# numericalEFT/MCIntegration.jl

Hardware: AMD Instinct MI355X
Metric: Msamples/sec (whole node), 16-D Gaussian :vegas (higher is better)
Workload: dtype f64

## Files before the change

mcintegration.jl_amd/_lib.py:

```python
import ctypes as C
import os

_PKG = os.path.dirname(os.path.abspath(__file__))
_SO = os.path.join(_PKG, "lib", "libmci_hip.so")

MCI_OK = 0
ERR_NAMES = {1: "INVALID", 2: "HIP", 3: "COMPILE", 4: "NORMALIZATION", 5: "HISTOGRAM", 6: "COMM", 7: "NO_DEVICE"}
CONTINUOUS, DISCRETE, FERMIK = 0, 1, 2
VEGAS, VEGASMC, MCMC = 0, 1, 2
ABI_VERSION = 5
SOLVERS = {"vegas": VEGAS, "vegasmc": VEGASMC, "mcmc": MCMC, VEGAS: VEGAS, VEGASMC: VEGASMC, MCMC: MCMC}

c_double_p = C.POINTER(C.c_double)
c_int32_p = C.POINTER(C.c_int32)


class MCIError(RuntimeError):
    def __init__(self, code, msg):
        super().__init__("[MCI_ERR_%s] %s" % (ERR_NAMES.get(code, code), msg))
        self.code = code


class LeafDesc(C.Structure):
    _fields_ = [("kind", C.c_int32), ("pool", C.c_int32), ("lower", C.c_double), ("upper", C.c_double),
# ... 54 lines not shown
    ("mci_get_histogram_copies", C.c_int, [_VP, c_int32_p]),
    ("mci_set_kernel_timing", C.c_int, [_VP, C.c_int32]),
    ("mci_iteration_run", C.c_int, [_VP, C.c_int32, C.c_int64, C.c_int64, C.c_int64, C.c_int32, C.c_uint64, C.c_int64, C.c_int64, C.c_double]),
    ("mci_iteration_reduce", C.c_int, [_VP]),
    ("mci_iteration_finish", C.c_int, [_VP, C.c_int32, C.c_int64, C.c_int32, C.c_double, c_double_p, c_double_p]),
    ("mci_integrate", C.c_int, [_VP, C.POINTER(IntegrateArgs), C.POINTER(ResultC)]),
    ("mci_integrate_sweep", C.c_int, [_VP, C.POINTER(IntegrateArgs), C.c_int32, c_double_p, C.POINTER(C.c_uint64), c_double_p, c_double_p,
                                      C.POINTER(ResultC), c_double_p, c_double_p, c_int32_p]),
    ("mci_sweep_supported", C.c_int, [_VP, C.POINTER(IntegrateArgs), C.c_char_p, C.c_int32]),
    ("mci_set_sweep_leaves", C.c_int, [_VP, C.c_int32]),
    ("mci_sweep_map_doubles", C.c_int, [_VP, c_int32_p]),
    ("mci_get_iteration_log", C.c_int, [_VP, C.c_int32, c_double_p]),
    ("mci_reserve_iteration_log", C.c_int, [_VP, C.c_int32]),
    ("mci_get_packed", C.c_int, [_VP, c_double_p, C.c_int64]),
    ("mci_set_packed", C.c_int, [_VP, c_double_p, C.c_int64]),
    ("mci_packed_device_ptr", _VP, [_VP]),
    ("mci_get_grid", C.c_int, [_VP, C.c_int32, c_double_p, C.c_int32]),
    ("mci_set_grid", C.c_int, [_VP, C.c_int32, c_double_p, C.c_int32]),
    ("mci_get_distribution", C.c_int, [_VP, C.c_int32, c_double_p, c_double_p, C.c_int32]),
    ("mci_set_distribution", C.c_int, [_VP, C.c_int32, c_double_p, C.c_int32]),
    ("mci_get_reweight", C.c_int, [_VP, c_double_p, C.c_int32]),
    ("mci_set_reweight", C.c_int, [_VP, c_double_p, C.c_int32]),
    ("mci_set_reweight_goal", C.c_int, [_VP, c_double_p, C.c_int32]),
    ("mci_get_acceptance", C.c_int, [_VP, c_double_p, c_double_p, C.c_int32]),
    ("mci_save_state", C.c_int, [_VP, C.c_char_p]),
    ("mci_load_state", C.c_int, [_VP, C.c_char_p]),
    ("mci_set_train_walk", C.c_int, [_VP, C.c_int32]),
    ("mci_set_rng_bits", C.c_int, [_VP, C.c_int32]),
    ("mci_set_rng_rounds", C.c_int, [_VP, C.c_int32]),
    ("mci_set_deterministic", C.c_int, [_VP, C.c_int32]),
    ("mci_set_chain_carry", C.c_int, [_VP, C.c_int32]),
    ("mci_set_iteration_counted", C.c_int, [_VP, C.c_int32]),
    ("mci_set_persistent", C.c_int, [_VP, C.c_int32]),
    ("mci_last_integrate_persistent", C.c_int, [_VP, C.POINTER(C.c_int32)]),
    ("mci_last_chain_launch", C.c_int, [_VP, C.POINTER(C.c_int64), c_int32_p]),
    ("mci_set_stratification", C.c_int, [_VP, C.c_int32, c_int32_p, C.c_double, C.c_int64]),
    ("mci_set_stratification_off", C.c_int, [_VP]),
    ("mci_set_stratification_carry", C.c_int, [_VP, C.c_int32]),
    ("mci_get_strat_carry", C.c_int, [_VP, c_int32_p, c_int32_p]),
    ("mci_get_stratification", C.c_int, [_VP, c_int32_p, C.POINTER(C.c_int64), c_double_p]),
    ("mci_get_strat_counts", C.c_int, [_VP, C.POINTER(C.c_int64), C.c_int64]),
    ("mci_strat_plan", C.c_int, [C.c_int64, C.c_int32, C.c_int64, c_int32_p]),
    ("mci_set_chain_speculation", C.c_int, [_VP, C.c_int32, C.c_double, C.c_int32]),
    ("mci_last_chain_speculation", C.c_int, [_VP, c_int32_p, c_int32_p]),
    ("mci_chain_speculation_status", C.c_int, [_VP, C.c_int32, c_int32_p]),
    ("mci_vegas_check_status", C.c_int, [_VP, c_int32_p, c_int32_p]),
    ("mci_last_integrate_discarded", C.c_int, [_VP, C.POINTER(C.c_int64), c_int32_p]),
    ("mci_speculation_tree", C.c_int, [C.c_int32, C.c_double, C.c_int32, c_int32_p, c_int32_p, c_int32_p, C.POINTER(C.c_uint64), C.POINTER(C.c_uint64)]),
    ("mci_compile_chain_speculation", C.c_int, [_VP, C.c_int32]),
    ("mci_train", C.c_int, [_VP]),
    ("mci_sample_dump", C.c_int, [_VP, C.c_int32, C.c_uint64, C.c_int64, C.c_int64, C.c_int64, c_double_p, c_double_p, c_double_p]),
    ("mci_kernel_times_ms", C.c_int, [_VP, C.POINTER(C.c_float), C.c_int32, c_int32_p, c_int32_p, c_int32_p]),
    ("mci_kernel_clocks", C.c_int, [_VP, c_double_p, C.c_int32, c_int32_p]),
    ("mci_comm_times_ms", C.c_int, [_VP, C.POINTER(C.c_float), C.c_int32, c_int32_p]),
    ("mci_comm_collectives", C.c_int, [_VP, C.POINTER(C.c_int64), C.POINTER(C.c_int64)]),
    ("mci_reduce_size", C.c_int, [_VP, C.POINTER(C.c_int64)]),
    ("mci_external_reduce_done", C.c_int, [_VP]),
    ("mci_standardize_block", None, [C.c_int64, C.c_int64, C.c_int64, C.POINTER(C.c_int64), C.POINTER(C.c_int64)]),
    ("mci_chain_burnin", C.c_double, [C.c_int64, C.c_int64, C.c_int32]),
    ("mci_mcmc_burnin", C.c_int64, [C.c_int64, C.c_int64, C.c_int32, C.c_int32, C.c_int32, C.c_double]),
    ("mci_mcmc_auto_chains", C.c_int64, [C.c_int64, C.c_int64, C.c_int32, C.c_int32, C.c_int32, C.c_int64, C.c_int64, C.c_int32]),
    ("mci_get_hold_histogram", C.c_int, [_VP, C.POINTER(C.c_uint64)]),
    ("mci_mcmc_launch_valid", C.c_int, [_VP, c_int32_p, c_int32_p, C.POINTER(C.c_int64), C.POINTER(C.c_int64)]),
    ("mci_iteration_discard", C.c_int, [_VP]),
    ("mci_get_block_means", C.c_int, [_VP, C.c_int32, c_double_p, C.POINTER(C.c_int64), c_int32_p]),
    ("mci_reset_block_log", C.c_int, [_VP]),
    ("mci_lineage_sums", None, [c_double_p, C.c_int64, C.c_int64, C.c_int64, c_double_p, C.c_int64, C.c_int64, c_double_p, c_double_p]),
    ("mci_maxdof", None, [c_int32_p, C.c_int32, C.c_int32, c_int32_p]),
    ("mci_mean_std", None, [c_double_p, c_double_p, C.c_int64, C.c_int64, c_double_p, c_double_p]),
    ("mci_average", None, [c_double_p, c_double_p, C.c_int64, C.c_int64, C.c_int64, c_double_p, c_double_p, c_double_p]),
    ("mci_do_reweight", None, [c_double_p, c_double_p, C.c_int64, C.c_double, c_double_p]),
    ("mci_version", C.c_char_p, []),
    ("mci_abi_version", C.c_int32, []),
]
DEBUG_SIGNATURES = [
    ("mci_debug_persist_words", C.c_int, [_VP, C.POINTER(C.c_uint64), C.c_int32]),
    ("mci_debug_walk_counts", C.c_int, [_VP, C.POINTER(C.c_int64)]),
    ("mci_debug_plant_wrong_decision", C.c_int, [_VP, C.c_int32]),
    ("mci_debug_persist_spin_ticks", C.c_int, [_VP, C.c_uint64]),
    ("mci_debug_override", C.c_int, [C.c_char_p, C.c_int64, C.c_int32]),
    ("mci_debug_compiler_id", C.c_int, [C.c_char_p, C.c_char_p, C.c_int32]),
    ("mci_debug_split_chunks", C.c_int, [_VP, C.POINTER(C.c_int64), C.POINTER(C.c_int64)]),
    ("mci_debug_vegas_cursor", C.c_int, [_VP, C.POINTER(C.c_int32), C.POINTER(C.c_uint64)]),
    ("mci_debug_strat_d", C.c_int, [_VP, c_double_p, C.c_int64]),
    ("mci_debug_strat_start_d", C.c_int, [_VP, c_double_p, C.c_int64]),
    ("mci_debug_strat_dump", C.c_int, [_VP, C.c_int64, c_double_p, c_double_p, C.POINTER(C.c_int64), c_double_p, c_double_p]),
    ("mci_debug_mcmc_policy", C.c_int, [C.c_int64, C.c_int64, C.c_int64, C.c_int64]),
    ("mci_debug_vegas_check", C.c_int, [_VP, C.c_int32, C.c_uint64, C.c_int64, C.c_int64, C.c_int64, C.c_int64, c_double_p, c_double_p, c_double_p, c_double_p,
                                        C.POINTER(C.c_int64)]),
    ("mci_debug_vegas_check_launches", C.c_int, [_VP, C.POINTER(C.c_int64)]),
    ("mci_debug_vegas_check_layout", C.c_int, [_VP, c_int32_p, c_int32_p, c_double_p, C.POINTER(C.c_uint64), c_int32_p]),
    ("mci_debug_sweep_workgroups", C.c_int, [_VP, C.c_int32]),
    ("mci_debug_sweep_threads", C.c_int, [_VP, C.c_int32]),
    ("mci_debug_sweep_last_launch", C.c_int, [_VP, c_int32_p, c_int32_p]),
    ("mci_debug_sweep_lds_bytes", C.c_int, [_VP, C.POINTER(C.c_int64)]),
]

_lib = None


def library_path():
    return _SO


def use_rocm_compiler(rocm=None):
    root = rocm or os.environ.get("ROCM_PATH") or "/opt/rocm"
    mapped = set()
    try:
        with open("/proc/self/maps") as fh:
            for line in fh:
                path = line.split(None, 5)[-1].strip() if line.count(" ") >= 5 else ""
                if "amd_comgr" in path or "hiprtc" in path:
                    mapped.add(os.path.realpath(path))
    except OSError:
        pass

    def installed(names):
        for name in names:
            path = os.path.join(root, "lib", name)
            if os.path.exists(path):
                return path
        return None
    comgr, hiprtc = installed(("libamd_comgr.so.3", "libamd_comgr.so.2", "libamd_comgr.so")), installed(("libhiprtc.so.7", "libhiprtc.so"))
    have_comgr = [p for p in mapped if "amd_comgr" in p]
    if have_comgr and (comgr is None or os.path.realpath(comgr) not in have_comgr):
        return False
    done = False
    for path in (comgr, hiprtc):
        if path is not None:
            C.CDLL(path, mode=C.RTLD_GLOBAL)
            done = True
    return done


def compiler_id():
    buf = C.create_string_buffer(1024)
    lib().mci_debug_compiler_id(None, buf, len(buf))
    return buf.value.decode()


def lib():
    global _lib
    if _lib is None:
        if not os.path.exists(_SO):
            raise ImportError("%s is missing: run `python __graft_entry__.py` (hipcc --offload-arch=gfx950) first; "
                              "the MI355X engine has no Python/CPU fallback" % _SO)
        L = C.CDLL(_SO, mode=C.RTLD_GLOBAL)
        for name, res, args in SIGNATURES + DEBUG_SIGNATURES:
            fn = getattr(L, name)
            fn.restype = res
            fn.argtypes = args
        if L.mci_abi_version() != ABI_VERSION:
            raise ImportError("%s has ABI %d, this package was written against ABI %d: rebuild with `python __graft_entry__.py`" % (_SO, L.mci_abi_version(), ABI_VERSION))
        _lib = L
    return _lib


def check(rc):
    if rc != MCI_OK:
        raise MCIError(rc, lib().mci_last_error().decode(errors="replace"))
```

mcintegration.jl_amd/csrc/mci_debug.h:

```cpp
#ifndef MCI_DEBUG_H
#define MCI_DEBUG_H
#include "../../include/mci.h"
#ifdef __cplusplus
extern "C" {
#endif
int mci_debug_persist_words(mci_problem *prob, unsigned long long *out, int32_t n);
int mci_debug_walk_counts(mci_problem *prob, int64_t *out);
int mci_debug_plant_wrong_decision(mci_problem *prob, int32_t on);
int mci_debug_persist_spin_ticks(mci_problem *prob, unsigned long long ticks);
int mci_debug_override(const char *key, int64_t value, int32_t on);
int mci_debug_split_chunks(const mci_problem *prob, int64_t *chunks, int64_t *bytes);
int mci_debug_strat_dump(mci_problem *prob, int64_t n, double *x, double *y, int64_t *h, double *jac, double *w);
int mci_debug_strat_d(mci_problem *prob, double *d, int64_t n);
int mci_debug_strat_start_d(mci_problem *prob, double *d, int64_t n);
int mci_debug_vegas_cursor(const mci_problem *prob, int32_t *used, uint64_t *base);
int mci_debug_compiler_id(const char *set, char *out, int32_t n);
int mci_debug_mcmc_policy(int64_t pilot_steps, int64_t grow, int64_t carry_holds, int64_t carry_half_floors);
int mci_debug_vegas_check(mci_problem *prob, int32_t iteration, uint64_t seed, int64_t nevalperblock, int64_t block_lo, int64_t nblocks,
                          int64_t measurefreq, const double *x, const double *jac, const double *w, double *packed, int64_t *bad);
int mci_debug_vegas_check_launches(const mci_problem *prob, int64_t *launches);
int mci_debug_vegas_check_layout(const mci_problem *prob, int32_t *head, int32_t *draws, double *scales, uint64_t *own, int32_t *obs);
int mci_debug_sweep_workgroups(mci_problem *prob, int32_t g);
int mci_debug_sweep_threads(mci_problem *prob, int32_t threads);
int mci_debug_sweep_last_launch(const mci_problem *prob, int32_t *workgroups, int32_t *threads);
int mci_debug_sweep_lds_bytes(const mci_problem *prob, int64_t *bytes);
#ifdef __cplusplus
}
#endif
#endif
```

mcintegration.jl_amd/csrc/mci_device.h:

```cpp
#pragma once

namespace mci {

typedef unsigned int u32;
typedef unsigned long long u64;
typedef long long i64;

template <int I> struct IC { static constexpr int value = I; };

template <int B, int E, class F> __device__ __forceinline__ void static_for(F &&f) {
    if constexpr (B < E) {
        f(IC<B>{});
        static_for<B + 1, E>(f);
    }
}

struct u32x4 { u32 x, y, z, w; };

#ifndef MCI_PHILOX_ROUNDS
#define MCI_PHILOX_ROUNDS 10
#endif

template <bool IN_VGPR> struct RoundKeys {
    u32 a[MCI_PHILOX_ROUNDS], b[MCI_PHILOX_ROUNDS];
// ... 87 lines not shown
    return __longlong_as_double((i64)(((u64)whi << 32) | (w << 20)));
}
template <int DPC, int J> __device__ __forceinline__ double block_u12(const u32x4 &r) {
    if constexpr (DPC == 2) return J == 0 ? u12(r.x, r.y) : u12(r.z, r.w);
    else return u12_word(J == 0 ? r.x : J == 1 ? r.y : J == 2 ? r.z : r.w);
}

enum { STREAM_VEGAS = 0, STREAM_POOLINIT = 1, STREAM_MC_INIT = 2, STREAM_MC_STEP = 3, STREAM_MCMC_INIT = 4, STREAM_MCMC_STEP = 5, STREAM_MCMC_GROUP = 6, STREAM_MC_GROUP = 7 };
enum { ST_NORMALIZATION = 1, ST_HIST_NONFINITE = 2, ST_HIST_NONPOSITIVE = 4, ST_RESCALE_NONFINITE = 8, ST_MCMC_INIT = 16, ST_PERSIST_STALL = 32 };

struct SpecNode {
    int depth;
    int anc;
    int nacc;
    int levels;
    u64 needacc;
    u64 needrej;
    u64 accdepth;
    u64 anydepth;
};

struct BatchArgs {
    const double *edges;
    const double *dacc;
    const double *ddist;
    const double *reweight;
    const double *ud;
    double *part_cols;
    double *part_hist;
    double *ghist;
    double *part_pa;
    u64 seed;
    u32 iteration;
    i64 neval_per_block;
    i64 block_lo;
    int wg_per_block;
    i64 measurefreq;
    i64 nchain;
    double burnin;
    i64 nburn;
    int *status;
    double *tile_w;
    u32 *tile_bins;
    i64 tile_stride;
    i64 chunk_lo, chunk_hi, chunk_len;
    int accum;
    i64 nrows;
    int tiles_wpb;
    i64 tiles_rows;
    const double *host_w;
    double *host_mx, *host_relw;
    int *host_midx;
    i64 hm_first, hm_count, hm_stride;
    unsigned long long *hold_hist;
    int hist_atomic;
    const double *carry_x;
    const int *carry_curr;
    i64 carry_nchain, carry_cap;
    const int *carry_src;
    double *store_x;
    int *store_curr;
    i64 store_cap;
    const double *carry_P;
    double *carry_w;
    i64 carry_total;
    double *store_P;
    struct HostStep {
        i64 ne, steps, nc;
        double *cx, *cprob, *cw, *cprobability;
        int *cbin;
        double *hx, *pprob, *pprop, *puacc;
        int *pbin, *pvi;
        double *cwabs;
        int *ccurr, *cit, *ctr;
        int *pnew, *put;
        int *hidx;
        int *done;
    } hs;
    const SpecNode *spec_tab;
    int spec_lanes, spec_maxacc;
    int spec_ntree, spec_first;
    float spec_accept[8];
    u64 *clock_out;
    u64 *cursor;
    u64 cursor_base;
    u32 cursor_log2_big, cursor_ones;
};
constexpr int kCursorStride = 32;

struct DumpArgs {
    const double *edges, *dacc, *ddist, *ud;
    double *x, *jac, *w;
    int soa;
    u64 seed;
    u32 iteration;
    i64 first_index;
    i64 n;
};

template <int CTRL, int ROW_MASK> __device__ __forceinline__ double dpp_read(double v) {
    const u64 u = (u64)__double_as_longlong(v);
    const int lo = __builtin_amdgcn_update_dpp(0, (int)(u32)u, CTRL, ROW_MASK, 0xf, false);
    const int hi = __builtin_amdgcn_update_dpp(0, (int)(u32)(u >> 32), CTRL, ROW_MASK, 0xf, false);
    return __longlong_as_double((long long)(((u64)(u32)hi << 32) | (u64)(u32)lo));
}
__device__ __forceinline__ double wave_scan_incl(double v) {
    v += dpp_read<0x111, 0xf>(v);
    v += dpp_read<0x112, 0xf>(v);
    v += dpp_read<0x114, 0xf>(v);
    v += dpp_read<0x118, 0xf>(v);
    v += dpp_read<0x142, 0xa>(v);
    v += dpp_read<0x143, 0xc>(v);
    return v;
}
__device__ __forceinline__ double wave_sum(double v) {
    const u64 u = (u64)__double_as_longlong(wave_scan_incl(v));
    const u32 lo = (u32)__builtin_amdgcn_readlane((int)(u32)u, 63), hi = (u32)__builtin_amdgcn_readlane((int)(u32)(u >> 32), 63);
    return __longlong_as_double((long long)(((u64)hi << 32) | (u64)lo));
}

__device__ __forceinline__ void lds_add(double *p, double v) {
    __hip_atomic_fetch_add(p, v, __ATOMIC_RELAXED, __HIP_MEMORY_SCOPE_WORKGROUP);
}
__device__ __forceinline__ void global_add(double *p, double v) {
    __hip_atomic_fetch_add(p, v, __ATOMIC_RELAXED, __HIP_MEMORY_SCOPE_AGENT);
}

template <class Cfg> struct Mode {
    static constexpr bool EDGE_LDS = Cfg::TABLE_MODE <= 1;
    static constexpr bool HIST_LDS = Cfg::TABLE_MODE == 0 || Cfg::TABLE_MODE == 3;
};

template <class Cfg> struct Tables {
    const double *EC;
    const double *E;
    const double *DA;
    const double *DD;
};

template <int N, bool FMA, bool U12> __device__ __forceinline__ double cont_yn(double y) {
    if constexpr (FMA) {
        double Nd = (double)N;
        asm("" : "+s"(Nd));
        return __builtin_fma(y, Nd, -Nd);
    } else return (U12 ? y - 1.0 : y) * (double)N;
}
template <class Cfg> constexpr bool all_draws_pair_table() {
    if (Cfg::PAIR_TABLE == 0 || Cfg::TABLE_MODE > 1) return false;
    for (int k = 0; k < Cfg::NDRAW; ++k)
        if (Cfg::leaf_kind(Cfg::draw_leaf(k)) != 0) return false;
    return true;
}

#ifndef MCI_GATHER_X4
#define MCI_GATHER_X4 0
#endif
__device__ __forceinline__ void gather_edges(const double *e, double &g0, double &g1) {
#if MCI_GATHER_X4
    typedef double d2u __attribute__((ext_vector_type(2), aligned(8)));
    const d2u v = *reinterpret_cast<const d2u *>(e);
    g0 = v.x;
    g1 = v.y;
#else
    g0 = e[0];
    g1 = e[1];
#endif
// ... 606 lines not shown
        double *prow = a.part_pa + rowid * (2 * PaTable<Cfg>::N);
        for (int i = tid; i < 2 * PaTable<Cfg>::N && tile == 0; i += T) prow[i] = ACCUM ? prow[i] + (double)sPA[i] : (double)sPA[i];
    }
    if constexpr (Mode<Cfg>::HIST_LDS && WRITE_HIST) {
#ifndef MCI_COPY_SUM_DPP
#define MCI_COPY_SUM_DPP 0
#endif
        constexpr bool SUMMED = MCI_COPY_SUM_DPP != 0 && Cfg::DET == 0 && Cfg::HCOPY > 1 && Cfg::HCOPY <= 16 && Cfg::NTILE == 1;
        if constexpr (SUMMED) {
            constexpr int N = Cfg::HTILE * Cfg::HCOPY, K = 4;
            for (int base = 0; base < N; base += T * K) {
                double v[K];
                static_for<0, K>([&](auto Kk) {
                    constexpr int k = decltype(Kk)::value;
                    const int j = base + k * T + tid;
                    v[k] = j < N ? sH[j] : 0.0;
                });
                static_for<0, K>([&](auto Kk) {
                    constexpr int k = decltype(Kk)::value;
                    if constexpr (Cfg::HCOPY > 1) v[k] += dpp_read<0x111, 0xf>(v[k]);
                    if constexpr (Cfg::HCOPY > 2) v[k] += dpp_read<0x112, 0xf>(v[k]);
                    if constexpr (Cfg::HCOPY > 4) v[k] += dpp_read<0x114, 0xf>(v[k]);
                    if constexpr (Cfg::HCOPY > 8) v[k] += dpp_read<0x118, 0xf>(v[k]);
                });
                __syncthreads();
                static_for<0, K>([&](auto Kk) {
                    constexpr int k = decltype(Kk)::value;
                    const int j = base + k * T + tid;
                    if (j < N && (tid & (Cfg::HCOPY - 1)) == Cfg::HCOPY - 1) sH[j / Cfg::HCOPY] = v[k];
                });
            }
            __syncthreads();
        }
        static_for<0, Cfg::NTILE>([&](auto Tt) {
            constexpr int tt = decltype(Tt)::value;
            if (tile == tt) {
                double *hrow = a.part_hist + rowid * Cfg::NBIN + Cfg::tile_boff(tt);
                for (int i = tid; i < Cfg::tile_nbin(tt); i += T) {
                    constexpr int SB = (Cfg::DET != 0 || SUMMED) ? 1 : Cfg::HCOPY, SC = Cfg::DET != 0 ? Cfg::HTILE : 1;
                    double v = sH[i * SB];
                    if constexpr (!SUMMED)
                    static_for<1, Cfg::HCOPY>([&](auto Cc) { v += sH[i * SB + decltype(Cc)::value * SC]; });
                    if (!accum && a.hist_atomic) {
                        if (v != 0.0) global_add(&a.ghist[(rowid % a.hist_atomic) * Cfg::NBIN + Cfg::tile_boff(tt) + i], v);
                    } else
                    hrow[i] = accum ? hrow[i] + v : v;
                }
            }
        });
    }
}

struct CursorRule {
    u64 units;
    u32 waves;
    u32 log2_big, ones;
};
__host__ __device__ inline u64 cursor_ones(const CursorRule &r) { return (u64)r.ones * r.waves; }
__host__ __device__ inline u64 cursor_tickets(const CursorRule &r) {
    if (r.units <= cursor_ones(r)) return r.units;
    u64 rem = r.units - cursor_ones(r), n = cursor_ones(r);
    for (u32 l = 1; l < r.log2_big; ++l) {
        const u64 level = (u64)r.waves << l;
        if (rem <= level) return n + ((rem + (1ull << l) - 1ull) >> l);
        n += r.waves;
        rem -= level;
    }
    return n + ((rem + (1ull << r.log2_big) - 1ull) >> r.log2_big);
}
__host__ __device__ inline void cursor_range(const CursorRule &r, u64 ntickets, u64 t, u64 &u0, u64 &u1) {
    u64 q = ntickets - 1ull - t, e, z = 1ull;
    if (q < cursor_ones(r)) e = q;
    else {
        q -= cursor_ones(r);
        u32 l = 1;
        for (; l < r.log2_big && q >= r.waves; ++l) q -= r.waves;
        z = 1ull << l;
        e = (u64)r.waves * (r.ones + z - 2ull) + q * z;
    }
    u1 = r.units - e;
    u0 = e + z < r.units ? r.units - e - z : 0ull;
}

struct WorkItem {
    i64 rowid, lb;
    int slice, tile;
};
template <class Cfg> __device__ __forceinline__ WorkItem work_item(const BatchArgs &a) {
    WorkItem w;
#ifdef MCI_WORK_ITEM_FROM_CALLER
    w.tile = 0;
    w.rowid = a.chunk_lo;
#else
    w.tile = Cfg::NTILE == 1 ? 0 : (int)(blockIdx.x % Cfg::NTILE);
    w.rowid = Cfg::NTILE == 1 ? (i64)blockIdx.x : (i64)(blockIdx.x / Cfg::NTILE);
#endif
    w.lb = w.rowid / a.wg_per_block;
    w.slice = (int)(w.rowid % a.wg_per_block);
    return w;
}

template <class Cfg, bool SPLIT = false> __device__ __forceinline__ void vegas_batch(const BatchArgs &a) {
    extern __shared__ __attribute__((aligned(16))) double smem[];
    const int tid = threadIdx.x, T = blockDim.x;
    constexpr bool NOHIST = SPLIT && Cfg::SPLIT_ALL != 0;
    constexpr bool EC = Cfg::EC_DOUBLES > 0 && (NOHIST || !SPLIT);
    using L = typename SelectType<NOHIST, LdsEC<Cfg>, Lds<Cfg>>::type;
    double *sE = smem + L::E, *sDA = smem + L::DA, *sDD = smem + L::DD;
    double *sH = smem + L::H, *sO = smem + L::O;
    stage_tables<Cfg>(a.edges, a.dacc, a.ddist, sE, sDA, sDD);
#ifndef MCI_ZERO_B128
#define MCI_ZERO_B128 0
#endif
    if constexpr (Mode<Cfg>::HIST_LDS && !NOHIST) {
        if constexpr (MCI_ZERO_B128 != 0 && L::H % 2 == 0 && (Cfg::HTILE * Cfg::HCOPY) % 2 == 0) {
            typedef double d2 __attribute__((ext_vector_type(2)));
            d2 *z = reinterpret_cast<d2 *>(sH);
            for (int i = tid; i < Cfg::HTILE * Cfg::HCOPY / 2; i += T) z[i] = d2{0.0, 0.0};
        } else
        for (int i = tid; i < Cfg::HTILE * Cfg::HCOPY; i += T) sH[i] = 0.0;
    }
    for (int i = tid; i < Cfg::NOBS * ocopy<Cfg>(); i += T) sO[i] = 0.0;
    Tables<Cfg> t;
    t.EC = nullptr;
    if constexpr (EC) {
        double *sEC = smem + (NOHIST ? LdsEC<Cfg>::EC : Lds<Cfg>::END);
        static_for<0, Cfg::NLEAF>([&](auto Lf) {
            constexpr int l = decltype(Lf)::value;
            if constexpr (Cfg::leaf_kind(l) == 0 && Cfg::leaf_ecoff(l) >= 0)
                for (int i = tid; i <= Cfg::leaf_nbin(l); i += T) sEC[Cfg::leaf_ecoff(l) + i] = a.edges[Cfg::leaf_eoff(l) + i];
        });
        t.EC = sEC;
    }
    __syncthreads();
    if constexpr (Mode<Cfg>::EDGE_LDS) t.E = sE;
    else t.E = a.edges;
    t.DA = sDA;
    t.DD = sDD;

    WorkItem wi = work_item<Cfg>(a);
    if constexpr (SPLIT) {
        wi.tile = 0;
        wi.rowid = (i64)blockIdx.x;
        wi.lb = wi.rowid / a.wg_per_block;
        wi.slice = (int)(wi.rowid % a.wg_per_block);
    }
    const int slice = wi.slice, tile = wi.tile;
    const i64 B = a.block_lo + wi.lb;
    const u32 stream = a.iteration * 8u + STREAM_VEGAS;
    const bool pulled = pipe_eligible<Cfg>() && !SPLIT && !EC && a.cursor != nullptr;
    const i64 stride = pulled ? 64 : (i64)a.wg_per_block * T;

    double acc[Cfg::NW];
    static_for<0, Cfg::NW>([&](auto I) { acc[decltype(I)::value] = 0.0; });
    double extra[Cfg::NCOLS - Cfg::NOBS];
    static_for<0, Cfg::NCOLS - Cfg::NOBS>([&](auto I) { extra[decltype(I)::value] = 0.0; });

#ifndef MCI_PIPE_VGPR_KEYS
#define MCI_PIPE_VGPR_KEYS 0
#endif
    constexpr bool KV = MCI_PIPE_VGPR_KEYS != 0 && pipe_eligible<Cfg>() && !SPLIT && Cfg::EC_DOUBLES == 0;
    constexpr int DPC = Cfg::RNG_BITS == 32 ? 4 : 2;
    const RoundKeys<KV> keys = make_round_keys<KV>((u32)a.seed, (u32)(a.seed >> 32));
    const i64 mfreq = a.measurefreq;
    const i64 n_lo = SPLIT ? a.chunk_lo : 0, n_hi = SPLIT ? a.chunk_hi : a.neval_per_block;
    i64 mrem = mfreq == 1 ? 0 : (n_lo + (i64)slice * T + tid + 1) % mfreq;
    const i64 mstep = mfreq == 1 ? 0 : stride % mfreq;
    constexpr bool PHASED = Cfg::L1_PHASE > 0 && Cfg::HOST_INTEGRAND == 0 && gather_draw_count<Cfg, EC>() > 0;
    auto run = [&](auto TT, auto MF1c) {
    constexpr bool MF1 = decltype(MF1c)::value != 0;
    auto process = [&](const i64 n, const Sample<Cfg> &s, double *defer_wh = nullptr, auto... counted) {
        constexpr bool COUNTED = sizeof...(counted) > 0;
        double w[Cfg::NW];
        if constexpr (Cfg::HOST_INTEGRAND != 0) {
            const i64 hidx = wi.lb * a.neval_per_block + n;
            static_for<0, Cfg::NW>([&](auto Q) { w[decltype(Q)::value] = a.host_w[decltype(Q)::value * a.tile_stride + hidx]; });
        } else {
            Cfg::integrand(s.x, w, a.ud, -1);
        }
        if constexpr (!COUNTED) extra[Cols<Cfg>::NEVAL - Cfg::NOBS] += 1.0;
        bool domeasure = true;
        if constexpr (!MF1) {
            domeasure = mrem == 0;
            mrem += mstep;
            mrem = mrem >= mfreq ? mrem - mfreq : mrem;
        }
        if constexpr (Cfg::HOST_MEASURE != 0) {
            const i64 hidx = wi.lb * a.neval_per_block + n;
            static_for<0, Cfg::NDRAW>([&](auto K) { a.host_mx[decltype(K)::value * a.tile_stride + hidx] = s.x[decltype(K)::value]; });
            static_for<0, Cfg::NW>([&](auto Q) {
                constexpr int q = decltype(Q)::value;
                a.host_relw[q * a.tile_stride + hidx] = domeasure ? w[q] * s.jaci[q / Cfg::NCOMP] : 0.0;
// ... 68 lines not shown
                    r = __hip_atomic_fetch_add((global_u64 *)addr, 1ull, __ATOMIC_RELAXED, __HIP_MEMORY_SCOPE_AGENT);
                }
                return r;
            };
            auto ticket = [&](u64 r) -> u64 {
                const u32 lo = (u32)__builtin_amdgcn_readfirstlane((int)(u32)r), hi = (u32)__builtin_amdgcn_readfirstlane((int)(u32)(r >> 32));
                return (((u64)hi << 32) | lo) - a.cursor_base;
            };
            i64 n = (i64)slice * T + tid, lim = a.neval_per_block;
            u32 trips = 0u;
            u64 next = 0ull;
            if (pulled) {
                next = pull();
                n = lim = 0;
            }
            for (;;) {
                if (pulled) {
                    const u64 t = ticket(next);
                    if (t >= ntickets) break;
                    next = pull();
                    u64 u0, u1;
                    cursor_range(rule, ntickets, t, u0, u1);
                    n = (i64)(u0 << 7) + (tid & 63);
                    lim = (i64)(u1 << 7) < a.neval_per_block ? (i64)(u1 << 7) : a.neval_per_block;
                    if constexpr (!MF1) mrem = (n + 1) % mfreq;
                }
                for (; n + stride < lim; n += 2 * stride) {
                    {
                        Sample<Cfg> s;
                        draw_sample_pipe<Cfg, KV, DPC, UNI>(keys, head, stream, first + (u64)n, s, pa, pb, sH);
                        process(n, s, pb.wh, 0);
                    }
                    {
                        Sample<Cfg> s;
                        draw_sample_pipe<Cfg, KV, DPC, UNI>(keys, head, stream, first + (u64)(n + stride), s, pb, pa, sH);
                        process(n + stride, s, pa.wh, 0);
                    }
                    trips += 1u;
                }
                if (!pulled) break;
            }
            double count = 2.0 * (double)trips;
            if (n < lim) {
                Sample<Cfg> s;
                draw_sample_pipe<Cfg, KV, DPC, UNI>(keys, head, stream, first + (u64)n, s, pa, pb, sH);
                process(n, s, pb.wh, 0);
                flush(pb);
                count += 1.0;
            } else flush(pa);
            extra[Cols<Cfg>::NEVAL - Cfg::NOBS] += count;
            if constexpr (MF1) extra[Cols<Cfg>::NORM - Cfg::NOBS] += count;
        };
        if (uniform_hi) loop(IC<1>{});
        else loop(IC<0>{});
    } else {
        for (i64 n = n_lo + (i64)slice * T + tid; n < n_hi; n += stride) {
            Sample<Cfg> s;
            draw_sample<Cfg, EC, KV, DPC>(t, keys, stream, (u64)(B * a.neval_per_block + n), s);
            process(n, s);
        }
    }
    };
#ifndef MCI_MF_ONLY
#define MCI_MF_ONLY 0
#endif
    auto run_mf = [&](auto TT) { run(TT, IC<(MCI_MF_ONLY != 0 ? 1 : 0)>{}); };
    const bool stamp = !SPLIT && Cfg::NTILE == 1 && a.clock_out != nullptr && blockIdx.x == 0 && tid < 64;
    u64 ck0 = 0ull, rt0 = 0ull;
    if (stamp) {
        ck0 = __builtin_amdgcn_s_memtime();
        rt0 = __builtin_amdgcn_s_memrealtime();
    }
    if constexpr (Cfg::NTILE == 1 || SPLIT) run_mf(IC<0>{});
    else static_for<0, Cfg::NTILE>([&](auto TT) { if (tile == decltype(TT)::value) run_mf(TT); });
    if (stamp) {
        const u64 ck1 = __builtin_amdgcn_s_memtime(), rt1 = __builtin_amdgcn_s_memrealtime();
        if (tid == 0) {
            a.clock_out[0] = ck1 - ck0;
            a.clock_out[1] = rt1 - rt0;
        }
    }
    __syncthreads();
    flush_workgroup<Cfg, L, !NOHIST>(a, smem, acc, extra, wi.rowid, tile);
}

#ifndef MCI_THREADS
#define MCI_THREADS 256
#endif
constexpr int kTilesU = MCI_THREADS >= 768 ? 8 : 4;
template <int... D> struct ISeq {};
template <int N, int... D> struct MakeISeq : MakeISeq<N - 1, N - 1, D...> {};
template <int... D> struct MakeISeq<0, D...> { typedef ISeq<D...> type; };
template <int G, int SH, class V, int... D> __device__ __forceinline__ V rotate_lanes(const V b, ISeq<D...>) {
    return __builtin_shufflevector(b, b, ((D + SH) % G)...);
}
template <class Cfg> constexpr int tile_draw_count(int tt) {
    int n = 0;
    for (int k = 0; k < Cfg::NDRAW; ++k) n += (is_tdraw<Cfg>(k) && Cfg::leaf_tile(Cfg::draw_leaf(k)) == tt) ? 1 : 0;
    return n;
}
template <class Cfg> constexpr int tile_draw(int tt, int gi) {
    int n = 0;
    for (int k = 0; k < Cfg::NDRAW; ++k)
        if (is_tdraw<Cfg>(k) && Cfg::leaf_tile(Cfg::draw_leaf(k)) == tt) {
            if (n == gi) return k;
            ++n;
        }
    return 0;
}
template <class Cfg> constexpr bool tile_banked(int tt) {
    const int G = tile_draw_count<Cfg>(tt);
    if (G < 2 || G > 16) return false;
    const int k0 = tile_draw<Cfg>(tt, 0), NB = Cfg::leaf_nbin(Cfg::draw_leaf(k0));
    if (Cfg::tile_nbin(tt) != G * NB) return false;
    for (int gi = 0; gi < G; ++gi) {
        const int k = tile_draw<Cfg>(tt, gi), leaf = Cfg::draw_leaf(k);
        if (Cfg::leaf_kind(leaf) != 0 || Cfg::leaf_nbin(leaf) != NB || Cfg::cover_mask(k) != Cfg::cover_mask(k0)) return false;
        if (Cfg::leaf_boff(leaf) - Cfg::tile_boff(tt) != gi * NB) return false;
    }
    return true;
}
template <class Cfg> __device__ __forceinline__ void vegas_tiles(const BatchArgs &a) {
    static_assert(Cfg::HCOPY == 1, "histogram copies go with one tile");
    extern __shared__ __attribute__((aligned(16))) double smem[];
    const int tid = threadIdx.x, T = blockDim.x;
    double *sH = smem + Lds<Cfg>::H;
    constexpr int T0 = Cfg::SPLIT_ALL != 0 ? 0 : 1;
    constexpr int NTM = Cfg::NTILE - T0 > 0 ? Cfg::NTILE - T0 : 1;
    const i64 q = (i64)blockIdx.x / 8;
    const int tile = T0 + (int)(q % NTM);
    const i64 rowid = (q / NTM) * 8 + (i64)(blockIdx.x % 8);
    const int wpb = a.tiles_wpb > 0 ? a.tiles_wpb : a.wg_per_block;
    if (rowid >= (a.tiles_rows > 0 ? a.tiles_rows : a.nrows)) return;
    const i64 lb = rowid / wpb;
    const int slice = (int)(rowid % wpb);
    for (int i = tid; i < Cfg::HTILE * Cfg::HCOPY; i += T) sH[i] = 0.0;
    __syncthreads();
    const i64 stride = (i64)wpb * T;
    static_for<T0, Cfg::NTILE>([&](auto TT) {
        constexpr int tt = decltype(TT)::value;
        if (tile == tt) {
            constexpr int U = kTilesU;
            constexpr int NWORD = tdraw_words<Cfg>();
            static_assert(U % 4 == 0, "the replay takes its samples in groups of four");
            const i64 cnt = a.chunk_hi - a.chunk_lo;
            const bool wide = (cnt & 3) == 0 && (a.chunk_len & 3) == 0 && (a.tile_stride & 3) == 0;
            const i64 per = wide ? 4 : 1;
            for (i64 n0 = ((i64)slice * T + tid) * per; n0 < cnt; n0 += stride * U) {
                double wh[U][Cfg::NI];
                u32 word[U][NWORD > 0 ? NWORD : 1];
                bool live[U];
                static_for<0, NWORD>([&](auto J) {
                    static_for<0, U>([&](auto Uu) { word[decltype(Uu)::value][decltype(J)::value] = 0u; });
                });
                if (wide) {
                    static_for<0, U / 4>([&](auto Q) {
                        constexpr int q = decltype(Q)::value;
                        const i64 n = n0 + (i64)q * stride * 4;
                        const bool lv = n < cnt;
                        const i64 idx = lb * a.chunk_len + (lv ? n : n0);
                        static_for<0, 4>([&](auto Vv) { live[4 * q + decltype(Vv)::value] = lv; });
                        typedef double d2 __attribute__((ext_vector_type(2)));
                        typedef u32 u4 __attribute__((ext_vector_type(4)));
                        static_for<0, Cfg::NI>([&](auto I) {
                            constexpr int i = decltype(I)::value;
                            const d2 *pw = reinterpret_cast<const d2 *>(a.tile_w + (i64)i * a.tile_stride + idx);
// ... 1392 lines not shown
```

mcintegration.jl_amd/csrc/mci_host_access.h:

```cpp
int mci_get_iteration_log(mci_problem *p, int32_t nrows, double *out) {
    if (p->ctx->offline) return fail(MCI_ERR_NO_DEVICE, "offline context");
    if (nrows < 1 || nrows > p->log_row) return fail(MCI_ERR_INVALID, "only %d iterations are logged", p->log_row);
    HIPCHK(hipMemcpyAsync(out, p->d_iterlog + (size_t)(p->log_row - nrows) * p->nstat, (size_t)nrows * p->nstat * sizeof(double),
                          hipMemcpyDeviceToHost, p->ctx->stream));
    return check_status(p);
}

int mci_get_packed(mci_problem *p, double *out, int64_t n) {
    if (p->ctx->offline) return fail(MCI_ERR_NO_DEVICE, "offline context");
    if (n != p->packed_n && n != p->packed_n + 64)
        return fail(MCI_ERR_INVALID, "packed size is %lld", (long long)p->packed_n);
    if (int rc = flush_merge(p)) return rc;
    HIPCHK(hipMemcpyAsync(out, p->d_packed, (size_t)n * sizeof(double), hipMemcpyDeviceToHost, p->ctx->stream));
    HIPCHK(hipStreamSynchronize(p->ctx->stream));
    return MCI_OK;
}

int mci_set_packed(mci_problem *p, const double *in, int64_t n) {
    if (p->ctx->offline) return fail(MCI_ERR_NO_DEVICE, "offline context");
    if (n != p->packed_n && n != p->packed_n + 64)
        return fail(MCI_ERR_INVALID, "packed size is %lld", (long long)p->packed_n);
    if (int rc = flush_merge(p)) return rc;
    HIPCHK(hipMemcpyAsync(p->d_packed, in, (size_t)n * sizeof(double), hipMemcpyHostToDevice, p->ctx->stream));
    HIPCHK(hipStreamSynchronize(p->ctx->stream));
// ... 217 lines not shown
        }
        if (ok && (prod == 0 || prod != nc || !(c_beta >= 0.0) || !std::isfinite(c_beta))) {
            fclose(f);
            return fail(MCI_ERR_INVALID, "%s: the carried allocation's plan does not match its ncube = %llu (prod nstrat = %llu, beta = %g)", path,
                        (unsigned long long)nc, (unsigned long long)prod, c_beta);
        }
        if (ok) {
            c_d.resize((size_t)nc);
            ok = fread(c_d.data(), sizeof(double), c_d.size(), f) == c_d.size();
        }
        for (size_t h = 0; ok && h < c_d.size(); ++h)
            if (!(c_d[h] >= 0.0) || !std::isfinite(c_d[h])) {
                fclose(f);
                return fail(MCI_ERR_INVALID, "%s: d_h[%zu] = %g of the carried allocation is negative or not finite", path, h, c_d[h]);
            }
    }
    fclose(f);
    if (!ok) return fail(MCI_ERR_INVALID, "%s is truncated", path);
    {
        auto &st = p->strat;
        st.c_valid = !c_d.empty();
        st.c_host = std::move(c_d);
        st.c_nstrat = c_nstrat;
        st.c_ncube = (int64_t)st.c_host.size();
        st.c_beta = c_beta;
        if (st.carry) st.alloc_valid = st.alloc_pending = false;
    }
    int rc = mci_set_reweight(p, rw.data(), p->ni + 1);
    for (size_t l = 0; l < p->leaves.size() && !rc; ++l)
        if (p->leaves[l].kind != MCI_FERMIK)
        rc = p->leaves[l].kind == MCI_CONTINUOUS ? mci_set_grid(p, (int)l, tabs[l].data(), (int)tabs[l].size())
                                                 : mci_set_distribution(p, (int)l, tabs[l].data(), (int)tabs[l].size());
    return rc;
}

static int sample_dump_device(mci_problem *p, int32_t iteration, uint64_t seed, int64_t first_index, int64_t n) {
    int rc = ensure_dump(p);
    if (rc) return rc;
    HIPCHK(hipSetDevice(p->ctx->device));
    const auto &s = p->shape;
    const int64_t per = s.ndraw + 1 + s.ni * s.ncomp;
    if (n * per > p->cap_dump) {
        if (p->d_dump) (void)hipFree(p->d_dump);
        p->d_dump = nullptr;
        p->cap_dump = 0;
        HIPCHK(hipMalloc((void **)&p->d_dump, (size_t)(n * per) * sizeof(double)));
        p->cap_dump = n * per;
    }
    mci::DumpArgs a{};
    a.edges = p->d_edges;
    a.dacc = p->d_dacc;
    a.ddist = p->d_ddist;
    a.ud = p->d_ud;
    a.x = p->d_dump;
    a.jac = p->d_dump + n * s.ndraw;
    a.w = a.jac + n;
    a.seed = seed;
    a.iteration = (mci::u32)iteration;
    a.first_index = first_index;
    a.n = n;
    void *args[] = {&a};
    const unsigned grid = (unsigned)((n + 255) / 256 < 1024 ? (n + 255) / 256 : 1024);
    HIPCHK(hipModuleLaunchKernel(p->f_dump, grid, 1, 1, 256, 1, 1, (unsigned)p->lds_bytes, p->ctx->stream, args, nullptr));
    return MCI_OK;
}

int mci_sample_dump(mci_problem *p, int32_t iteration, uint64_t seed, int64_t nevalperblock, int64_t block_index, int64_t n,
                    double *x, double *jac, double *w) {
    if (p->ctx->offline) return fail(MCI_ERR_NO_DEVICE, "offline context");
    if (n < 1 || n > nevalperblock) return fail(MCI_ERR_INVALID, "n must be in 1..neval_per_block");
    int rc = sample_dump_device(p, iteration, seed, block_index * nevalperblock, n);
    if (rc) return rc;
    const auto &s = p->shape;
    const double *dx = p->d_dump, *djac = dx + n * s.ndraw, *dw = djac + n;
    if (x) HIPCHK(hipMemcpyAsync(x, dx, (size_t)n * s.ndraw * sizeof(double), hipMemcpyDeviceToHost, p->ctx->stream));
    if (jac) HIPCHK(hipMemcpyAsync(jac, djac, (size_t)n * sizeof(double), hipMemcpyDeviceToHost, p->ctx->stream));
    if (w) HIPCHK(hipMemcpyAsync(w, dw, (size_t)n * s.ni * s.ncomp * sizeof(double), hipMemcpyDeviceToHost, p->ctx->stream));
    HIPCHK(hipStreamSynchronize(p->ctx->stream));
    return MCI_OK;
}

int mci_set_kernel_timing(mci_problem *p, int32_t mode) {
    if (!p) return fail(MCI_ERR_INVALID, "NULL argument");
    p->kernel_timing = mode < 0 ? -1 : mode > 0 ? 1 : 0;
    return MCI_OK;
}

int mci_kernel_times_ms(mci_problem *p, float *ms, int32_t n, int32_t *got, int32_t *wg, int32_t *threads) {
    if (p->ctx->offline) return fail(MCI_ERR_NO_DEVICE, "offline context");
    HIPCHK(hipStreamSynchronize(p->ctx->stream));
    int64_t have = p->launch.launches < mci_problem::kEvRing ? p->launch.launches : mci_problem::kEvRing;
    if (have > n) have = n;
    int64_t k = 0;
    for (int64_t i = 0; i < have; ++i) {
        const int slot = (int)((p->launch.launches - have + i) % mci_problem::kEvRing);
        if (!p->launch.ev_valid[slot]) continue;
        float t = 0.f;
        HIPCHK(hipEventElapsedTime(&t, p->evs[2 * slot], p->evs[2 * slot + 1]));
        ms[k++] = t;
    }
    have = k;
    if (got) *got = (int32_t)have;
    if (wg) *wg = p->launch.last_wg;
    if (threads) *threads = p->launch.last_threads;
    return MCI_OK;
}

int mci_kernel_clocks(mci_problem *p, double *mhz, int32_t n, int32_t *got) {
    if (!p || !mhz || !got) return fail(MCI_ERR_INVALID, "NULL argument");
    if (p->ctx->offline) return fail(MCI_ERR_NO_DEVICE, "offline context");
    *got = 0;
    if (!p->d_clocks) return MCI_OK;
    HIPCHK(hipSetDevice(p->ctx->device));
    int khz = 0;
    HIPCHK(hipDeviceGetAttribute(&khz, hipDeviceAttributeWallClockRate, p->ctx->device));
    std::vector<unsigned long long> h((size_t)2 * mci_problem::kEvRing);
    HIPCHK(hipMemcpyAsync(h.data(), p->d_clocks, h.size() * sizeof(unsigned long long), hipMemcpyDeviceToHost, p->ctx->stream));
    HIPCHK(hipStreamSynchronize(p->ctx->stream));
    int64_t have = p->launch.launches < mci_problem::kEvRing ? p->launch.launches : mci_problem::kEvRing;
    if (have > n) have = n;
    int32_t k = 0;
    for (int64_t i = 0; i < have; ++i) {
        const int slot = (int)((p->launch.launches - have + i) % mci_problem::kEvRing);
        if (!p->launch.ev_valid[slot] || !p->launch.clock_valid[slot] || !h[(size_t)2 * slot + 1]) continue;
        mhz[k++] = (double)h[(size_t)2 * slot] / (double)h[(size_t)2 * slot + 1] * (double)khz * 1.0e-3;
    }
    *got = k;
    return MCI_OK;
}
```

mcintegration.jl_amd/csrc/mci_host_iteration.h:

```cpp
int mci_iteration_run(mci_problem *p, int32_t solver, int64_t nevalperblock, int64_t block_lo, int64_t block_hi,
                      int32_t iteration, uint64_t seed, int64_t measurefreq, int64_t nchain, double thermal_ratio) {
    if (p->ctx->offline) return fail(MCI_ERR_NO_DEVICE, "offline context: no device to run on");
    if (solver != MCI_VEGAS && solver != MCI_VEGASMC && solver != MCI_MCMC) return fail(MCI_ERR_INVALID, "Solver %d is not supported!", solver);
    const bool auto_chains = nchain <= 0;
    if (measurefreq <= 0) return fail(MCI_ERR_INVALID, "measurefreq must be positive");
    const int64_t nblocks = block_hi - block_lo;
    if (nblocks < 1 || nevalperblock < 1) return fail(MCI_ERR_INVALID, "empty iteration");
    if (p->has_fermik && solver != MCI_MCMC) return fail(MCI_ERR_INVALID, "FermiK variables work with solver=:mcmc only");
    if (p->strat.on) {
        if (solver != MCI_VEGAS) return fail(MCI_ERR_INVALID, "stratification works with solver = :vegas only (mci_set_stratification_off first)");
        return strat_run(p, nevalperblock, block_lo, block_hi, iteration, seed, measurefreq);
    }
    const int kern = (p->in_self_check && p->check_slot >= 0 && solver == MCI_VEGAS) ? p->check_slot : kslot(solver, measurefreq);
    int rc = (solver == MCI_VEGAS || p->deterministic || p->shape.host_integrand || p->spec_lanes == 1) ? compile_solver(p, kern) : MCI_OK;
    if (rc) return rc;
    if (solver == MCI_VEGAS && !p->in_self_check && !p->vegas_check_done[kern == kSlotVegasAny ? 1 : 0] &&
        (rc = vegas_check_gate(p, kern, nevalperblock, block_lo, block_hi, iteration, seed, measurefreq)))
        return rc;
    if (solver == MCI_VEGAS && (rc = compile_solver(p, kern))) return rc;
    if (solver == MCI_VEGAS && p->shape.host_integrand && (rc = ensure_dump(p))) return rc;
    if ((rc = flush_merge(p))) return rc;
    HIPCHK(hipSetDevice(p->ctx->device));
    const auto &s = p->shape;
    int T = solver_threads(p, solver);
// ... 35 lines not shown
        for (int v = 0; v < p->npool; ++v) nslots += p->maxdof[v];
        if (!(thermal_ratio >= 0.0)) return fail(MCI_ERR_INVALID, "thermal_ratio must be non-negative");
        if (nchain <= 0) {
            if ((rc = hold_consume(p))) return rc;
            const int64_t hold_eff = p->launch.mcmc_warm && p->launch.hold_prev > p->launch.hold_max ? p->launch.hold_prev : p->launch.hold_max;
            nchain = mci_mcmc_auto_chains(nevalperblock, nblocks, nslots, p->ni + 1, p->npool, hold_eff, p->launch.mcmc_warm && p->launch.hold_valid ? 0 : p->launch.hold_len,
                                          may_carry ? 1 : 0);
        }
        if (nchain > nevalperblock) return fail(MCI_ERR_INVALID, "nchain=%lld exceeds the %lld steps of a block", (long long)nchain, (long long)nevalperblock);
        nburn = (may_carry && nchain > 1) ? 0 : mci_mcmc_burnin(nevalperblock / nchain, nchain, nslots, p->ni + 1, p->npool, thermal_ratio);
        units = nchain;
    } else {
        nchain = 1;
    }
    int G = 1, spec_maxacc = 0;
    if (solver != MCI_VEGAS && !s.host_integrand && !p->deterministic && p->spec_lanes != 1) {
        if (p->spec_lanes > 1) G = p->spec_lanes;
        else {
            G = 64;
            while (G > 1 && nblocks * nchain * G > mci_problem::kSpecFill) G >>= 1;
            if (G < 8) G = 1;
        }
    }
    int T_launch = T;
    if (G > 1 && p->spec_state[solver - 1] < 0) G = 1;
    if (G > 1) {
        rc = compile_spec(p, solver);
        if (rc == MCI_ERR_COMPILE && p->spec_lanes == -1) {
            fprintf(stderr, "mci: the several-lanes-per-chain kernel of this problem did not compile; one lane per chain instead\n%s\n", mci_last_error());
            p->spec_state[solver - 1] = -2;
            G = 1;
        } else if (rc) return rc;
    }
    if (G > 1 && !p->in_self_check && ((p->spec_need_check[solver - 1] && !(g_over.spec_self_check.on && g_over.spec_self_check.v == 0)) ||
                                       (g_over.spec_self_check.on && g_over.spec_self_check.v == 1 && p->spec_state[solver - 1] == 0))) {
        if ((rc = spec_self_check(p, solver, G, nevalperblock, block_lo, block_hi, iteration, seed, measurefreq, thermal_ratio))) return rc;
        if (p->spec_state[solver - 1] < 0) G = 1;
    }
    if (G > 1) {
        if ((rc = spec_upload(p, solver, G, p->spec_accept, p->spec_maxacc))) return rc;
        spec_maxacc = p->spec_tab_maxacc;
        units = nchain * G;
        T_launch = units >= 256 ? 256 : (int)((units + 63) / 64) * 64;
    }
    if (G == 1 && (rc = compile_solver(p, kern))) return rc;
    p->launch.last_spec_lanes = G;
    p->launch.last_spec_maxacc = spec_maxacc;
    int wpb = p->wg_per_block;
    if (G > 1) {
        if (wpb <= 0) wpb = (int)((2048 + nblocks - 1) / nblocks);
        const int64_t maxw = (units + T_launch - 1) / T_launch;
        if (wpb > maxw) wpb = (int)maxw;
        if (wpb < 1) wpb = 1;
    } else
    if (wpb <= 0) {
        const int64_t big = T >= 1024 ? 1024 : T >= 512 ? 2048 : 4096;
        int64_t target = (units * nblocks >= (int64_t)1 << 25 && p->lds_bytes <= 32 * 1024) ? big : 2048;
        if (solver == MCI_VEGAS && units * nblocks < ((int64_t)1 << 22) && target > 256) target = 256;
        if (solver == MCI_VEGAS && units * nblocks * s.ndraw < ((int64_t)1 << 19) && target > 64) target = 64;
        wpb = (int)((target + nblocks - 1) / nblocks);
        const int64_t maxw = (units + T - 1) / T;
        if (wpb > maxw) wpb = (int)maxw;
        if (wpb < 1) wpb = 1;
    }
    bool cursor = false;
    if (solver == MCI_VEGAS && G == 1 && !p->in_self_check && vegas_pipe_unit(p) && !(g_over.vegas_cursor.on && g_over.vegas_cursor.v == 0)) {
        const bool forced = g_over.vegas_cursor.on && g_over.vegas_cursor.v == 1;
        if (forced) cursor = true;
        else if (p->wg_per_block <= 0 && units * nblocks >= ((int64_t)1 << 25)) {
            int resident = 0;
            if ((rc = cursor_resident(p, kern, T, &resident))) return rc;
            if (resident >= nblocks && (resident / nblocks) * nblocks > kAtomicRows) {
                cursor = true;
                wpb = (int)(resident / nblocks);
                const int64_t maxw = (units + T - 1) / T;
                if (wpb > maxw) wpb = (int)maxw;
            }
        }
    }
    const bool hist_lds = (s.table_mode == 0 || s.table_mode == 3);
    const bool split = solver == MCI_VEGAS && s.ntile > 1;
    if (!split && wpb * s.ntile > 4096 / nblocks && s.ntile > 1) wpb = (int)(4096 / nblocks / s.ntile) > 0 ? (int)(4096 / nblocks / s.ntile) : 1;
    const int64_t nrows = nblocks * wpb;
    const bool atomic_flush = solver == MCI_VEGAS && hist_lds && s.ntile == 1 && atomic_rows_ok(p) && nrows <= kAtomicRows && !s.host_integrand;
    const int64_t nwg = split ? nrows : nrows * s.ntile;
    if ((rc = ensure_capacity(p, nrows, nblocks))) return rc;
    if (solver != MCI_VEGAS && nrows > p->cap_pa) {
        if (p->d_part_pa) (void)hipFree(p->d_part_pa);
        p->d_part_pa = nullptr;
        p->cap_pa = 0;
        HIPCHK(hipMalloc((void **)&p->d_part_pa, (size_t)nrows * 2 * p->npa * sizeof(double)));
        p->cap_pa = nrows;
    }
    int64_t chunk_len = nevalperblock, nchunks = 1;
    if (split) {
        const int64_t words = p->tdraw_words > 0 ? p->tdraw_words : 1;
        const int64_t bytes = (int64_t)s.ni * 8 + words * 4;
        if (!s.host_integrand && !s.host_measure) {
            int64_t cap = (int64_t)1 << 27;
            if (cap * bytes > (int64_t)7500000000) cap = (int64_t)7500000000 / bytes;
            if (g_over.split_chunk.on && g_over.split_chunk.v > 0) cap = g_over.split_chunk.v;
            int64_t per = (cap / nblocks) & ~(int64_t)3;
            if (per < 4) per = 4;
            if (per < chunk_len) {
                chunk_len = per;
                nchunks = (nevalperblock + chunk_len - 1) / chunk_len;
            }
        }
        const int64_t nsamp = nblocks * chunk_len;
        if (nsamp > p->cap_tile) {
            tile_release(p);
            const size_t wbytes = (((size_t)nsamp * s.ni * sizeof(double)) + 255) & ~(size_t)255;
            if ((rc = tile_alloc(p, wbytes + (size_t)nsamp * words * sizeof(uint32_t)))) return rc;
            p->d_tile_bins = (uint32_t *)((char *)p->d_tile_w + wbytes);
            p->cap_tile = nsamp;
        }
        p->launch.last_split_chunks = nchunks;
        p->launch.last_split_bytes = nsamp * bytes;
    }
    mci::BatchArgs a{};
    a.edges = p->d_edges;
    a.dacc = p->d_dacc;
    a.ddist = p->d_ddist;
    a.reweight = p->d_reweight;
    a.ud = p->d_ud;
    a.part_cols = p->d_part_cols;
    a.part_hist = p->d_part_hist;
    a.ghist = p->d_ghist;
    a.part_pa = p->d_part_pa;
    a.seed = seed;
    a.iteration = (mci::u32)iteration;
    a.neval_per_block = nevalperblock;
    a.block_lo = block_lo;
    a.wg_per_block = wpb;
    a.measurefreq = measurefreq;
    a.nchain = nchain;
    a.burnin = burnin;
    a.nburn = nburn;
    const int ghist_buffers = atomic_flush ? (nrows > 64 ? 3 : 1) : 0;
    a.hist_atomic = ghist_buffers;
    if (solver != MCI_VEGAS) {
        const bool carried = may_carry && nchain > 1;
        const bool keep = carry_on && nchain > 1;
        if (keep && p->in_self_check) return fail(MCI_ERR_INVALID, "the self-check's launch would overwrite the stored chains");
        if (carried) {
            a.carry_x = p->d_chain_x[p->launch.chain_cur];
            a.carry_curr = p->d_chain_curr[p->launch.chain_cur];
            a.carry_nchain = p->launch.chain_nchain;
            a.carry_cap = p->chain_cap[p->launch.chain_cur];
        }
        if (carried) {
            if (nblocks * nchain > p->cap_carry_src) {
                if (p->d_carry_src) (void)hipFree(p->d_carry_src);
                p->d_carry_src = nullptr;
                p->cap_carry_src = 0;
                HIPCHK(hipMalloc((void **)&p->d_carry_src, (size_t)(nblocks * nchain) * sizeof(int)));
                p->cap_carry_src = nblocks * nchain;
            }
            if (nblocks * p->launch.chain_nchain > p->cap_carry_W) {
                if (p->d_carry_W) (void)hipFree(p->d_carry_W);
                p->d_carry_W = nullptr;
                p->cap_carry_W = 0;
                HIPCHK(hipMalloc((void **)&p->d_carry_W, (size_t)(nblocks * p->launch.chain_nchain) * sizeof(double)));
                p->cap_carry_W = nblocks * p->launch.chain_nchain;
            }
            mci::ResampleArgs ra{};
            ra.curr_old = p->d_chain_curr[p->launch.chain_cur];
// ... 164 lines not shown
        } else {
            const int64_t mfq = measurefreq > 0 ? measurefreq : 1;
            const int64_t last = solver == MCI_VEGASMC ? nevalperblock / nchain : nevalperblock / nchain + nburn;
            hm_first = 1;
            if (solver == MCI_VEGASMC) {
                hm_first = (int64_t)(burnin / (double)mfq);
                if (hm_first < 1) hm_first = 1;
                while (hm_first > 1 && (double)((hm_first - 1) * mfq) >= burnin) --hm_first;
                while ((double)(hm_first * mfq) < burnin) ++hm_first;
            } else if (nburn > 0) {
                hm_first = (nburn + mfq - 1) / mfq;
                if (hm_first < 1) hm_first = 1;
            }
            hm_count = last / mfq - hm_first + 1;
            if (hm_count < 0) hm_count = 0;
            hm_n = nchain * hm_count;
            hm_rows = solver == MCI_MCMC ? s.ncomp : nw;
        }
        const int64_t n = nblocks * hm_n > 0 ? nblocks * hm_n : 1;
        if ((double)n * (double)(s.ndraw + nw + 1) * 8.0 > 8.0 * 1024 * 1024 * 1024)
            return fail(MCI_ERR_INVALID, "a host measure over %lld records of %d doubles per launch (more than 8 GiB): lower neval, raise measurefreq "
                                         "or give the measure as device source (mci_set_measure_source)", (long long)n, s.ndraw + nw);
        if (n > p->cap_hmeas) {
            if (p->d_mx) (void)hipFree(p->d_mx);
            if (p->d_mrelw) (void)hipFree(p->d_mrelw);
            if (p->d_midx) (void)hipFree(p->d_midx);
            if (p->h_mx) (void)hipHostFree(p->h_mx);
            if (p->h_mrelw) (void)hipHostFree(p->h_mrelw);
            if (p->h_midx) (void)hipHostFree(p->h_midx);
            p->d_mx = p->d_mrelw = p->h_mx = p->h_mrelw = nullptr;
            p->d_midx = p->h_midx = nullptr;
            p->cap_hmeas = 0;
            HIPCHK(hipMalloc((void **)&p->d_mx, (size_t)n * s.ndraw * sizeof(double)));
            HIPCHK(hipMalloc((void **)&p->d_mrelw, (size_t)n * nw * sizeof(double)));
            HIPCHK(hipMalloc((void **)&p->d_midx, (size_t)n * sizeof(int32_t)));
            HIPCHK(hipHostMalloc((void **)&p->h_mx, (size_t)n * s.ndraw * sizeof(double), hipHostMallocDefault));
            HIPCHK(hipHostMalloc((void **)&p->h_mrelw, (size_t)n * nw * sizeof(double), hipHostMallocDefault));
            HIPCHK(hipHostMalloc((void **)&p->h_midx, (size_t)n * sizeof(int32_t), hipHostMallocDefault));
            p->cap_hmeas = n;
        }
        if (nblocks * s.nobs > p->cap_mobs) {
            if (p->d_mobs) (void)hipFree(p->d_mobs);
            p->d_mobs = nullptr;
            HIPCHK(hipMalloc((void **)&p->d_mobs, (size_t)nblocks * s.nobs * sizeof(double)));
            p->cap_mobs = nblocks * s.nobs;
        }
        a.host_mx = p->d_mx;
        a.host_relw = p->d_mrelw;
        a.host_midx = p->d_midx;
        a.hm_first = hm_first;
        a.hm_count = hm_count;
        a.hm_stride = nblocks * hm_n;
        if (solver != MCI_VEGAS) {
            HIPCHK(hipMemsetAsync(p->d_mx, 0, (size_t)n * s.ndraw * sizeof(double), p->ctx->stream));
            HIPCHK(hipMemsetAsync(p->d_mrelw, 0, (size_t)n * hm_rows * sizeof(double), p->ctx->stream));
            HIPCHK(hipMemsetAsync(p->d_midx, 0xFF, (size_t)n * sizeof(int32_t), p->ctx->stream));
        }
    }
    if (cursor) {
        mci::CursorRule r;
        r.units = (mci::u64)((nevalperblock + 127) >> 7);
        r.waves = (mci::u32)(wpb * (T / 64));
        r.log2_big = (mci::u32)(g_over.cursor_log2_big.on && g_over.cursor_log2_big.v >= 1 && g_over.cursor_log2_big.v <= 16 ? g_over.cursor_log2_big.v : mci_problem::kCursorLog2Big);
        r.ones = (mci::u32)(g_over.cursor_ones.on && g_over.cursor_ones.v >= 1 && g_over.cursor_ones.v <= 4096 ? g_over.cursor_ones.v : mci_problem::kCursorOnes);
        if (nblocks != p->cursor_nblocks) {
            if (nblocks > p->cap_cursor) {
                if (p->d_cursor) (void)hipFree(p->d_cursor);
                p->d_cursor = nullptr;
                p->cap_cursor = 0;
                HIPCHK(hipMalloc((void **)&p->d_cursor, (size_t)nblocks * mci::kCursorStride * sizeof(unsigned long long)));
                p->cap_cursor = nblocks;
            }
            HIPCHK(hipMemsetAsync(p->d_cursor, 0, (size_t)nblocks * mci::kCursorStride * sizeof(unsigned long long), p->ctx->stream));
            p->cursor_nblocks = nblocks;
            p->cursor_base = 0;
        }
        a.cursor = p->d_cursor;
        a.cursor_base = p->cursor_base;
        a.cursor_log2_big = r.log2_big;
        a.cursor_ones = r.ones;
        p->cursor_base += mci::cursor_tickets(r) + r.waves;
    }
    p->launch.last_cursor = cursor;
    void *args[] = {&a};
    hipFunction_t f = p->f_solver[G > 1 ? (solver == MCI_VEGASMC ? kSlotVegasmcSpec : kSlotMcmcSpec) : kern];
    hipStream_t st = p->ctx->stream;
    const int slot = (int)(p->launch.launches % mci_problem::kEvRing);
    p->launch.time_this_launch = p->kernel_timing > 0 || (p->kernel_timing < 0 && nblocks * nevalperblock >= ((int64_t)1 << 20));
    if (p->launch.time_this_launch && solver == MCI_VEGAS) {
        if (!p->d_clocks) {
            HIPCHK(hipMalloc((void **)&p->d_clocks, (size_t)2 * mci_problem::kEvRing * sizeof(unsigned long long)));
            HIPCHK(hipMemsetAsync(p->d_clocks, 0, (size_t)2 * mci_problem::kEvRing * sizeof(unsigned long long), st));
        }
        a.clock_out = p->d_clocks + 2 * slot;
    }
    if (p->launch.time_this_launch) HIPCHK(hipEventRecord(p->evs[2 * slot], st));
    if (solver != MCI_VEGAS && s.host_integrand) {
        const int64_t nc = nblocks * nchain, steps = nevalperblock / nchain;
        const int nw = s.ni * s.ncomp, nd = s.ndraw;
        if (nc >= ((int64_t)1 << 31) || steps + nburn >= ((int64_t)1 << 31) - 1) return fail(MCI_ERR_INVALID, "too many chains or steps for the host-closure path");
        if (nc > p->cap_hstep) {
            if (p->d_hstep) (void)hipFree(p->d_hstep);
            p->d_hstep = nullptr;
            p->cap_hstep = 0;
            HIPCHK(hipMalloc(&p->d_hstep, (size_t)nc * ((3 * nd + nw + 4) * sizeof(double) + (2 * nd + 7) * sizeof(int)) + 16));
            p->cap_hstep = nc;
        }
        if (nc > p->cap_hidx) {
            if (p->h_hidx) (void)hipHostFree(p->h_hidx);
            p->h_hidx = nullptr;
            p->cap_hidx = 0;
            HIPCHK(hipHostMalloc((void **)&p->h_hidx, (size_t)(nc + 1) * sizeof(int32_t), hipHostMallocDefault));
            p->cap_hidx = nc;
        }
        {
            double *dp = (double *)p->d_hstep;
            a.hs.cx = dp; dp += (size_t)nd * nc;
            a.hs.cprob = dp; dp += (size_t)nd * nc;
            a.hs.pprob = dp; dp += (size_t)nd * nc;
            a.hs.cw = dp; dp += (size_t)nw * nc;
            a.hs.cprobability = dp; dp += nc;
            a.hs.pprop = dp; dp += nc;
            a.hs.puacc = dp; dp += nc;
            a.hs.cwabs = dp; dp += nc;
            int *ip = (int *)dp;
            a.hs.cbin = ip; ip += (size_t)nd * nc;
            a.hs.pbin = ip; ip += (size_t)nd * nc;
            a.hs.pvi = ip; ip += nc;
            a.hs.ccurr = ip; ip += nc;
            a.hs.cit = ip; ip += nc;
            a.hs.ctr = ip; ip += nc;
            a.hs.pnew = ip; ip += nc;
            a.hs.put = ip; ip += nc;
            a.hs.hidx = ip; ip += nc;
            a.hs.done = ip;
        }
        a.hs.hx = p->d_hx;
        a.hs.nc = nc;
        a.hs.steps = steps;
        HIPCHK(hipMemsetAsync(p->d_part_cols, 0, (size_t)nrows * s.ncols * sizeof(double), st));
        if (hist_lds && s.nbin > 0) HIPCHK(hipMemsetAsync(p->d_part_hist, 0, (size_t)nrows * s.nbin * sizeof(double), st));
        HIPCHK(hipMemsetAsync(p->d_part_pa, 0, (size_t)nrows * 2 * p->npa * sizeof(double), st));
        HIPCHK(hipMemsetAsync(a.hs.done, 0, sizeof(int), st));
        if (solver == MCI_VEGASMC) {
            for (int64_t ne = 0; ne <= steps + 1; ++ne) {
                a.hs.ne = ne;
                HIPCHK(hipModuleLaunchKernel(f, (unsigned)nwg, 1, 1, (unsigned)T, 1, 1, (unsigned)solver_lds(p, solver), st, args, nullptr));
                if (ne > steps) break;
                HIPCHK(hipMemcpyAsync(p->h_hx, p->d_hx, (size_t)nc * nd * sizeof(double), hipMemcpyDeviceToHost, st));
                HIPCHK(hipStreamSynchronize(st));
                if ((rc = eval_host_integrand(p, nullptr, p->h_hx, p->h_hw, nc))) return rc;
                HIPCHK(hipMemcpyAsync(p->d_hw, p->h_hw, (size_t)nc * nw * sizeof(double), hipMemcpyHostToDevice, st));
            }
        } else {
            const int64_t limit = steps + nburn + 2 + 10000;
            for (int64_t ne = 0;; ++ne) {
                a.hs.ne = ne;
                HIPCHK(hipModuleLaunchKernel(f, (unsigned)nwg, 1, 1, (unsigned)T, 1, 1, (unsigned)solver_lds(p, solver), st, args, nullptr));
                HIPCHK(hipMemcpyAsync(p->h_hidx, a.hs.hidx, (size_t)(nc + 1) * sizeof(int32_t), hipMemcpyDeviceToHost, st));
                HIPCHK(hipMemcpyAsync(p->h_hx, p->d_hx, (size_t)nc * nd * sizeof(double), hipMemcpyDeviceToHost, st));
                HIPCHK(hipStreamSynchronize(st));
                if (p->h_hidx[nc] >= nc) break;
                if (ne > limit) return fail(MCI_ERR_INVALID, "host-closure :mcmc chains did not finish (%d of %lld)", (int)p->h_hidx[nc], (long long)nc);
                if ((rc = eval_host_integrand(p, p->h_hidx, p->h_hx, p->h_hw, nc))) return rc;
                HIPCHK(hipMemcpyAsync(p->d_hw, p->h_hw, (size_t)nc * s.ncomp * sizeof(double), hipMemcpyHostToDevice, st));
            }
        }
    } else
    for (int64_t c = 0; c < nchunks; ++c) {
        if (nchunks > 1) {
            a.chunk_lo = c * chunk_len;
            a.chunk_hi = a.chunk_lo + chunk_len < nevalperblock ? a.chunk_lo + chunk_len : nevalperblock;
            a.accum = c > 0 ? 1 : 0;
        }
        HIPCHK(hipModuleLaunchKernel(f, (unsigned)nwg, 1, 1, (unsigned)T_launch, 1, 1, (unsigned)solver_lds(p, solver), st, args, nullptr));
        if (split && c + 1 < nchunks)
            HIPCHK(hipModuleLaunchKernel(p->f_tiles[kern == kSlotVegasAny ? 1 : 0], (unsigned)(((hist_rows + 7) / 8) * 8 * (s.ntile - (s.split_all ? 0 : 1))), 1, 1, (unsigned)T, 1, 1, (unsigned)p->lds_bytes, st, args, nullptr));
    }
    if (solver == MCI_MCMC) p->launch.hold_measured = a.hold_hist != nullptr;
    if (a.hold_hist && auto_chains && (rc = hold_publish(p, nevalperblock / nchain, solver != MCI_VEGAS && p->launch.last_carried))) return rc;
    if (split)
        HIPCHK(hipModuleLaunchKernel(p->f_tiles[kern == kSlotVegasAny ? 1 : 0], (unsigned)(((hist_rows + 7) / 8) * 8 * (s.ntile - (s.split_all ? 0 : 1))), 1, 1, (unsigned)T, 1, 1, (unsigned)p->lds_bytes, st, args, nullptr));
    if (p->launch.time_this_launch) HIPCHK(hipEventRecord(p->evs[2 * slot + 1], st));
    p->launch.ev_valid[slot] = p->launch.time_this_launch;
    p->launch.clock_valid[slot] = a.clock_out != nullptr && !split && s.ntile == 1;
    p->launch.launches += 1;
    if (s.host_measure) {
        const int64_t n = nblocks * hm_n;
        const int nw = s.ni * s.ncomp, nc = s.ncomp;
        std::vector<double> obs((size_t)nblocks * s.nobs, 0.0);
        if (n > 0 && !p->in_self_check) {
            HIPCHK(hipMemcpyAsync(p->h_mx, p->d_mx, (size_t)n * s.ndraw * sizeof(double), hipMemcpyDeviceToHost, st));
            HIPCHK(hipMemcpyAsync(p->h_mrelw, p->d_mrelw, (size_t)n * hm_rows * sizeof(double), hipMemcpyDeviceToHost, st));
            if (solver == MCI_MCMC) HIPCHK(hipMemcpyAsync(p->h_midx, p->d_midx, (size_t)n * sizeof(int32_t), hipMemcpyDeviceToHost, st));
            HIPCHK(hipStreamSynchronize(st));
            const double *relw = p->h_mrelw;
            if (solver == MCI_MCMC && p->hmeas_fn) {
                p->h_mtmp.assign((size_t)n * nw, 0.0);
                for (int64_t i = 0; i < n; ++i)
                    if (p->h_midx[i] >= 0)
                        for (int q = 0; q < nc; ++q) p->h_mtmp[(size_t)(p->h_midx[i] * nc + q) * n + i] = p->h_mrelw[(size_t)q * n + i];
                relw = p->h_mtmp.data();
            }
            if (solver != MCI_MCMC && p->hmeas_idx_fn) p->h_mitmp.resize((size_t)hm_n);
            const bool squeeze = solver == MCI_VEGAS && measurefreq > 1;
            const int64_t keep = squeeze ? nevalperblock / measurefreq : hm_n;
            std::vector<double> sx, sw;
            if (squeeze) {
                sx.resize((size_t)(keep > 0 ? keep : 1) * s.ndraw);
                sw.resize((size_t)(keep > 0 ? keep : 1) * nw);
            }
            for (int64_t b = 0; b < nblocks; ++b) {
                const int64_t off = b * hm_n;
                double *ob = obs.data() + (size_t)b * s.nobs;
                int hrc = 0;
                if (squeeze) {
                    for (int k = 0; k < s.ndraw; ++k)
                        for (int64_t j = 0; j < keep; ++j) sx[(size_t)k * keep + j] = p->h_mx[(size_t)k * n + off + (j + 1) * measurefreq - 1];
                    for (int q = 0; q < nw; ++q)
                        for (int64_t j = 0; j < keep; ++j) sw[(size_t)q * keep + j] = relw[(size_t)q * n + off + (j + 1) * measurefreq - 1];
                    if (p->hmeas_fn) hrc = p->hmeas_fn(sx.data(), sw.data(), keep, keep, s.ndraw, nw, block_lo + b, ob, s.nobs, p->hmeas_user);
                    else {
                        p->h_mitmp.resize((size_t)(keep > 0 ? keep : 1));
                        for (int j = 0; j < s.ni && !hrc; ++j) {
                            std::fill(p->h_mitmp.begin(), p->h_mitmp.end(), (int32_t)j);
                            hrc = p->hmeas_idx_fn(p->h_mitmp.data(), sx.data(), sw.data() + (size_t)j * nc * keep, keep, keep, s.ndraw, nc, block_lo + b, ob,
                                                  s.nobs, p->hmeas_user);
                        }
                    }
                } else if (p->hmeas_fn) {
                    hrc = p->hmeas_fn(p->h_mx + off, relw + off, hm_n, n, s.ndraw, nw, block_lo + b, ob, s.nobs, p->hmeas_user);
                } else if (solver == MCI_MCMC) {
                    hrc = p->hmeas_idx_fn(p->h_midx + off, p->h_mx + off, relw + off, hm_n, n, s.ndraw, nc, block_lo + b, ob, s.nobs, p->hmeas_user);
                } else {
                    for (int j = 0; j < s.ni && !hrc; ++j) {
                        std::fill(p->h_mitmp.begin(), p->h_mitmp.end(), (int32_t)j);
                        hrc = p->hmeas_idx_fn(p->h_mitmp.data(), p->h_mx + off, relw + (size_t)j * nc * n + off, hm_n, n, s.ndraw, nc, block_lo + b, ob,
                                              s.nobs, p->hmeas_user);
                    }
                }
                if (hrc) return fail(MCI_ERR_INVALID, "the host measure failed (%d)", hrc);
            }
        }
        HIPCHK(hipMemcpyAsync(p->d_mobs, obs.data(), obs.size() * sizeof(double), hipMemcpyHostToDevice, st));
        hipLaunchKernelGGL(mci::k_add_host_obs, dim3((unsigned)((nblocks * s.nobs + 255) / 256)), dim3(256), 0, st, p->d_mobs, (int)nblocks, s.nobs, s.ncols, wpb,
                           p->d_part_cols);
        HIPCHK(hipGetLastError());
        HIPCHK(hipStreamSynchronize(st));
    }
    p->launch.last_samples = nblocks * nevalperblock;
    p->launch.last_wg = (int)nwg;
    p->launch.last_threads = T_launch;
    p->launch.last_nblocks = (int)nblocks;
    if (solver != MCI_VEGAS) p->launch.last_nchain = nchain;
    const int nb256 = (s.nbin + 255) / 256;
    if (hist_lds && s.nbin > 0 && !atomic_flush)
        hipLaunchKernelGGL(mci::k_hist_stage1, dim3(nb256, mci_problem::kGroups), dim3(256), 0, st, p->d_part_hist, (int)hist_rows, s.nbin,
                           (int)mci_problem::kGroups, p->d_stage1);
    HIPCHK(hipGetLastError());
    mci::MergeArgs &m = p->merge;
    m.part_cols = p->d_part_cols;
    m.ncols = s.ncols;
    m.nobs = s.nobs;
    m.ni = s.ni;
    m.nblocks = (int)nblocks;
    m.wg_per_block = wpb;
    m.stage1 = p->d_stage1;
    m.ngroup = (int)mci_problem::kGroups;
    m.ghist = p->d_ghist;
    m.use_ghist = (hist_lds && !atomic_flush) ? 0 : atomic_flush ? ghist_buffers : 1;
    m.nbin = s.nbin;
    m.packed = p->d_packed;
    m.status = p->d_status;
    m.scratch = p->d_scratch;
    m.part_pa = solver != MCI_VEGAS ? p->d_part_pa : nullptr;
    m.npa = p->npa;
    m.nrows = (int)nrows;
    m.block_means = nullptr;
    m.hist_no_offset = (p->in_self_check && p->check_slot >= 0) ? 1 : 0;
    m.hold = a.hold_hist;
    if (solver != MCI_VEGAS && !p->in_self_check) {
        const int64_t stride = nblocks * s.nobs;
        if (stride != p->launch.blk_stride || block_lo != p->launch.blk_lo) {
            p->launch.blk_rows = 0;
            p->launch.blk_carried = 0;
            p->launch.blk_stride = stride;
            p->launch.blk_lo = block_lo;
        }
        if ((rc = grow_block_log(p, p->launch.blk_rows + 1))) return rc;
        m.block_means = p->d_blocklog + (size_t)p->launch.blk_rows * stride;
        p->launch.blk_rows += 1;
        p->launch.blk_carried += p->launch.last_carried ? 1 : 0;
    }
    p->merge_pending = true;
    return MCI_OK;
}

static int flush_merge(mci_problem *p) {
    if (!p->merge_pending) return MCI_OK;
    p->merge_pending = false;
    HIPCHK(hipSetDevice(p->ctx->device));
    const int nb256 = (p->shape.nbin + 255) / 256;
    hipLaunchKernelGGL(mci::k_finalize, dim3(nb256 + 1 + (2 * p->npa + 3) / 4), dim3(256), 0, p->ctx->stream, p->merge);
    HIPCHK(hipGetLastError());
    return MCI_OK;
}

int mci_iteration_reduce(mci_problem *p) {
    if (p->ctx->offline) return fail(MCI_ERR_NO_DEVICE, "offline context");
    if (!p->ctx->comm) return MCI_OK;
    int rc = flush_merge(p);
    if (rc) return rc;
    const bool timed = p->launch.time_this_launch;
    const int slot = (int)(p->reduces % mci_problem::kCevRing);
    if (timed) {
        if (p->cevs.empty()) {
            p->cevs.resize(2 * mci_problem::kCevRing);
            for (auto &e : p->cevs) HIPCHK(hipEventCreate(&e));
        }
        HIPCHK(hipEventRecord(p->cevs[2 * slot], p->ctx->stream));
    }
    const size_t count = (size_t)p->packed_n + (p->launch.hold_deferred ? 64 : 0);
    int r = g_rccl.AllReduce(p->d_packed, p->d_packed, count, kNcclFloat64, kNcclSum, p->ctx->comm, p->ctx->stream);
    if (r) return fail(MCI_ERR_COMM, "ncclAllReduce: %s", g_rccl.GetErrorString ? g_rccl.GetErrorString(r) : "?");
    p->ctx->collectives += 1;
    p->ctx->last_count = (long long)count;
    if (p->launch.hold_deferred && (rc = hold_publish_reduced(p))) return rc;
    if (timed) HIPCHK(hipEventRecord(p->cevs[2 * slot + 1], p->ctx->stream));
    p->cev_valid[slot] = timed;
    p->reduces += 1;
    return MCI_OK;
}

int mci_comm_collectives(const mci_ctx *c, int64_t *calls, int64_t *last_count) {
    if (!c) return fail(MCI_ERR_INVALID, "NULL argument");
    if (calls) *calls = c->collectives;
    if (last_count) *last_count = c->last_count;
    return MCI_OK;
}

int mci_external_reduce_done(mci_problem *p) {
    if (!p) return fail(MCI_ERR_INVALID, "NULL argument");
    if (p->ctx->offline) return fail(MCI_ERR_NO_DEVICE, "offline context");
    if (!p->launch.hold_ext_pending) return MCI_OK;
    p->launch.hold_ext_pending = false;
    HIPCHK(hipSetDevice(p->ctx->device));
    return hold_publish_reduced(p);
}

int mci_reduce_size(const mci_problem *p, int64_t *n) {
    if (!p || !n) return fail(MCI_ERR_INVALID, "NULL argument");
    *n = p->packed_n + 64;
    return MCI_OK;
}

int mci_comm_times_ms(mci_problem *p, float *ms, int32_t n, int32_t *got) {
    if (!p || !ms || !got) return fail(MCI_ERR_INVALID, "NULL argument");
    if (p->ctx->offline) return fail(MCI_ERR_NO_DEVICE, "offline context");
    HIPCHK(hipStreamSynchronize(p->ctx->stream));
    int64_t have = p->reduces < mci_problem::kCevRing ? p->reduces : mci_problem::kCevRing;
    if (have > n) have = n;
    int32_t k = 0;
    for (int64_t i = 0; i < have; ++i) {
        const int slot = (int)((p->reduces - have + i) % mci_problem::kCevRing);
        if (!p->cev_valid[slot]) continue;
        float t = 0.f;
        HIPCHK(hipEventElapsedTime(&t, p->cevs[2 * slot], p->cevs[2 * slot + 1]));
        ms[k++] = t;
    }
    *got = k;
    return MCI_OK;
}

static int launch_train(mci_problem *p, int do_train, int do_reweight, double gamma, double *log_row) {
    const auto &s = p->shape;
    int maxn = 1;
    for (auto &L : p->leaves) maxn = L.nbin > maxn ? L.nbin : maxn;
    mci::TrainArgs a{};
    a.leaves = p->d_leaves;
    a.nleaf = s.nleaf;
    a.packed = p->d_packed;
    a.nstat = p->nstat;
    a.edges = p->d_edges;
    a.dacc = p->d_dacc;
    a.ddist = p->d_ddist;
    a.iter_log_row = log_row;
    a.reweight = p->d_reweight;
    a.goal = p->h_goal.empty() ? nullptr : p->d_goal;
    a.nd = s.ni + 1;
    a.do_reweight = do_reweight;
    a.gamma = gamma;
    a.do_train = do_train;
    if (do_train) p->ntrain += 1;
    a.serial_walk = p->train_serial >= 0 ? p->train_serial : (p->launch.last_samples == 0 || p->launch.last_samples >= mci_problem::kSerialWalkSamples) ? 1 : 0;
    if (p->debug_wrong_decision && a.serial_walk == 1) a.serial_walk = 3;
    a.status = p->d_status;
    a.maxn = maxn;
    a.spare = (size_t)(mci::train_lds_doubles(maxn) + mci::train_spare_doubles(maxn)) * sizeof(double) <= (size_t)kTrainLdsMax ? 1 : 0;
    const size_t sm = (size_t)(mci::train_lds_doubles(maxn) + (a.spare ? mci::train_spare_doubles(maxn) : maxn)) * sizeof(double);
    const unsigned tt = maxn > 256 ? 512u : 256u;
    if (sm > 64 * 1024 && !p->train_lds_raised) {
        HIPCHK(hipFuncSetAttribute((const void *)mci::k_train, hipFuncAttributeMaxDynamicSharedMemorySize, (int)kTrainLdsMax));
        HIPCHK(hipFuncSetAttribute((const void *)mci::k_finish, hipFuncAttributeMaxDynamicSharedMemorySize, (int)kTrainLdsMax));
        p->train_lds_raised = true;
    }
    if (p->merge_pending) {
        p->merge_pending = false;
        hipLaunchKernelGGL(mci::k_finish, dim3(s.nleaf + 1 + (2 * p->npa + 3) / 4), dim3(tt), sm, p->ctx->stream, p->merge, a);
    } else {
        hipLaunchKernelGGL(mci::k_train, dim3(s.nleaf + 1), dim3(tt), sm, p->ctx->stream, a);
    }
    HIPCHK(hipGetLastError());
    return MCI_OK;
}

static int grow_iteration_log(mci_problem *p, int64_t need) {
    if (need <= p->cap_iter) return MCI_OK;
    int64_t ncap = p->cap_iter ? p->cap_iter : 64;
    while (ncap < need) ncap *= 2;
    double *n = nullptr;
    HIPCHK(hipMalloc((void **)&n, (size_t)ncap * p->nstat * sizeof(double)));
    if (p->d_iterlog) {
        HIPCHK(hipMemcpyAsync(n, p->d_iterlog, (size_t)p->cap_iter * p->nstat * sizeof(double), hipMemcpyDeviceToDevice, p->ctx->stream));
        HIPCHK(hipStreamSynchronize(p->ctx->stream));
        (void)hipFree(p->d_iterlog);
    }
    p->d_iterlog = n;
    p->cap_iter = ncap;
    return MCI_OK;
}

int mci_reserve_iteration_log(mci_problem *p, int32_t rows) {
    if (!p || rows < 0) return fail(MCI_ERR_INVALID, "bad argument");
    if (p->ctx->offline) return fail(MCI_ERR_NO_DEVICE, "offline context");
    HIPCHK(hipSetDevice(p->ctx->device));
    return grow_iteration_log(p, (int64_t)p->log_row + rows);
}

int mci_iteration_finish(mci_problem *p, int32_t solver, int64_t block_total, int32_t adapt, double gamma, double *mean, double *std) {
    if (p->ctx->offline) return fail(MCI_ERR_NO_DEVICE, "offline context");
    HIPCHK(hipSetDevice(p->ctx->device));
    const auto &s = p->shape;
    if (int grc = grow_iteration_log(p, (int64_t)p->log_row + 1)) return grc;
    double *row = p->d_iterlog + (size_t)p->log_row * p->nstat;
    const bool strat = p->strat.last_run;
    int rc = launch_train(p, adapt ? 1 : 0, (solver == MCI_VEGASMC || solver == MCI_MCMC) ? 1 : 0, gamma, row);
    if (rc) return rc;
    if (strat && (rc = strat_finish(p, row, adapt))) return rc;
    p->log_row += 1;
    if (mean || std) {
        std::vector<double> h(p->nstat);
        HIPCHK(hipMemcpyAsync(h.data(), row, (size_t)p->nstat * sizeof(double), hipMemcpyDeviceToHost, p->ctx->stream));
        if ((rc = check_status(p))) return rc;
        std::vector<double> m(s.nobs), e(s.nobs);
        if (strat) strat_mean_std(h.data(), s.nobs, m.data(), e.data());
        else
        mci_mean_std(h.data(), h.data() + s.nobs, s.nobs, block_total, m.data(), e.data());
        if (mean) memcpy(mean, m.data(), s.nobs * sizeof(double));
        if (std) memcpy(std, e.data(), s.nobs * sizeof(double));
    }
    return MCI_OK;
}

int mci_train(mci_problem *p) {
    if (p->ctx->offline) return fail(MCI_ERR_NO_DEVICE, "offline context");
    int rc = flush_merge(p);
    if (rc) return rc;
    rc = launch_train(p, 1, 0, 1.0, nullptr);
    if (rc) return rc;
    return check_status(p);
}
```

mcintegration.jl_amd/csrc/mci_host_jit.h:

```cpp
enum { kSlotVegasAny = 3, kSlotDump = 4, kSlotVegasmcSpec = 5, kSlotMcmcSpec = 6 };
static int kslot(int solver, int64_t measurefreq) { return solver == MCI_VEGAS && measurefreq != 1 ? kSlotVegasAny : solver; }
static int slot_solver(int slot) { return slot == kSlotVegasAny ? MCI_VEGAS : slot == kSlotVegasmcSpec ? MCI_VEGASMC : slot == kSlotMcmcSpec ? MCI_MCMC : slot; }

namespace {
struct Candidate {
    std::string src;
    int threads = 256;
    std::vector<char> code;
    std::string log, path;
    bool cached = false;
    int rc = 0;
    long vgprs() const { return mcijit::kernel_vgprs(code, "mci_vegas_batch"); }
    long scratch() const { return mcijit::kernel_scratch_bytes(code, "mci_vegas_batch"); }
};
void compile_all(std::vector<Candidate *> &cs) {
    std::vector<std::thread> th;
    for (size_t i = 1; i < cs.size(); ++i)
        th.emplace_back([c = cs[i]] { c->rc = mcijit::compile(c->src, c->threads, c->code, c->log, c->cached, &c->path); });
    if (!cs.empty()) cs[0]->rc = mcijit::compile(cs[0]->src, cs[0]->threads, cs[0]->code, cs[0]->log, cs[0]->cached, &cs[0]->path);
    for (auto &t : th) t.join();
}
}

static int load_slot(mci_problem *p, int slot, Candidate &c, int64_t lds) {
// ... 446 lines not shown
    if (solver == MCI_VEGASMC_LANES || solver == MCI_MCMC_LANES) {
        const int sl = solver == MCI_VEGASMC_LANES ? kSlotVegasmcSpec : kSlotMcmcSpec;
        if (!p->compiled[sl]) return fail(MCI_ERR_INVALID, "the several-lanes-per-chain kernel has not been compiled yet");
        snprintf(buf, (size_t)n, "%s", p->code_object[sl].c_str());
        return MCI_OK;
    }
    if (solver == MCI_VEGAS_STRAT) {
        if (!p->strat.compiled) return fail(MCI_ERR_INVALID, "the stratified :vegas kernel has not been compiled yet");
        snprintf(buf, (size_t)n, "%s", p->strat.code_object.c_str());
        return MCI_OK;
    }
    if (solver == MCI_VEGAS_SWEEP) {
        if (!p->sweep.compiled) return fail(MCI_ERR_INVALID, "the sweep kernel has not been compiled yet");
        snprintf(buf, (size_t)n, "%s", p->sweep.code_object.c_str());
        return MCI_OK;
    }
    if (solver == MCI_VEGAS_SWEEP_LEAVES) {
        if (!p->sweep.leaves.compiled) return fail(MCI_ERR_INVALID, "the sweep kernel for several leaves has not been compiled yet");
        snprintf(buf, (size_t)n, "%s", p->sweep.leaves.code_object.c_str());
        return MCI_OK;
    }
    if (solver < 0 || solver > 2) return fail(MCI_ERR_INVALID, "Solver %d is not supported!", solver);
    const int slot = (solver == MCI_VEGAS && !p->compiled[solver] && p->compiled[kSlotVegasAny]) ? kSlotVegasAny : solver;
    if (!p->compiled[slot]) return fail(MCI_ERR_INVALID, "solver %d has not been compiled yet", solver);
    snprintf(buf, (size_t)n, "%s", p->code_object[slot].c_str());
    return MCI_OK;
}

int mci_set_rng_bits(mci_problem *p, int32_t bits) {
    if (!p) return fail(MCI_ERR_INVALID, "NULL argument");
    if (bits != 52 && bits != 32) return fail(MCI_ERR_INVALID, "rng bits must be 52 (default: the resolution of rand(Float64)) or 32");
    if (p->shape.rng_bits != bits) {
        p->shape.rng_bits = bits;
        drop_modules(p);
    }
    return MCI_OK;
}

int mci_set_rng_rounds(mci_problem *p, int32_t rounds) {
    if (!p) return fail(MCI_ERR_INVALID, "NULL argument");
    if (rounds != 10 && rounds != 7) return fail(MCI_ERR_INVALID, "Philox4x32 rounds must be 10 (default) or 7 (the fewest that pass BigCrush)");
    if (p->shape.rng_rounds != rounds) {
        p->shape.rng_rounds = rounds;
        drop_modules(p);
    }
    return MCI_OK;
}

int mci_set_train_walk(mci_problem *p, int32_t mode) {
    if (!p) return fail(MCI_ERR_INVALID, "NULL argument");
    if (mode < -1 || mode > 2) return fail(MCI_ERR_INVALID, "train walk mode must be -1 (automatic), 0 (prefix scan), 1 (serial recurrence) or 2 (serial recurrence, general form only)");
    p->train_serial = mode;
    return MCI_OK;
}

int mci_debug_plant_wrong_decision(mci_problem *p, int32_t on) {
    if (!p) return fail(MCI_ERR_INVALID, "NULL argument");
    p->debug_wrong_decision = on != 0;
    return MCI_OK;
}

int mci_debug_override(const char *key, int64_t value, int32_t on) {
    Override *o = override_slot(key);
    if (!o) return fail(MCI_ERR_INVALID, "no such override: %s", key ? key : "(null)");
    o->on = on != 0;
    o->v = value;
    return MCI_OK;
}

int mci_debug_split_chunks(const mci_problem *p, int64_t *chunks, int64_t *bytes) {
    if (!p) return fail(MCI_ERR_INVALID, "NULL argument");
    if (chunks) *chunks = p->launch.last_split_chunks;
    if (bytes) *bytes = p->launch.last_split_bytes;
    return MCI_OK;
}

int mci_debug_vegas_cursor(const mci_problem *p, int32_t *used, uint64_t *base) {
    if (!p) return fail(MCI_ERR_INVALID, "NULL argument");
    if (used) *used = p->launch.last_cursor ? 1 : 0;
    if (base) *base = p->cursor_base;
    return MCI_OK;
}

int mci_debug_compiler_id(const char *set, char *out, int32_t n) {
    if (set) mcijit::compiler_id_override() = set;
    if (out && n > 0) snprintf(out, (size_t)n, "%s", mcijit::compiler_id().c_str());
    return MCI_OK;
}

int mci_debug_mcmc_policy(int64_t pilot_steps, int64_t grow, int64_t carry_holds, int64_t carry_half_floors) {
    if (pilot_steps > 0) mci_problem::kMcmcPilotSteps = pilot_steps;
    if (grow > 0) mci_problem::kMcmcGrow = grow;
    if (carry_holds > 0) mci_problem::kMcmcCarryHolds = carry_holds;
    if (carry_half_floors > 0) mci_problem::kMcmcCarryHalfFloors = carry_half_floors;
    return MCI_OK;
}

int mci_debug_persist_spin_ticks(mci_problem *p, unsigned long long ticks) {
    if (!p || ticks == 0) return fail(MCI_ERR_INVALID, "bad argument");
    p->persist_spin_ticks = ticks;
    return MCI_OK;
}

int mci_set_deterministic(mci_problem *p, int32_t on) {
    if (!p) return fail(MCI_ERR_INVALID, "NULL argument");
    const bool want = on != 0;
    if (want != p->deterministic) {
        p->deterministic = want;
        p->shape.det = want ? 1 : 0;
        drop_modules(p);
    }
    return MCI_OK;
}

int mci_set_chain_carry(mci_problem *p, int32_t mode) {
    if (!p) return fail(MCI_ERR_INVALID, "NULL argument");
    if (mode < -1 || mode > 1) return fail(MCI_ERR_INVALID, "chain carry mode must be -1 (automatic) or 1 (many-chain launches of :vegasmc and :mcmc continue the chains of the iteration before) or 0 (every launch starts its chains afresh)");
    p->chain_carry = mode;
    if (mode == 0) p->launch.chain_valid = false;
    return MCI_OK;
}

int mci_set_iteration_counted(mci_problem *p, int32_t counted) {
    if (!p) return fail(MCI_ERR_INVALID, "NULL argument");
    p->launch_counted = counted != 0;
    return MCI_OK;
}

int mci_set_persistent(mci_problem *p, int32_t mode) {
    if (!p) return fail(MCI_ERR_INVALID, "NULL argument");
    if (mode < -1 || mode > 1) return fail(MCI_ERR_INVALID, "persistent mode must be -1 (automatic: launch-bound :vegas calls), 0 (one launch chain per iteration) or 1 (whenever the layout allows)");
    p->persistent = mode;
    return MCI_OK;
}

int mci_debug_persist_words(mci_problem *p, unsigned long long *out, int32_t n) {
    if (!p || !out || !p->d_persist) return fail(MCI_ERR_INVALID, "no persistent launch yet");
    HIPCHK(hipStreamSynchronize(p->ctx->stream));
    HIPCHK(hipMemcpy(out, p->d_persist, (size_t)(n < (int)kPersistWords ? n : (int)kPersistWords) * sizeof(unsigned long long), hipMemcpyDeviceToHost));
    return MCI_OK;
}

int mci_debug_walk_counts(mci_problem *p, int64_t *out) {
    if (!p || !out || !p->d_status) return fail(MCI_ERR_INVALID, "NULL argument");
    int h[2] = {0, 0};
    HIPCHK(hipStreamSynchronize(p->ctx->stream));
    HIPCHK(hipMemcpy(h, p->d_status + 1, sizeof(h), hipMemcpyDeviceToHost));
    out[0] = h[0];
    out[1] = h[1];
    return MCI_OK;
}

int mci_last_integrate_persistent(const mci_problem *p, int32_t *persistent) {
    if (!p || !persistent) return fail(MCI_ERR_INVALID, "NULL argument");
    *persistent = p->last_persistent ? 1 : 0;
    return MCI_OK;
}

int mci_last_chain_launch(const mci_problem *p, int64_t *nchain, int32_t *carried) {
    if (!p) return fail(MCI_ERR_INVALID, "NULL argument");
    if (nchain) *nchain = p->launch.last_nchain;
    if (carried) *carried = p->launch.last_carried ? 1 : 0;
    return MCI_OK;
}

int mci_check_status(mci_problem *p) {
// ... 58 lines not shown
```

mcintegration.jl_amd/csrc/mci_host_problem.h:

```cpp
int mci_problem_create(mci_ctx *ctx, const mci_problem_desc *d, mci_problem **out) {
    if (!ctx || !d || !out) return fail(MCI_ERR_INVALID, "NULL argument");
    if (d->nleaf < 1 || d->npool < 1 || d->nintegrand < 1) return fail(MCI_ERR_INVALID, "At least one integrand is required.");
    if (d->nintegrand > 31) return fail(MCI_ERR_INVALID, "at most 31 integrands are supported");
    mci_problem *p = new mci_problem();
    p->ctx = ctx;
    p->npool = d->npool;
    p->ni = d->nintegrand;
    const int Nd = p->ni + 1;
    p->dof.assign((size_t)Nd * p->npool, 0);
    for (int i = 0; i < p->ni * p->npool; ++i) {
        if (d->dof[i] < 0) { delete p; return fail(MCI_ERR_INVALID, "dof must be non-negative"); }
        p->dof[i] = d->dof[i];
    }
    p->maxdof.assign(p->npool, 0);
    mci_maxdof(p->dof.data(), Nd, p->npool, p->maxdof.data());
    p->pool_leaf0.assign(p->npool, -1);
    p->pool_nleaf.assign(p->npool, 0);
    auto &s = p->shape;
    int eoff = 0, aoff = 0, doff = 0, boff = 0;
    for (int l = 0; l < d->nleaf; ++l) {
        const mci_leaf_desc &ld = d->leaves[l];
        if (ld.pool < 0 || ld.pool >= p->npool) { delete p; return fail(MCI_ERR_INVALID, "leaf %d: pool out of range", l); }
        if (p->pool_leaf0[ld.pool] < 0) p->pool_leaf0[ld.pool] = l;
        else if (p->pool_leaf0[ld.pool] + p->pool_nleaf[ld.pool] != l) { delete p; return fail(MCI_ERR_INVALID, "leaves of pool %d are not contiguous", ld.pool); }
// ... 224 lines not shown
        if (s.split_all) {
            int64_t budget = (lim1 - fixed) / 8;
            for (size_t l = 0; l < p->leaves.size(); ++l) {
                const Leaf &L = p->leaves[l];
                if (L.kind != MCI_CONTINUOUS || s.ec_doubles + L.nbin + 1 > budget) continue;
                s.leaf_ecoff[l] = s.ec_doubles;
                s.ec_doubles += L.nbin + 1;
            }
        }
        p->lds_bytes_k1 = fixed + (int64_t)s.ec_doubles * 8;
        p->ntdraw = 0;
        int tdraw_maxbin = 2;
        if (s.ntile > 1)
            for (int k = 0; k < s.ndraw; ++k) {
                const Leaf &L = p->leaves[s.draw_leaf[k]];
                if (L.adapt && s.cover_mask[k] && s.leaf_tile[s.draw_leaf[k]] >= (s.split_all ? 0 : 1)) {
                    p->ntdraw += 1;
                    if (L.nbin > 65536) { delete p; return fail(MCI_ERR_INVALID, "leaf %d: more than 65536 bins with tiled histograms", s.draw_leaf[k]); }
                    if (s.leaf_nbin[s.draw_leaf[k]] > tdraw_maxbin) tdraw_maxbin = s.leaf_nbin[s.draw_leaf[k]];
                }
            }
        {
            int bits = 1;
            while ((1 << bits) < tdraw_maxbin) ++bits;
            p->tdraw_words = (p->ntdraw * bits + 31) / 32;
        }
        s.htile = 0;
        for (int v : s.tile_nbin) s.htile = v > s.htile ? v : s.htile;
        s.table_mode = mode;
        s.pair_table = pair;
        const bool hist_lds = (mode == 0 || mode == 3);
        p->lds_bytes = fixed + (mode <= 1 ? (pair ? e2 : e1) : 0) + (hist_lds ? (int64_t)s.htile * 8 : 0);
        s.hcopy = 1;
        {
            int hc = 1;
            const int64_t one = (int64_t)s.htile * 8;
            int nadd = 0;
            for (int k = 0; k < s.ndraw; ++k) nadd += (p->leaves[s.draw_leaf[k]].adapt && s.cover_mask[k]) ? 1 : 0;
            if (mode == 0 && s.ntile == 1 && p->lds_bytes <= lim0 && nadd >= 4)
                while (hc < 8 && p->lds_bytes + one * (2 * hc - 1) <= lim0) hc *= 2;
            if (g_over.hist_copies.on) {
                hc = (int)g_over.hist_copies.v;
                while (hc > 1 && (!hist_lds || s.ntile != 1 || (hc & (hc - 1)) || p->lds_bytes + one * (hc - 1) > lim1)) hc >>= 1;
                if (hc < 1) hc = 1;
            }
            s.hcopy = p->hcopy_auto = p->hcopy_rule = hc;
        }
        const int64_t hcopy_bytes = (int64_t)s.htile * 8 * (s.hcopy - 1);
        if (mode == 3 && s.ntile == 1) {
            const int64_t budget = (lim1 - p->lds_bytes - hcopy_bytes) / 8;
            for (size_t l = 0; l < p->leaves.size(); ++l) {
                const Leaf &L = p->leaves[l];
                if (L.kind != MCI_CONTINUOUS || s.ec_doubles + L.nbin + 1 > budget) continue;
                s.leaf_ecoff[l] = s.ec_doubles;
                s.ec_doubles += L.nbin + 1;
            }
            p->lds_bytes_k1 = p->lds_bytes + (int64_t)s.ec_doubles * 8;
        }
        s.l1_phase = (mode == 3 && s.split_all) ? 1 : 0;
        if (g_over.l1_phase.on) s.l1_phase = (mode >= 2 && g_over.l1_phase.v > 0) ? 1 : 0;
        if (p->lds_bytes > lim0) p->threads = 512;
        if (p->lds_bytes > lim0) {
            p->vegas_plan_a = true;
            p->threads_vegas = 1024;
        }
        if (s.hcopy > 1 && !p->vegas_plan_a) {
            p->hcopy_plan = true;
            p->threads_vegas = 512;
        }
    }
    p->nstat = 2 * s.nobs + 2 + Nd;
    p->packed_n = p->nstat + s.nbin + 2 * p->npa;
    p->h_reweight.assign(Nd, 1.0 / Nd);
    s.body = "w[0] = 1.0;";
    if (!ctx->offline) {
        HIPCHK(hipSetDevice(ctx->device));
        int rc = upload(p);
        if (rc) { delete p; return rc; }
        HIPCHK(hipMalloc((void **)&p->d_packed, (size_t)(p->packed_n + 64) * sizeof(double)));
        HIPCHK(hipMemset(p->d_packed, 0, (size_t)(p->packed_n + 64) * sizeof(double)));
        HIPCHK(hipMalloc((void **)&p->d_ghist, 3 * (size_t)(s.nbin ? s.nbin : 1) * sizeof(double)));
        HIPCHK(hipMemset(p->d_ghist, 0, 3 * (size_t)(s.nbin ? s.nbin : 1) * sizeof(double)));
        HIPCHK(hipMalloc((void **)&p->d_stage1, (size_t)mci_problem::kGroups * (s.nbin ? s.nbin : 1) * sizeof(double)));
        HIPCHK(hipMalloc((void **)&p->d_status, 4 * sizeof(int)));
        HIPCHK(hipMemset(p->d_status, 0, 4 * sizeof(int)));
        std::vector<mci::LeafDev> ld;
        for (auto &L : p->leaves) ld.push_back({L.kind, L.nbin, L.eoff, L.doff, L.boff, L.adapt, L.alpha});
        HIPCHK(hipMalloc((void **)&p->d_leaves, ld.size() * sizeof(mci::LeafDev)));
        HIPCHK(hipMemcpy(p->d_leaves, ld.data(), ld.size() * sizeof(mci::LeafDev), hipMemcpyHostToDevice));
        p->evs.resize(2 * mci_problem::kEvRing);
        for (auto &e : p->evs) HIPCHK(hipEventCreate(&e));
    }
    *out = p;
    return MCI_OK;
}

static void strat_free_buffers(mci_problem *p);
int mci_problem_destroy(mci_problem *p) {
    if (!p) return MCI_OK;
    if (!p->ctx->offline) {
        (void)hipStreamSynchronize(p->ctx->stream);
        for (void *q : {(void *)p->d_edges, (void *)p->d_dacc, (void *)p->d_ddist, (void *)p->d_reweight, (void *)p->d_ud,
                        (void *)p->d_part_cols, (void *)p->d_part_hist, (void *)p->d_ghist, (void *)p->d_stage1,
                        (void *)p->d_packed, (void *)p->d_scratch, (void *)p->d_iterlog, (void *)p->d_dump,
                        (void *)p->d_status, (void *)p->d_leaves})
            if (q) (void)hipFree(q);
        for (int k = 0; k < mci_problem::kSlots; ++k)
            if (p->module[k]) (void)hipModuleUnload(p->module[k]);
        if (p->module_persist) (void)hipModuleUnload(p->module_persist);
        if (p->strat.module) (void)hipModuleUnload(p->strat.module);
        if (p->sweep.module) (void)hipModuleUnload(p->sweep.module);
        if (p->sweep.leaves.module) (void)hipModuleUnload(p->sweep.leaves.module);
        strat_free_buffers(p);
        if (p->d_persist) (void)hipFree(p->d_persist);
    }
    persist_job_drop(p);
    if (!p->ctx->offline) {
        if (p->d_goal) (void)hipFree(p->d_goal);
        if (p->d_part_pa) (void)hipFree(p->d_part_pa);
        if (p->d_hold) (void)hipFree(p->d_hold);
        for (int b = 0; b < 2; ++b) {
            if (p->d_chain_x[b]) (void)hipFree(p->d_chain_x[b]);
            if (p->d_chain_curr[b]) (void)hipFree(p->d_chain_curr[b]);
        }
        if (p->d_reweight_used) (void)hipFree(p->d_reweight_used);
        if (p->d_carry_W) (void)hipFree(p->d_carry_W);
        if (p->d_carry_src) (void)hipFree(p->d_carry_src);
        if (p->d_spec_tab) (void)hipFree(p->d_spec_tab);
        for (int b = 0; b < 2; ++b)
            if (p->d_chain_P[b]) (void)hipFree(p->d_chain_P[b]);
        if (p->d_carry_w) (void)hipFree(p->d_carry_w);
        if (p->d_clocks) (void)hipFree(p->d_clocks);
        if (p->d_cursor) (void)hipFree(p->d_cursor);
        if (p->d_edges_backup) (void)hipFree(p->d_edges_backup);
        if (p->h_hold) (void)hipHostFree(p->h_hold);
        if (p->h_hold_d) (void)hipHostFree(p->h_hold_d);
        if (p->h_log) (void)hipHostFree(p->h_log);
        if (p->hold_ev) (void)hipEventDestroy(p->hold_ev);
        if (p->d_blocklog) (void)hipFree(p->d_blocklog);
        for (auto &e : p->cevs) (void)hipEventDestroy(e);
        if (p->d_hx) (void)hipFree(p->d_hx);
        if (p->d_hstep) (void)hipFree(p->d_hstep);
        if (p->h_hidx) (void)hipHostFree(p->h_hidx);
        if (p->d_hw) (void)hipFree(p->d_hw);
        if (p->h_hx) (void)hipHostFree(p->h_hx);
        if (p->h_hw) (void)hipHostFree(p->h_hw);
        tile_release(p);
        if (p->d_mx) (void)hipFree(p->d_mx);
        if (p->d_mrelw) (void)hipFree(p->d_mrelw);
        if (p->d_mobs) (void)hipFree(p->d_mobs);
        if (p->h_mx) (void)hipHostFree(p->h_mx);
        if (p->h_mrelw) (void)hipHostFree(p->h_mrelw);
        if (p->d_midx) (void)hipFree(p->d_midx);
        if (p->h_midx) (void)hipHostFree(p->h_midx);
        for (auto &e : p->evs) (void)hipEventDestroy(e);
    }
    delete p;
    return MCI_OK;
}

int mci_set_integrand_source(mci_problem *p, const char *body, const double *ud, int32_t nud) {
    if (!p || !body) return fail(MCI_ERR_INVALID, "NULL argument");
    p->shape.body = body;
    p->shape.host_integrand = 0;
    p->host_fn = nullptr;
    p->h_ud.assign(ud, ud + (nud > 0 ? nud : 0));
    drop_modules(p);
    if (!p->ctx->offline) {
        if (p->d_ud) (void)hipFree(p->d_ud);
        p->d_ud = nullptr;
        HIPCHK(hipMalloc((void **)&p->d_ud, (p->h_ud.size() ? p->h_ud.size() : 1) * sizeof(double)));
        if (p->h_ud.size()) HIPCHK(hipMemcpy(p->d_ud, p->h_ud.data(), p->h_ud.size() * sizeof(double), hipMemcpyHostToDevice));
    }
    return MCI_OK;
}

int mci_set_integrand_host(mci_problem *p, mci_host_integrand_fn fn, void *user) {
    if (!p || !fn) return fail(MCI_ERR_INVALID, "NULL argument");
    p->host_fn = fn;
    p->host_user = user;
    p->host_idx_fn = nullptr;
    p->shape.host_integrand = 1;
    p->shape.body = "";
    p->h_ud.clear();
    drop_modules(p);
    if (!p->ctx->offline && !p->d_ud) HIPCHK(hipMalloc((void **)&p->d_ud, sizeof(double)));
    return MCI_OK;
}

int mci_set_integrand_host_indexed(mci_problem *p, mci_host_integrand_idx_fn fn, void *user) {
    if (!p || !fn) return fail(MCI_ERR_INVALID, "NULL argument");
    p->host_idx_fn = fn;
    p->host_fn = nullptr;
    p->host_user = user;
    p->shape.host_integrand = 1;
    p->shape.body = "";
    p->h_ud.clear();
    drop_modules(p);
    if (!p->ctx->offline && !p->d_ud) HIPCHK(hipMalloc((void **)&p->d_ud, sizeof(double)));
    return MCI_OK;
}

static int eval_host_integrand(mci_problem *p, const int32_t *idx, const double *x, double *w, int64_t n) {
    const auto &s = p->shape;
    const int nw = s.ni * s.ncomp, nc = s.ncomp;
    int hrc = 0;
    if (!idx) {
        memset(w, 0, (size_t)n * nw * sizeof(double));
        if (p->host_fn) hrc = p->host_fn(x, w, n, s.ndraw, nw, p->host_user);
        else {
            std::vector<int32_t> which((size_t)n);
            for (int j = 0; j < s.ni && !hrc; ++j) {
                std::fill(which.begin(), which.end(), j);
                hrc = p->host_idx_fn(which.data(), x, w + (size_t)j * nc * n, n, s.ndraw, nc, p->host_user);
            }
        }
// ... 120 lines not shown
```

mcintegration.jl_amd/csrc/mci_host_strat.h:

```cpp
static_assert(mci::kStratMaxCols == mci::kStratReduceCols, "k_strat_reduce keeps the columns the sample kernel writes");
static int flush_merge(mci_problem *p);

static const int64_t kStratSamplesPerCube = 8;

int mci_strat_plan(int64_t neval, int32_t ndim, int64_t max_nhcube, int32_t *nstrat) {
    if (!nstrat || ndim < 1) return fail(MCI_ERR_INVALID, "stratification: ndim must be positive");
    if (max_nhcube < 1) return fail(MCI_ERR_INVALID, "stratification: max_nhcube must be positive");
    const int64_t per = neval / kStratSamplesPerCube, cap = per < max_nhcube ? per : max_nhcube;
    if (cap < 1) return fail(MCI_ERR_INVALID, "stratification: neval = %lld is too small for %lld samples per hypercube", (long long)neval,
                             (long long)kStratSamplesPerCube);
    auto power_le = [cap](int64_t v, int n) {
        int64_t r = 1;
        for (int i = 0; i < n; ++i) {
            if (r > cap / v) return cap + 1;
            r *= v;
        }
        return r;
    };
    int64_t s = (int64_t)floor(pow((double)cap, 1.0 / ndim));
    if (s < 1) s = 1;
    while (s > 1 && power_le(s, ndim) > cap) --s;
    while (power_le(s + 1, ndim) <= cap) ++s;
    int64_t ncube = power_le(s, ndim);
    for (int d = 0; d < ndim; ++d) nstrat[d] = (int32_t)s;
// ... 382 lines not shown
    if ((rc = ensure_capacity(p, nwg, 1))) return rc;
    if (nchunk > st.cap_chunk) {
        for (void *q : {(void *)st.d_part, (void *)st.d_rec_s, (void *)st.d_rec_h})
            if (q) (void)hipFree(q);
        st.d_part = st.d_rec_s = nullptr;
        st.d_rec_h = nullptr;
        st.cap_chunk = 0;
        HIPCHK(hipMalloc((void **)&st.d_part, (size_t)nchunk * 2 * NW * sizeof(double)));
        HIPCHK(hipMalloc((void **)&st.d_rec_s, (size_t)nchunk * 2 * 2 * NW * sizeof(double)));
        HIPCHK(hipMalloc((void **)&st.d_rec_h, (size_t)nchunk * 2 * sizeof(long long)));
        st.cap_chunk = nchunk;
    }
    if (!st.d_stat) HIPCHK(hipMalloc((void **)&st.d_stat, 2 * mci::kStratMaxCols * sizeof(double)));
    st.ran = true;
    st.last_nchunk = nchunk;

    mci::BatchArgs a{};
    a.edges = p->d_edges;
    a.dacc = p->d_dacc;
    a.ddist = p->d_ddist;
    a.reweight = p->d_reweight;
    a.ud = p->d_ud;
    a.part_cols = p->d_part_cols;
    a.part_hist = p->d_part_hist;
    a.ghist = p->d_ghist;
    a.seed = seed;
    a.iteration = (mci::u32)iteration;
    a.neval_per_block = nevalperblock;
    a.block_lo = block_lo;
    a.wg_per_block = (int)nwg;
    a.measurefreq = 1;
    a.nchain = 1;
    a.status = p->d_status;
    a.hist_atomic = 0;
    a.nrows = nwg;
    mci::StratArgs sa{};
    sa.off = st.d_off;
    sa.dnext = st.d_d;
    sa.part = st.d_part;
    sa.rec_h = st.d_rec_h;
    sa.rec_s = st.d_rec_s;
    sa.ncube = st.ncube;
    sa.nsamp = N;
    sa.chunk = S;
    sa.nchunk = nchunk;
    sa.first_index = block_lo * nevalperblock;
    sa.nloc = (int)(S / 2 + 1);
    sa.beta = st.beta;
    for (int d = 0; d < s.ndraw; ++d) {
        const uint32_t n = (uint32_t)st.nstrat[d];
        strat_magic(n, &sa.magic[d], &sa.shift[d]);
        sa.nstrat[d] = (int)n;
        sa.inv[d] = 1.0 / (double)n;
    }
    struct Scratch {
        void *q[5] = {nullptr, nullptr, nullptr, nullptr, nullptr};
        ~Scratch() {
            for (void *v : q)
                if (v) (void)hipFree(v);
        }
    } dump;
    const bool dumping = st.hn > 0;
    if (dumping) {
        if (st.hn != N) return fail(MCI_ERR_INVALID, "mci_debug_strat_dump: %lld samples asked for, the iteration has %lld", (long long)st.hn, (long long)N);
        HIPCHK(hipMalloc(&dump.q[0], (size_t)N * s.ndraw * sizeof(double)));
        HIPCHK(hipMalloc(&dump.q[1], (size_t)N * s.ndraw * sizeof(double)));
        HIPCHK(hipMalloc(&dump.q[2], (size_t)N * sizeof(long long)));
        HIPCHK(hipMalloc(&dump.q[3], (size_t)N * sizeof(double)));
        HIPCHK(hipMalloc(&dump.q[4], (size_t)N * NW * sizeof(double)));
        sa.dump_x = (double *)dump.q[0];
        sa.dump_y = (double *)dump.q[1];
        sa.dump_h = (long long *)dump.q[2];
        sa.dump_jac = (double *)dump.q[3];
        sa.dump_w = (double *)dump.q[4];
    }
    void *args[] = {&a, &sa};
    const int slot = (int)(p->launch.launches % mci_problem::kEvRing);
    p->launch.time_this_launch = p->kernel_timing > 0 || (p->kernel_timing < 0 && N >= ((int64_t)1 << 20));
    if (p->launch.time_this_launch) HIPCHK(hipEventRecord(p->evs[2 * slot], p->ctx->stream));
    HIPCHK(hipModuleLaunchKernel(st.f, (unsigned)nwg, 1, 1, (unsigned)T, 1, 1, (unsigned)lds, p->ctx->stream, args, nullptr));
    if (p->launch.time_this_launch) HIPCHK(hipEventRecord(p->evs[2 * slot + 1], p->ctx->stream));
    p->launch.ev_valid[slot] = p->launch.time_this_launch;
    p->launch.clock_valid[slot] = false;
    p->launch.launches += 1;
    if (dumping) {
        hipStream_t hs = p->ctx->stream;
        HIPCHK(hipMemcpyAsync(st.hx, dump.q[0], (size_t)N * s.ndraw * sizeof(double), hipMemcpyDeviceToHost, hs));
        HIPCHK(hipMemcpyAsync(st.hy, dump.q[1], (size_t)N * s.ndraw * sizeof(double), hipMemcpyDeviceToHost, hs));
        HIPCHK(hipMemcpyAsync(st.hh, dump.q[2], (size_t)N * sizeof(long long), hipMemcpyDeviceToHost, hs));
        HIPCHK(hipMemcpyAsync(st.hjac, dump.q[3], (size_t)N * sizeof(double), hipMemcpyDeviceToHost, hs));
        HIPCHK(hipMemcpyAsync(st.hw, dump.q[4], (size_t)N * NW * sizeof(double), hipMemcpyDeviceToHost, hs));
        HIPCHK(hipStreamSynchronize(hs));
        st.hn = 0;
    }
    const int nb256 = (s.nbin + 255) / 256;
    if (s.nbin > 0)
        hipLaunchKernelGGL(mci::k_hist_stage1, dim3(nb256, mci_problem::kGroups), dim3(256), 0, p->ctx->stream, p->d_part_hist, (int)nwg, s.nbin,
                           (int)mci_problem::kGroups, p->d_stage1);
    HIPCHK(hipGetLastError());
    mci::MergeArgs &m = p->merge;
    m.hist_no_offset = 0;
    m.part_cols = p->d_part_cols;
    m.ncols = s.ncols;
    m.nobs = s.nobs;
    m.ni = s.ni;
    m.nblocks = (int)mblocks;
    m.wg_per_block = (int)(nwg / mblocks);
    m.stage1 = p->d_stage1;
    m.ngroup = (int)mci_problem::kGroups;
    m.ghist = p->d_ghist;
    m.use_ghist = 0;
    m.nbin = s.nbin;
    m.packed = p->d_packed;
    m.status = p->d_status;
    m.scratch = p->d_scratch;
    m.part_pa = nullptr;
    m.npa = p->npa;
    m.nrows = (int)nwg;
    m.block_means = nullptr;
    m.hold = nullptr;
    p->merge_pending = true;
    p->launch.last_samples = N;
    p->launch.last_wg = (int)nwg;
    p->launch.last_threads = T;
    p->launch.last_nblocks = (int)mblocks;
    st.last_run = true;
    return MCI_OK;
}

static int strat_finish(mci_problem *p, double *row, int32_t adapt) {
    auto &st = p->strat;
    st.last_run = false;
    mci::StratReduceArgs r{};
    r.off = st.d_off;
    r.part = st.d_part;
    r.rec_h = st.d_rec_h;
    r.rec_s = st.d_rec_s;
    r.ncube = st.ncube;
    r.nchunk = st.last_nchunk;
    r.nw = p->shape.ni * p->shape.ncomp;
    r.beta = st.beta;
    r.dnext = st.d_d;
    r.out = st.d_stat;
    r.log_row = row;
    hipLaunchKernelGGL(mci::k_strat_reduce, dim3(1), dim3(mci::kStratReduceThreads), 0, p->ctx->stream, r);
    HIPCHK(hipGetLastError());
    st.alloc_pending = adapt != 0;
    st.c_valid = true;
    st.c_host.clear();
    if (st.c_nstrat != st.nstrat) st.c_nstrat = st.nstrat;
    st.c_ncube = st.ncube;
    st.c_beta = st.beta;
    return MCI_OK;
}

static void strat_mean_std(const double *row, int nobs, double *mean, double *std) {
    for (int o = 0; o < nobs; ++o) {
        mean[o] = row[o];
        std[o] = row[nobs + o] > 0.0 ? sqrt(row[nobs + o]) : 0.0;
    }
}
```

mcintegration.jl_amd/csrc/mci_host_types.h:

```cpp
namespace {

struct Id128 { char b[128]; };
struct Rccl {
    void *h = nullptr;
    int (*GetUniqueId)(void *) = nullptr;
    int (*CommInitRank)(void **, int, Id128 , int) = nullptr;
    int (*AllReduce)(const void *, void *, size_t, int, int, void *, hipStream_t) = nullptr;
    int (*CommDestroy)(void *) = nullptr;
    const char *(*GetErrorString)(int) = nullptr;
};
Rccl g_rccl;
const int kNcclFloat64 = 8, kNcclSum = 0;

int find_loaded_rccl(struct dl_phdr_info *info, size_t, void *out) {
    const char *n = info->dlpi_name;
    if (n && strstr(n, "librccl.so")) {
        *(std::string *)out = n;
        return 1;
    }
    return 0;
}

int rccl_load() {
    if (g_rccl.h) return MCI_OK;
// ... 95 lines not shown
    int tdraw_words = 0;
    hipFunction_t f_tiles[2] = {nullptr, nullptr};
    mci::MergeArgs merge{};
    bool merge_pending = false;
    bool has_fermik = false;
    mci_host_integrand_fn host_fn = nullptr;
    mci_host_integrand_idx_fn host_idx_fn = nullptr;
    int32_t *h_hidx = nullptr;
    int64_t cap_hidx = 0;
    std::vector<double> h_tmp;
    void *host_user = nullptr;
    double *d_hx = nullptr, *d_hw = nullptr, *h_hx = nullptr, *h_hw = nullptr;
    int64_t cap_host = 0;
    void *d_hstep = nullptr;
    int64_t cap_hstep = 0;
    mci_host_measure_fn hmeas_fn = nullptr;
    mci_host_measure_idx_fn hmeas_idx_fn = nullptr;
    void *hmeas_user = nullptr;
    double *d_mx = nullptr, *d_mrelw = nullptr, *h_mx = nullptr, *h_mrelw = nullptr, *d_mobs = nullptr;
    int32_t *d_midx = nullptr, *h_midx = nullptr;
    int64_t cap_hmeas = 0, cap_mobs = 0;
    std::vector<double> h_mtmp;
    std::vector<int32_t> h_mitmp;
    int threads = 256, wg_per_block = 0;
    bool threads_explicit = false;
    bool vegas_wide = false;
    int threads_vegas = 0;
    bool vegas_plan_a = false;
    int kernel_timing = -1;
    int hcopy_auto = 1, hcopy_rule = 1;
    bool deterministic = false;
    int threads_det[3] = {0, 0, 0};
    bool hcopy_plan = false;
    int train_serial = -1;
    bool debug_wrong_decision = false;
    static const int64_t kSerialWalkSamples = (int64_t)1 << 26;
    bool train_lds_raised = false;
    std::vector<hipEvent_t> cevs;
    bool cev_valid[64] = {};
    int64_t reduces = 0;
    static const int kCevRing = 64;
    unsigned long long *h_hold = nullptr;
    double *h_hold_d = nullptr;
    hipEvent_t hold_ev = nullptr;
    double *d_blocklog = nullptr;
    int64_t cap_blocklog = 0;
    double *d_chain_x[2] = {nullptr, nullptr};
    double *d_chain_P[2] = {nullptr, nullptr};
    double *d_carry_w = nullptr;
    int64_t cap_carry_w = 0;
    hipFunction_t f_carryw[2] = {nullptr, nullptr};
    int *d_chain_curr[2] = {nullptr, nullptr};
    int64_t chain_cap[2] = {0, 0};
    int chain_carry = -1;
    int64_t ntrain = 0;
    bool launch_counted = false;
    double *d_reweight_used = nullptr, *d_carry_W = nullptr;
    int *d_carry_src = nullptr;
    int64_t cap_carry_src = 0, cap_carry_W = 0;
    unsigned long long *d_clocks = nullptr;
    std::vector<hipEvent_t> evs;
    static const int kEvRing = 512;
    int log_row = 0;
    double *h_log = nullptr;
    size_t cap_hlog = 0;
    hipModule_t module_persist = nullptr;
    hipFunction_t f_persist = nullptr;
    bool persist_compiled = false, persist_failed = false;
    std::string persist_code_object;
    int persist_threads = 256;
    struct PersistJob;
    PersistJob *persist_job = nullptr;
    unsigned long long *d_persist = nullptr;
    double *d_edges_backup = nullptr;
    unsigned long long persist_arrive = 0, persist_done = 0;
    unsigned long long persist_spin_ticks = 200000000ull;
    int persistent = -1;
    bool last_persistent = false;
    static const int kGroups = mci::kMergeGroups;
    static const int kCursorLog2Big = 4, kCursorOnes = 4;
    unsigned long long *d_cursor = nullptr;
    int64_t cap_cursor = 0, cursor_nblocks = 0;
    unsigned long long cursor_base = 0;
    hipFunction_t cursor_occ_f = nullptr;
    int cursor_occ_threads = 0, cursor_occ_resident = 0;
    int64_t cursor_occ_lds = 0;
    static const int64_t kChainFill = 131072;
    static int64_t kMcmcPilotSteps, kMcmcGrow;
    static int64_t kMcmcCarryHolds, kMcmcCarryHalfFloors;
    struct LaunchState {
        int last_wg = 0, last_threads = 0, last_nblocks = 0;
        int64_t last_samples = 0;
        int64_t last_nchain = 0;
        int last_spec_lanes = 1, last_spec_maxacc = 0;
        bool last_carried = false;
        bool last_cursor = false;
        int64_t last_split_chunks = 0, last_split_bytes = 0;
        int64_t launches = 0;
        bool time_this_launch = true;
        bool ev_valid[kEvRing] = {};
        bool clock_valid[kEvRing] = {};
        int chain_cur = 0;
        bool chain_valid = false;
        int chain_solver = -1, chain_iteration = -1;
        int64_t chain_lo = 0, chain_hi = 0, chain_nchain = 0;
        int64_t chain_ntrain = 0;
        int64_t blk_rows = 0, blk_stride = 0, blk_lo = -1;
        int blk_carried = 0;
        int64_t hold_max = 0;
        int64_t hold_len = 0;
        int64_t hold_prev = 0;
        bool hold_valid = false;
        bool hold_measured = false;
        bool mcmc_warm = false;
        bool hold_inflight = false;
        bool hold_from_packed = false;
        bool hold_deferred = false;
        bool hold_ext_pending = false;
        int64_t hold_launches = 0;
        int64_t hold_len_inflight = 0;
        bool hold_carried_inflight = false;
    } launch;
    static_assert(std::is_trivially_copyable<LaunchState>::value, "the launch record holds values only");
    struct Strat {
        bool on = false;
        std::vector<int> want;
        double beta = 0.75;
        int64_t max_nhcube = (int64_t)1 << 24;
        std::vector<int> nstrat;
        int64_t ncube = 0, nsamp = 0;
        long long *d_off = nullptr;
        bool ran = false;
        bool alloc_valid = false;
        bool alloc_pending = false;
        double *d_d = nullptr;
        bool carry = false;
        bool c_valid = false;
        std::vector<int> c_nstrat;
        int64_t c_ncube = 0;
        double c_beta = 0.0;
        std::vector<double> c_host;
        int carry_how = 0;
        double *d_tsum = nullptr;
        int64_t cap_cube = 0;
        double *d_part = nullptr, *d_rec_s = nullptr, *d_stat = nullptr;
        long long *d_rec_h = nullptr;
        int64_t cap_chunk = 0, last_nchunk = 0;
        bool last_run = false;
        bool compiled = false;
        int compiled_det = -1;
        hipModule_t module = nullptr;
        hipFunction_t f = nullptr;
        std::string code_object;
        double *hx = nullptr, *hy = nullptr, *hjac = nullptr, *hw = nullptr;
        long long *hh = nullptr;
        int64_t hn = 0;
        double *hstart = nullptr;
        int64_t hstart_n = 0;
    } strat;
    struct Sweep {
        bool compiled = false;
        int threads = 0;
        hipModule_t module = nullptr;
        hipFunction_t f = nullptr;
        std::string code_object;
        int grid = 0;
        int want_threads = 0;
        int last_grid = 0, last_threads = 0;
        int leaves_mode = 0;
        struct Unit {
            bool compiled = false;
            int threads = 0;
            hipModule_t module = nullptr;
            hipFunction_t f = nullptr;
            std::string code_object;
        } leaves;
    } sweep;
};

static const int kRepeatStride = 16384, kMaxRepeats = 7;

int64_t mci_problem::kMcmcPilotSteps = 4096;
int64_t mci_problem::kMcmcGrow = 2;
int64_t mci_problem::kMcmcCarryHolds = 4;
int64_t mci_problem::kMcmcCarryHalfFloors = 2;

namespace {
struct Override { bool on = false; int64_t v = 0; };
struct Overrides { Override table_mode, hist_tile_bins, no_split_all, l1_phase, train_walk, hist_copies, fresh_floors, fresh_burnin_pct, spec_self_check, split_chunk, vegas_self_check, vegas_cursor, cursor_log2_big, cursor_ones; } g_over;
Override *override_slot(const char *key) {
    if (!key) return nullptr;
    if (!strcmp(key, "table_mode")) return &g_over.table_mode;
    if (!strcmp(key, "hist_tile_bins")) return &g_over.hist_tile_bins;
    if (!strcmp(key, "no_split_all")) return &g_over.no_split_all;
    if (!strcmp(key, "l1_phase")) return &g_over.l1_phase;
    if (!strcmp(key, "train_walk")) return &g_over.train_walk;
    if (!strcmp(key, "hist_copies")) return &g_over.hist_copies;
    if (!strcmp(key, "fresh_floors")) return &g_over.fresh_floors;
    if (!strcmp(key, "fresh_burnin_pct")) return &g_over.fresh_burnin_pct;
    if (!strcmp(key, "spec_self_check")) return &g_over.spec_self_check;
    if (!strcmp(key, "split_chunk")) return &g_over.split_chunk;
    if (!strcmp(key, "vegas_self_check")) return &g_over.vegas_self_check;
    if (!strcmp(key, "vegas_cursor")) return &g_over.vegas_cursor;
    if (!strcmp(key, "cursor_log2_big")) return &g_over.cursor_log2_big;
    if (!strcmp(key, "cursor_ones")) return &g_over.cursor_ones;
    return nullptr;
}
}

static void persist_job_drop(mci_problem *p);
namespace { void persist_orphans_join(); }
static const size_t kPersistWords = 8 + 3 * 8 * 8 + 16;

namespace {

int tile_alloc(mci_problem *p, size_t bytes) {
    mci_ctx *c = p->ctx;
    void *base = nullptr;
    {
        std::lock_guard<std::mutex> g(c->spare_mu);
        if (c->spare && c->spare_bytes >= bytes && c->spare_bytes <= 2 * bytes + ((size_t)64 << 20)) {
            base = c->spare;
            p->tile_bytes = c->spare_bytes;
            c->spare = nullptr;
            c->spare_bytes = 0;
        }
    }
    if (!base) {
        HIPCHK(hipMalloc(&base, bytes));
        p->tile_bytes = bytes;
    }
    p->d_tile_w = (double *)base;
    return MCI_OK;
}
void tile_release(mci_problem *p) {
    if (!p->d_tile_w) return;
    mci_ctx *c = p->ctx;
    void *drop = p->d_tile_w;
    {
        std::lock_guard<std::mutex> g(c->spare_mu);
        if (p->tile_bytes > c->spare_bytes) {
            drop = c->spare;
            c->spare = p->d_tile_w;
            c->spare_bytes = p->tile_bytes;
        }
    }
    if (drop) (void)hipFree(drop);
    p->d_tile_w = nullptr;
    p->d_tile_bins = nullptr;
    p->tile_bytes = 0;
    p->cap_tile = 0;
}

int upload(mci_problem *p) {
    if (p->ctx->offline) return MCI_OK;
    auto up = [&](double *&d, const std::vector<double> &h) -> int {
        size_t n = h.size() ? h.size() : 1;
        if (!d) HIPCHK(hipMalloc((void **)&d, n * sizeof(double)));
        if (h.size()) HIPCHK(hipMemcpyAsync(d, h.data(), h.size() * sizeof(double), hipMemcpyHostToDevice, p->ctx->stream));
        return MCI_OK;
    };
    int rc;
    if ((rc = up(p->d_edges, p->h_edges))) return rc;
    if ((rc = up(p->d_dacc, p->h_dacc))) return rc;
    if ((rc = up(p->d_ddist, p->h_ddist))) return rc;
    if ((rc = up(p->d_reweight, p->h_reweight))) return rc;
    HIPCHK(hipStreamSynchronize(p->ctx->stream));
    return MCI_OK;
}

int ensure_capacity(mci_problem *p, int64_t nwg, int64_t nblocks) {
    const auto &s = p->shape;
    if (nwg > p->cap_wg) {
        if (p->d_part_cols) (void)hipFree(p->d_part_cols);
        if (p->d_part_hist) (void)hipFree(p->d_part_hist);
        p->d_part_cols = p->d_part_hist = nullptr;
        HIPCHK(hipMalloc((void **)&p->d_part_cols, (size_t)nwg * s.ncols * sizeof(double)));
        if (s.table_mode == 0 || s.table_mode == 3) HIPCHK(hipMalloc((void **)&p->d_part_hist, (size_t)nwg * (s.nbin ? s.nbin : 1) * sizeof(double)));
        p->cap_wg = nwg;
    }
    if (nblocks > p->cap_blocks) {
        if (p->d_scratch) (void)hipFree(p->d_scratch);
        p->d_scratch = nullptr;
        HIPCHK(hipMalloc((void **)&p->d_scratch, (size_t)nblocks * s.ncols * sizeof(double)));
        p->cap_blocks = nblocks;
    }
    return MCI_OK;
}
// ... 145 lines not shown
```

mcintegration.jl_amd/csrc/mci_static_kernels.h:

```cpp
#pragma once
#include <hip/hip_runtime.h>

#include "mci_train.h"

namespace mci {

__global__ void __launch_bounds__(256) k_hist_stage1(const double *__restrict__ part_hist, int nwg, int nbin, int ngroup,
                                                     double *__restrict__ out) {
    const int bin = blockIdx.x * 256 + threadIdx.x;
    const int g = blockIdx.y;
    if (bin >= nbin) return;
    const int per = (nwg + ngroup - 1) / ngroup;
    const int w0 = g * per, w1 = min(nwg, w0 + per);
    double s0 = 0.0, s1 = 0.0, s2 = 0.0, s3 = 0.0;
    int w = w0;
    for (; w + 3 < w1; w += 4) {
        s0 += part_hist[(size_t)(w + 0) * nbin + bin];
        s1 += part_hist[(size_t)(w + 1) * nbin + bin];
        s2 += part_hist[(size_t)(w + 2) * nbin + bin];
        s3 += part_hist[(size_t)(w + 3) * nbin + bin];
    }
    for (; w < w1; ++w) s0 += part_hist[(size_t)w * nbin + bin];
    out[(size_t)g * nbin + bin] = (s0 + s1) + (s2 + s3);
}

__global__ void __launch_bounds__(256) k_add_host_obs(const double *__restrict__ obs, int nblocks, int nobs, int ncols, int wg_per_block,
                                                      double *__restrict__ part_cols) {
    const int i = blockIdx.x * 256 + threadIdx.x;
    if (i >= nblocks * nobs) return;
    const int b = i / nobs, o = i % nobs;
    part_cols[(size_t)b * wg_per_block * ncols + o] += obs[i];
}

__global__ void __launch_bounds__(256) k_finalize(MergeArgs m) {
    const int nhb = (m.nbin + 255) / 256;
    const int hoff = 2 * m.nobs + 2 + m.ni + 1;
    if ((int)blockIdx.x < nhb) {
        const int bin = blockIdx.x * 256 + threadIdx.x;
        if (bin < m.nbin) m.packed[hoff + bin] = merge_hist_bin(m, bin);
        return;
    }
    if ((int)blockIdx.x > nhb) {
        merge_pa(m, (int)blockIdx.x - nhb - 1);
        return;
    }
    merge_stats(m);
}

struct ResampleArgs {
    const int *curr_old;
    long long n_old, n_new;
    int nd;
    const double *rw_now, *rw_used;
    int *src;
    double *W;
    const double *w_chain;
};
__global__ void __launch_bounds__(256) k_resample_chains(ResampleArgs a) {
    constexpr int kLdsW = 8192;
    __shared__ double sW[kLdsW];
    __shared__ long long part[256];
    const int tid = threadIdx.x, T = 256;
    const int *co = a.curr_old + (size_t)blockIdx.x * a.n_old;
    double *W = a.W + (size_t)blockIdx.x * a.n_old;
    int *src = a.src + (size_t)blockIdx.x * a.n_new;
    const long long per = (a.n_old + T - 1) / T, j0 = tid * per < a.n_old ? tid * per : a.n_old, j1 = j0 + per < a.n_old ? j0 + per : a.n_old;
    constexpr int kNd = 16;
    if (a.w_chain) {
        __shared__ double dpart[256];
        const double *wc = a.w_chain + (size_t)blockIdx.x * a.n_old;
        double mine = 0.0;
        for (long long j = j0; j < j1; ++j) mine += wc[j];
        dpart[tid] = mine;
        __syncthreads();
        double below = 0.0;
        for (int t = 0; t < tid; ++t) below += dpart[t];
        double run = 0.0;
        for (long long j = j0; j < j1; ++j) {
            run += wc[j];
            const double v = below + run;
            W[j] = v;
            if (a.n_old <= kLdsW) sW[j] = v;
        }
    } else
    if (a.nd <= kNd) {
        long long cnt[kNd];
        double w[kNd];
#pragma unroll
        for (int i = 0; i < kNd; ++i) {
            cnt[i] = 0;
            w[i] = i < a.nd ? a.rw_now[i] / a.rw_used[i] : 0.0;
        }
        for (long long j = j0; j < j1; ++j) {
            const int c = co[j];
#pragma unroll
            for (int i = 0; i < kNd; ++i) cnt[i] += c == i ? 1 : 0;
// ... 16 lines not shown
#pragma unroll
            for (int i = 0; i < kNd; ++i) {
                cnt[i] += c == i ? 1 : 0;
                if (i < a.nd) {
                    const double term = w[i] * (double)cnt[i];
                    acc = i == 0 ? term : acc + term;
                }
            }
            W[j] = acc;
            if (a.n_old <= kLdsW) sW[j] = acc;
        }
    } else
    for (int i = 0; i < a.nd; ++i) {
        const double w = a.rw_now[i] / a.rw_used[i];
        long long mine = 0;
        for (long long j = j0; j < j1; ++j) mine += co[j] == i ? 1 : 0;
        __syncthreads();
        part[tid] = mine;
        __syncthreads();
        long long cnt = 0;
        for (int t = 0; t < tid; ++t) cnt += part[t];
        for (long long j = j0; j < j1; ++j) {
            cnt += co[j] == i ? 1 : 0;
            const double term = w * (double)cnt;
            W[j] = i == 0 ? term : W[j] + term;
        }
    }
    __threadfence_block();
    __syncthreads();
    const bool in_lds = (a.w_chain != nullptr || a.nd <= kNd) && a.n_old <= kLdsW;
    const double step = W[a.n_old - 1] / (double)a.n_new;
    if (!(W[a.n_old - 1] > 0.0)) {
        for (long long c = tid; c < a.n_new; c += T) src[c] = (int)(c % a.n_old);
        return;
    }
    for (long long c = tid; c < a.n_new; c += T) {
        const double target = ((double)c + 0.6180339887498949) * step;
        long long lo = 0, hi = a.n_old - 1;
        while (lo < hi) {
            const long long mid = (lo + hi) >> 1;
            if ((in_lds ? sW[mid] : W[mid]) > target) hi = mid;
            else lo = mid + 1;
        }
        src[c] = (int)lo;
    }
}

__global__ void __launch_bounds__(512) k_train(TrainArgs a) {
    extern __shared__ __attribute__((aligned(16))) double sm[];
    __shared__ double ps[256];
    __shared__ int bad;
    __shared__ double ssum;
    if ((int)blockIdx.x == a.nleaf) {
        iteration_bookkeeping(a);
        return;
    }
    if (!a.do_train) return;
    const LeafDev L = a.leaves[blockIdx.x];
    if (!L.adapt) return;
    double *h = a.packed + a.nstat + L.boff;
    train_leaf(L, h, h, sm, ps, bad, ssum, a.edges, a.dacc, a.ddist, a.serial_walk, a.status, false, nullptr, false, a.spare ? sm + train_lds_doubles(a.maxn) : nullptr);
}

__global__ void __launch_bounds__(512) k_finish(MergeArgs m, TrainArgs a) {
    extern __shared__ __attribute__((aligned(16))) double sm[];
    __shared__ double ps[256];
    __shared__ int bad;
    __shared__ double ssum;
    const int tid = threadIdx.x, T = blockDim.x;
    if ((int)blockIdx.x == a.nleaf) {
        merge_stats(m);
        __syncthreads();
        iteration_bookkeeping(a);
        return;
    }
    if ((int)blockIdx.x > a.nleaf) {
        merge_pa(m, (int)blockIdx.x - a.nleaf - 1);
        return;
    }
    const LeafDev L = a.leaves[blockIdx.x];
    double *hl = sm + train_lds_doubles(a.maxn);
    double *hp = a.packed + a.nstat + L.boff;
    const bool train = a.do_train && L.adapt;
    if (train) train_stage_grid(L, sm, a.edges);
    for (int i = tid; i < L.nbin; i += T) {
        const double v = merge_hist_bin(m, L.boff + i);
        hl[i] = v;
        hp[i] = v;
    }
    __syncthreads();
    if (!train) return;
    train_leaf(L, hl, hp, sm, ps, bad, ssum, a.edges, a.dacc, a.ddist, a.serial_walk, a.status, true, nullptr, false, a.spare ? hl : nullptr);
}

struct StratAllocArgs {
    const double *d;
    long long *off;
    double *tsum;
    long long ncube, nsamp;
    int ntile;
    int uniform;
};
__device__ inline void strat_stretch(const StratAllocArgs &a, long long &lo, long long &hi) {
    const long long tl = (a.ncube + a.ntile - 1) / a.ntile, t0 = (long long)blockIdx.x * tl, t1 = t0 + tl < a.ncube ? t0 + tl : a.ncube;
    const long long per = (t1 - t0 + 255) / 256;
    lo = t0 + (long long)threadIdx.x * per;
    if (lo > t1) lo = t1;
    hi = lo + per < t1 ? lo + per : t1;
}
__global__ void __launch_bounds__(256) k_strat_alloc(StratAllocArgs a, int phase) {
    __shared__ double part[256];
    const int tid = threadIdx.x;
    const long long M = a.nsamp - 2 * a.ncube;
    if (phase == 1) {
        if (tid != 0) return;
        double base = 0.0;
        for (int g = 0; g < a.ntile; ++g) {
            a.tsum[a.ntile + g] = base;
            base += a.tsum[g];
        }
        a.tsum[2 * a.ntile] = base;
        a.tsum[2 * a.ntile + 1] = (a.uniform || !(base > 0.0) || !isfinite(base)) ? 1.0 : 0.0;
        return;
    }
    long long lo, hi;
    strat_stretch(a, lo, hi);
    double mine = 0.0;
    if (!(phase == 2 && a.tsum[2 * a.ntile + 1] != 0.0))
        for (long long h = lo; h < hi; ++h) mine += a.d[h];
    part[tid] = mine;
    __syncthreads();
    if (phase == 0) {
        if (tid == 0) {
            double s = 0.0;
            for (int t = 0; t < 256; ++t) s += part[t];
            a.tsum[blockIdx.x] = s;
        }
        return;
    }
    if (blockIdx.x == 0 && tid == 0) a.off[0] = 0;
    if (a.tsum[2 * a.ntile + 1] != 0.0) {
        for (long long h = lo; h < hi; ++h) {
            double C = (double)M * (double)(h + 1) / (double)a.ncube;
            if (h == a.ncube - 1 || C > (double)M) C = (double)M;
            a.off[h + 1] = 2 * (h + 1) + (long long)floor(C);
        }
        return;
    }
    double sbase = 0.0;
    for (int t = 0; t < tid; ++t) sbase += part[t];
    const double tbase = a.tsum[a.ntile + blockIdx.x], total = a.tsum[2 * a.ntile];
    double run = 0.0;
    for (long long h = lo; h < hi; ++h) {
        run += a.d[h];
        double C = (double)M * (tbase + (sbase + run)) / total;
        if (h == a.ncube - 1 || C > (double)M) C = (double)M;
        a.off[h + 1] = 2 * (h + 1) + (long long)floor(C);
    }
}

__host__ __device__ inline int strat_remap_cell(int j, int n_old, int n_new) {
    return (int)(((2ull * (unsigned long long)j + 1ull) * (unsigned long long)n_old) / (2ull * (unsigned long long)n_new));
}
__host__ __device__ inline long long strat_remap_index(const int *j, const int *n_old, const int *n_new, int ndim) {
    long long h = 0, stride = 1;
    for (int d = 0; d < ndim; ++d) {
        h += (long long)strat_remap_cell(j[d], n_old[d], n_new[d]) * stride;
        stride *= n_old[d];
    }
    return h;
}
enum { kStratRemapMaxDraw = 32 };
struct StratRemapArgs {
    const double *d_old;
    double *d_new;
// ... 89 lines not shown
```

mcintegration.jl_amd/csrc/mci_train.h:

```cpp
#pragma once
#include "mci_device.h"

namespace mci {


struct LeafDev {
    int kind;
    int nbin;
    int eoff;
    int doff;
    int boff;
    int adapt;
    double alpha;
};


enum { kMergeGroups = 32 };

struct MergeArgs {
    const double *part_cols;
    int ncols, nobs, ni, nblocks, wg_per_block;
    const double *stage1;
    int ngroup;
    double *ghist;
// ... 116 lines not shown
    const int per = (n + T - 1) / T, b = tid * per, e = min(n, b + per);
    double loc = 0.0;
    for (int k = b; k < e; ++k) loc += v[k];
    const double x = wave_scan_incl(loc);
    __syncthreads();
    if (lane == 63) ps[wave] = x;
    __syncthreads();
    double base = 0.0;
    for (int w = 0; w < wave; ++w) base += ps[w];
    (void)nwave;
    double run = base + (x - loc);
    for (int k = b; k < e; ++k) {
        run += v[k];
        out[k] = run;
    }
    __syncthreads();
    return out[n - 1];
}

enum { kWalkPad = 64 };
__host__ __device__ inline int train_lds_doubles(int n) { return (n + kWalkPad) + (n + 2) + (n + kWalkPad) + 2; }
__host__ __device__ inline int train_spare_doubles(int n) { return 2 * (2 * n + kWalkPad) + (2 * n + kWalkPad) / 16 + 2; }

__device__ inline double sum16(const double *v, int n) {
    double s = 0.0;
    int i = threadIdx.x & 15;
    for (; i + 496 < n; i += 512) {
        double t[32];
#pragma unroll
        for (int k = 0; k < 32; ++k) t[k] = v[i + 16 * k];
#pragma unroll
        for (int k = 0; k < 32; ++k) s += t[k];
    }
    for (; i + 112 < n; i += 128) {
        double t[8];
#pragma unroll
        for (int k = 0; k < 8; ++k) t[k] = v[i + 16 * k];
#pragma unroll
        for (int k = 0; k < 8; ++k) s += t[k];
    }
    for (; i < n; i += 16) s += v[i];
    s += dpp_read<0x108, 0xf>(s);
    s += dpp_read<0x104, 0xf>(s);
    s += dpp_read<0x102, 0xf>(s);
    s += dpp_read<0x101, 0xf>(s);
    return __shfl(s, 0, 16);
}

#ifdef MCI_TRAIN_SHORT_SUMS
template <int DEPTH = 3> __device__ inline double sum_julia(const double *v, int n) { return sum16(v, n); }
#else
template <int DEPTH = 3> __device__ inline double sum_julia(const double *v, int n) {
    if constexpr (DEPTH == 0) return sum16(v, n);
    else {
        if (n <= 1024) return sum16(v, n);
        const int h = ((n - 1) >> 1) + 1;
        return sum_julia<DEPTH - 1>(v, h) + sum_julia<DEPTH - 1>(v + h, n - h);
    }
}
#endif

__device__ inline double rescale_pow(double b, double alpha) {
    if (alpha == 2.0) return b * b;
    if (alpha == 1.0) return b;
    if (alpha == 3.0) return b * b * b;
    return pow(b, alpha);
}

struct TrainArgs {
    const LeafDev *leaves;
    int nleaf;
    double *packed;
    int nstat;
    double *edges, *dacc, *ddist;
    double *iter_log_row;
    double *reweight;
    const double *goal;
    int nd, do_reweight;
    double gamma;
    int do_train, serial_walk;
    int *status;
    int maxn;
    int spare;
};

#ifndef MCI_TRAIN_SCAN_ONLY
#define MCI_WALK_BIN(K, OFF, DN)                                                                                                       \
    "ds_write_b64 %4, %0 offset:" OFF "\n\tv_cmp_ge_f64 vcc, %0, %3\n\tv_add_f64 %1, %0, -%3\n\tv_cmp_ge_f64_e64 %2, %1, %3\n\t"          \
    "v_add_f64 %0, %0, " DN "\n\ts_cbranch_vccz .Lwd" K "_%=\n\tv_add_f64 %0, %1, " DN "\n\ts_cmp_lg_u64 %2, 0\n\t"                      \
    "s_cbranch_scc1 .Lwr" K "_%=\n.Lwd" K "_%=:\n\t"
#define MCI_WALK_MORE(K, DN)                                                                                                           \
    ".Lwr" K "_%=:\n\tv_add_f64 %1, %1, -%3\n\tv_cmp_ge_f64 vcc, %1, %3\n\ts_cbranch_vccnz .Lwr" K "_%=\n\tv_add_f64 %0, %1, " DN "\n\t"   \
    "s_branch .Lwd" K "_%=\n\t"
__device__ __forceinline__ void walk_bins16(double &acc, const double (&v)[16], const double vnext, const double f, const unsigned rec_addr) {
    double a1;
    unsigned long long c2;
    asm volatile(
                 MCI_WALK_BIN("0", "0", "%6")
                 MCI_WALK_BIN("1", "8", "%7")
                 MCI_WALK_BIN("2", "16", "%8")
                 MCI_WALK_BIN("3", "24", "%9")
                 MCI_WALK_BIN("4", "32", "%10")
                 MCI_WALK_BIN("5", "40", "%11")
                 MCI_WALK_BIN("6", "48", "%12")
                 MCI_WALK_BIN("7", "56", "%13")
                 MCI_WALK_BIN("8", "64", "%14")
                 MCI_WALK_BIN("9", "72", "%15")
                 MCI_WALK_BIN("10", "80", "%16")
                 MCI_WALK_BIN("11", "88", "%17")
                 MCI_WALK_BIN("12", "96", "%18")
                 MCI_WALK_BIN("13", "104", "%19")
                 MCI_WALK_BIN("14", "112", "%20")
                 MCI_WALK_BIN("15", "120", "%21")
                 "s_branch .Lwend_%=\n\t"
                 MCI_WALK_MORE("0", "%6")
                 MCI_WALK_MORE("1", "%7")
                 MCI_WALK_MORE("2", "%8")
                 MCI_WALK_MORE("3", "%9")
                 MCI_WALK_MORE("4", "%10")
                 MCI_WALK_MORE("5", "%11")
                 MCI_WALK_MORE("6", "%12")
                 MCI_WALK_MORE("7", "%13")
                 MCI_WALK_MORE("8", "%14")
                 MCI_WALK_MORE("9", "%15")
                 MCI_WALK_MORE("10", "%16")
                 MCI_WALK_MORE("11", "%17")
                 MCI_WALK_MORE("12", "%18")
                 MCI_WALK_MORE("13", "%19")
                 MCI_WALK_MORE("14", "%20")
                 MCI_WALK_MORE("15", "%21")
                 ".Lwend_%=:"
                 : "+v"(acc), "=&v"(a1), "=&s"(c2)
                 : "v"(f), "v"(rec_addr), "v"(v[0]), "v"(v[1]), "v"(v[2]), "v"(v[3]), "v"(v[4]), "v"(v[5]), "v"(v[6]), "v"(v[7]), "v"(v[8]),
                   "v"(v[9]), "v"(v[10]), "v"(v[11]), "v"(v[12]), "v"(v[13]), "v"(v[14]), "v"(v[15]), "v"(vnext)
                 : "vcc", "scc", "memory");
}

#undef MCI_WALK_BIN
#undef MCI_WALK_MORE

template <bool RECORD> __device__ __forceinline__ void walk_slots16(double &acc, const double (&e)[16], double *__restrict__ rec) {
    if (!RECORD) rec[0] = acc;
#pragma unroll
    for (int k = 0; k < 16; ++k) {
        if (RECORD) rec[k] = acc;
        acc = acc + e[k];
    }
}

__device__ __forceinline__ void walk_trip(double &acc, const double (&v)[16], const double vnext, const double f, const unsigned rec_addr) {
    walk_bins16(acc, v, vnext, f, rec_addr);
}
#endif

enum { kTrainQ = 4 };

__device__ inline void train_stage_grid(const LeafDev &L, double *sm, const double *__restrict__ edges) {
    if (L.kind != 0) return;
    const int tid = threadIdx.x, T = blockDim.x, N = L.nbin;
    double *d = sm, *sg = sm + N + kWalkPad;
    const double *g = edges + L.eoff;
    for (int base = 0; base <= N; base += kTrainQ * T) {
        double v[kTrainQ];
#pragma unroll
        for (int q = 0; q < kTrainQ; ++q) {
            const int i = base + q * T + tid;
            v[q] = i <= N ? g[i] : 0.0;
        }
#pragma unroll
        for (int q = 0; q < kTrainQ; ++q) {
            const int i = base + q * T + tid;
            if (i <= N) sg[i] = v[q];
        }
    }
    if (tid < kWalkPad) d[N + tid] = 0.0;
}

__device__ inline void train_leaf(const LeafDev &L, const double *h, double *hclear, double *sm, double *ps, int &bad, double &ssum,
                                  double *__restrict__ edges, double *__restrict__ dacc, double *__restrict__ ddist, int serial_walk,
                                  int *__restrict__ status, bool staged = false, unsigned long long *tt = nullptr, bool checked = false,
                                  double *spare = nullptr) {
#ifdef MCI_PERSIST_TRACE
#define MCI_TT(k) if (tt && threadIdx.x == 0) tt[k] = wall_clock64();
#else
#define MCI_TT(k)
    (void)tt;
#endif
    const int tid = threadIdx.x, T = blockDim.x;
    const int N = L.nbin;
    double *d = sm;
    double *sg = sm + N + kWalkPad;
    double *wa = sg + N + 2;
    MCI_TT(0)
    if (!checked) {
        if (tid == 0) bad = 0;
        __syncthreads();
        for (int i = tid; i < N; i += T) {
            const double v = h[i];
            if (!isfinite(v)) atomicOr(&bad, ST_HIST_NONFINITE);
            else if (!(v > 0.0)) atomicOr(&bad, ST_HIST_NONPOSITIVE);
        }
        __syncthreads();
    }
    if (bad) {
        if (tid == 0) atomicOr(status, bad);
        return;
    }
    if (L.kind == 0) {
        double *g = edges + L.eoff;
        MCI_TT(1)
        if (!staged) train_stage_grid(L, sm, edges);
        double mine = 0.0;
        for (int i = tid; i < N; i += T) {
            double v;
            if (N <= 1) v = h[i];
            else if (i == 0) v = (h[0] * 7.0 + h[1]) / 8.0;
            else if (i == N - 1) v = (h[N - 1] * 7.0 + h[N - 2]) / 8.0;
            else v = (h[i - 1] + h[i] * 6.0 + h[i + 1]) / 8.0;
            d[i] = v;
            mine += v;
        }
        if (!serial_walk) {
            const double w = wave_sum(mine);
            if ((tid & 63) == 0) ps[32 + (tid >> 6)] = w;
        }
        __syncthreads();
        MCI_TT(2)
        if (N > 1) {
            double s;
            if (serial_walk) {
                s = sum_julia(d, N);
                __syncthreads();
            } else {
                s = 0.0;
                for (int w = 0; w < (T >> 6); ++w) s += ps[32 + w];
            }
            MCI_TT(3)
            int anybad = 0;
            auto rescale_q = [&](auto power, auto QC) {
                constexpr int Q = decltype(QC)::value;
                for (int base = 0; base < N; base += Q * T) {
                    double v[Q];
#pragma unroll
                    for (int q = 0; q < Q; ++q) {
                        const int i = base + q * T + tid;
                        v[q] = i < N ? d[i] / s : 1.0;
                    }
#pragma unroll
                    for (int q = 0; q < Q; ++q) {
                        const double r = power(-(1 - v[q]) / log(v[q]));
                        v[q] = (v[q] > 0 && v[q] <= 0.99999999) ? r : v[q];
                    }
#pragma unroll
                    for (int q = 0; q < Q; ++q) {
                        const int i = base + q * T + tid;
                        if (!isfinite(v[q])) anybad = 1;
                        if (i < N) d[i] = v[q];
                    }
                }
            };
            auto rescale_bins = [&](auto power) {
#ifdef MCI_TRAIN_SCAN_ONLY
                rescale_q(power, IC<(MCI_THREADS >= 512 ? 2 : kTrainQ)>{});
#else
                if (2 * T >= N) rescale_q(power, IC<2>{});
                else rescale_q(power, IC<kTrainQ>{});
#endif
            };
            const double alpha = L.alpha;
#if defined(MCI_TRAIN_POWER) && MCI_TRAIN_POWER == 2
// ... 43 lines not shown
                        lo[q] += wa[lo[q]] < target[q] ? 1 : 0;
                        lo[q] = lo[q] > N - 1 ? N - 1 : lo[q];
                    }
                    double vnew[Q];
#pragma unroll
                    for (int q = 0; q < Q; ++q) {
                        const int i = base + q * T + tid, j = lo[q];
                        const double acc_f = wa[j] - target[q];
                        const double v = sg[j + 1] - (acc_f / d[j]) * (sg[j + 1] - sg[j]);
                        vnew[q] = (i == 0 || i >= N) ? sg[i < N ? 0 : N] : v;
                    }
#pragma unroll
                    for (int q = 0; q < Q; ++q) {
                        const int i = base + q * T + tid;
                        if (i <= N) g[i] = vnew[q];
                    }
                }
            };
#ifdef MCI_TRAIN_SCAN_ONLY
            place_points(IC<(MCI_THREADS >= 512 ? 2 : kTrainQ)>{});
#else
            if (2 * T > N) place_points(IC<2>{});
            else place_points(IC<kTrainQ>{});
#endif
            __syncthreads();
            MCI_TT(6)
            if (hclear)
                for (int i = tid; i < N; i += T) hclear[i] = 1.0e-10;
            MCI_TT(7)
            return;
        }
#ifndef MCI_TRAIN_SCAN_ONLY
        const double f_ninc = sum_julia(d, N) / (double)N;
        if (!(f_ninc > 0.0 && isfinite(f_ninc))) {
            if (tid == 0) atomicOr(status, ST_RESCALE_NONFINITE);
            return;
        }
        int *flag = (int *)(ps + 64);
        int *pw = (int *)ps;
        const int lane = tid & 63, wave = tid >> 6;
        const int per = (N + T - 1) / T, b = min(N, tid * per), e = min(N, b + per);
        bool given = spare != nullptr && serial_walk != 2 && N > 1;
        double *es = spare, *rs = spare + 2 * N + kWalkPad, *heads = rs + 2 * N + kWalkPad;
        const double f_inv = 1.0 / f_ninc, f_lo = 0.5 * f_ninc, f_hi = 2.0 * f_ninc;
        auto points = [&](int j) {
            if (j >= N - 1) return 0;
            const double c = floor(wa[j] * f_inv) - (j > 0 ? floor(wa[j - 1] * f_inv) : 0.0);
            if (serial_walk == 3 && j == N / 2) return c > 0.0 ? (int)c + 1 : 1;
            return c > 0.0 ? (int)c : 0;
        };
        auto slots = [&](int j, int c) { return c + ((c >= 1 && d[j + 1] >= f_lo && d[j + 1] <= f_hi) ? 0 : 1); };
        int sbase = 0, nslot = 0;
        if (given) {
            if (tid == 0) *flag = 0;
            block_prefix(d, wa, N, ps);
            int mine = 0;
            for (int j = b; j < e; ++j) mine += slots(j, points(j));
            int x = mine;
#pragma unroll
            for (int off = 1; off < 64; off <<= 1) {
                const int y = __shfl_up(x, off, 64);
                if (lane >= off) x += y;
            }
            if (lane == 63) pw[wave] = x;
            __syncthreads();
            for (int w = 0; w < (T >> 6); ++w) {
                if (w < wave) sbase += pw[w];
                nslot += pw[w];
            }
            sbase += x - mine;
            int sl = sbase;
            for (int j = b; j < e; ++j) {
                const int c = points(j);
                for (int k = 0; k < c - 1; ++k) es[sl++] = -f_ninc;
                if (c >= 1 && slots(j, c) == c) es[sl++] = d[j + 1] - f_ninc;
                else {
                    if (c >= 1) es[sl++] = -f_ninc;
                    es[sl++] = d[j + 1];
                }
            }
            for (int k = nslot + tid; k < nslot + kWalkPad; k += T) es[k] = 0.0;
            __syncthreads();
        }
        int cnt;
        for (;;) {
            if (tid == 0) {
                double va[16], vb[16];
                double acc_f = 0.0 + d[0];
                if (given) {
#pragma unroll
                    for (int k = 0; k < 16; ++k) va[k] = es[k];
                    for (int sb = 0; sb < nslot; sb += 32) {
#pragma unroll
                        for (int k = 0; k < 16; ++k) vb[k] = es[sb + 16 + k];
                        walk_slots16<false>(acc_f, va, heads + (sb >> 4));
#pragma unroll
                        for (int k = 0; k < 16; ++k) va[k] = es[sb + 32 + k];
                        walk_slots16<false>(acc_f, vb, heads + (sb >> 4) + 1);
                    }
                } else {
                    const unsigned rec = (unsigned)(size_t)wa;
#pragma unroll
                    for (int k = 0; k < 16; ++k) va[k] = d[k];
                    for (int jb = 0; jb < N; jb += 32) {
#pragma unroll
                        for (int k = 0; k < 16; ++k) vb[k] = d[jb + 16 + k];
                        walk_trip(acc_f, va, vb[0], f_ninc, rec + 8u * (unsigned)jb);
#pragma unroll
                        for (int k = 0; k < 16; ++k) va[k] = d[jb + 32 + k];
                        walk_trip(acc_f, vb, va[0], f_ninc, rec + 8u * (unsigned)(jb + 16));
                    }
                }
            }
            __syncthreads();
            if (given) {
                for (int t = tid; t * 16 < nslot; t += T) {
                    double ev[16];
#pragma unroll
                    for (int k = 0; k < 16; ++k) ev[k] = es[t * 16 + k];
                    double acc_f = heads[t];
                    walk_slots16<true>(acc_f, ev, rs + t * 16);
                }
                __syncthreads();
            }
            cnt = 0;
            int wrong = 0, sl = sbase;
            for (int j = b; j < e; ++j) {
                int c = 0;
                for (double a = given ? rs[sl] : wa[j]; a >= f_ninc; a -= f_ninc) c += 1;
                cnt += c;
                if (given) {
                    const int cp = points(j);
                    wrong |= (j < N - 1 && c != cp) ? 1 : 0;
                    sl += slots(j, cp);
                }
            }
            if (!given) break;
            if (wrong) atomicOr(flag, 1);
            __syncthreads();
            if (*flag == 0) break;
            given = false;
        }
        if (tid == 0) atomicAdd(status + (given ? 1 : 2), 1);
        {
            int x = cnt;
#pragma unroll
            for (int off = 1; off < 64; off <<= 1) {
                const int y = __shfl_up(x, off, 64);
                if (lane >= off) x += y;
            }
            if (lane == 63) pw[wave] = x;
            __syncthreads();
            int base = 0, total = 0;
            for (int w = 0; w < (T >> 6); ++w) {
                if (w < wave) base += pw[w];
                total += pw[w];
            }
            int i = 1 + base + x - cnt;
            int sl = sbase;
            for (int j = b; j < e; ++j) {
                for (double a = given ? rs[sl] : wa[j]; a >= f_ninc;) {
                    a -= f_ninc;
                    if (i < N) g[i] = sg[j + 1] - (a / d[j]) * (sg[j + 1] - sg[j]);
                    i += 1;
                }
                if (given) sl += slots(j, points(j));
            }
            for (int k = 1 + total + tid; k < N; k += T) g[k] = sg[N];
            if (tid == 0) {
                g[0] = sg[0];
                g[N] = sg[N];
            }
        }
#endif
    }
#ifndef MCI_TRAIN_CONTINUOUS_ONLY
    else {
        double *acc = dacc + L.eoff, *dist = ddist + L.doff;
        const double s = N > 1 ? sum_julia(h, N) : 1.0;
        if (tid == 0) {
            int lbad = 0;
            if (N > 1) {
                for (int i = 0; i < N; ++i) {
                    double v = h[i] / s;
                    if (v > 0 && v <= 0.99999999) v = rescale_pow(-(1 - v) / log(v), L.alpha);
                    if (!isfinite(v)) lbad = ST_RESCALE_NONFINITE;
                    d[i] = v;
                }
            } else {
                d[0] = h[0];
            }
            if (lbad) {
                atomicOr(status, lbad);
            } else {
                double s = 0.0;
                for (int i = 0; i < N; ++i) s += d[i];
                double run = 0.0;
                acc[0] = 0.0;
                for (int i = 0; i < N; ++i) {
                    const double v = d[i] / s;
                    dist[i] = v;
                    run += v;
                    acc[i + 1] = run;
                }
            }
        }
    }
#endif
    __syncthreads();
    if (hclear)
        for (int i = tid; i < N; i += T) hclear[i] = 1.0e-10;
#undef MCI_TT
}

__device__ inline void iteration_bookkeeping(const TrainArgs &a) {
    const int tid = threadIdx.x, T = blockDim.x;
    double *row = a.iter_log_row;
    if (row)
        for (int i = tid; i < a.nstat; i += T) row[i] = a.packed[i];
#ifndef MCI_TRAIN_CONTINUOUS_ONLY
    if (a.do_reweight && tid == 0) do_reweight_dev(a.reweight, a.packed + (a.nstat - a.nd), a.nd, a.gamma, a.goal);
#endif
}

struct PersistArgs {
    MergeArgs m;
    TrainArgs t;
    int niter;
    int map_off;
    u64 *ctr;
    u64 arrive0, done0;
    u64 spin_ticks;
};

enum : u64 { kPersistDoneShift = 40, kPersistArriveMask = (1ull << 40) - 1 };
__device__ __forceinline__ bool persist_wait(const PersistArgs &f, u64 t0, u64 t1, int *verdict) {
    if (threadIdx.x == 0) {
        int ok = 1;
        const u64 start = wall_clock64();
        unsigned n = 0;
        for (;;) {
            const u64 w = __hip_atomic_load(&f.ctr[0], __ATOMIC_RELAXED, __HIP_MEMORY_SCOPE_AGENT);
            if ((w & kPersistArriveMask) >= t0 && (long long)(((w >> kPersistDoneShift) - t1) << kPersistDoneShift) >= 0) break;
            __builtin_amdgcn_s_sleep(1);
            if (((++n & 255u) == 0u || f.spin_ticks < 256ull) &&
                (__hip_atomic_load(&f.ctr[2], __ATOMIC_RELAXED, __HIP_MEMORY_SCOPE_AGENT) != 0ull || wall_clock64() - start > f.spin_ticks)) {
                ok = 0;
                break;
            }
        }
        if (!ok) {
            __hip_atomic_store(&f.ctr[2], 1ull, __ATOMIC_RELAXED, __HIP_MEMORY_SCOPE_AGENT);
            atomicOr(f.m.status, ST_PERSIST_STALL);
        }
        __builtin_amdgcn_fence(__ATOMIC_ACQUIRE, "agent");
        *verdict = ok;
    }
    __syncthreads();
    return *verdict != 0;
}
__device__ __forceinline__ void persist_signal(u64 *ctr, u64 inc) {
    __builtin_amdgcn_s_waitcnt(0x0F70);
    __syncthreads();
    if (threadIdx.x == 0) {
        __builtin_amdgcn_fence(__ATOMIC_RELEASE, "agent");
        __hip_atomic_fetch_add(ctr, inc, __ATOMIC_RELAXED, __HIP_MEMORY_SCOPE_AGENT);
    }
}

template <class Cfg> __device__ __forceinline__ void vegas_persist(const BatchArgs &a0, const PersistArgs &f) {
    static_assert(Cfg::NLEAF == 1 && Cfg::leaf_kind(0) == 0, "the persistent kernel refines ONE Continuous grid (the host checks)");
    extern __shared__ __attribute__((aligned(16))) double smem[];
    const int tid = threadIdx.x, T = blockDim.x;
    constexpr int N = Cfg::leaf_nbin(0);
    double *sm = smem, *hl = sm + train_lds_doubles(N), *ps = hl + N, *gcur = smem + f.map_off, *flags = gcur + N + 2;
    int *verdict = reinterpret_cast<int *>(flags + 2);
    const u64 G = gridDim.x - 1;
    const int wg = (int)blockIdx.x;
    const size_t rows = (size_t)G * f.m.ncols;
#ifdef MCI_PERSIST_TRACE
#define MCI_PT(k)                                                                                                                      \
    if (tid == 0 && it < 8 && (wg == 0 || wg == (int)G - 1 || wg == (int)G)) {                                                          \
        f.ctr[8 + ((wg == 0 ? 0 : wg == (int)G ? 1 : 2) * 8 + it) * 8 + (k)] = wall_clock64();                                          \
        if (wg == 0 && (k) == 0 && (it == 0 || it == 7)) f.ctr[8 + 3 * 8 * 8 + 8 + (it == 0 ? 0 : 1)] = clock64();   \
    }
#else
#define MCI_PT(k)
#endif
    const LeafDev L = f.t.leaves[0];
    const bool train = f.t.do_train && L.adapt;
    if (wg == (int)G) {
        for (int it = 0; it < f.niter; ++it) {
            MCI_PT(0)
            if (!persist_wait(f, f.arrive0 + (u64)(it + 1) * G, f.done0 + (u64)it, verdict)) return;
// ... 90 lines not shown
```

mcintegration.jl_amd/engine.py:

```python
import atexit
import ctypes as C
import weakref

import numpy as np

from . import _lib
from ._lib import LeafDesc, ProblemDesc, c_double_p, c_int32_p, check, lib
from .integrand import HostIntegrand, HostMeasure, Integrand, Measure
from .variables import ContinuousVar, FermiK

_ctx_cache = {}


def _dp(a):
    return a.ctypes.data_as(c_double_p)


def context(device=0):
    if device not in _ctx_cache:
        p = C.c_void_p()
        check(lib().mci_ctx_create(device, C.byref(p)))
        _ctx_cache[device] = p
    return _ctx_cache[device]

# ... 475 lines not shown

    def set_deterministic(self, on=True):
        check(lib().mci_set_deterministic(self.p, 1 if on else 0))

    def set_chain_carry(self, mode):
        check(lib().mci_set_chain_carry(self.p, {"auto": -1, "off": 0, "on": 1, -1: -1, 0: 0, 1: 1}[mode]))

    def set_iteration_counted(self, counted):
        check(lib().mci_set_iteration_counted(self.p, 1 if counted else 0))

    def set_persistent(self, mode):
        check(lib().mci_set_persistent(self.p, {"auto": -1, "off": 0, "on": 1, -1: -1, 0: 0, 1: 1}[mode]))

    def last_integrate_persistent(self):
        v = C.c_int32()
        check(lib().mci_last_integrate_persistent(self.p, C.byref(v)))
        return bool(v.value)

    def last_chain_launch(self):
        n, c = C.c_int64(), C.c_int32()
        check(lib().mci_last_chain_launch(self.p, C.byref(n), C.byref(c)))
        return int(n.value), bool(c.value)

    def set_chain_speculation(self, lanes=-1, accept=0.0, max_accepts=-1):
        check(lib().mci_set_chain_speculation(self.p, int(lanes), float(accept), int(max_accepts)))

    def last_chain_speculation(self):
        g, m = C.c_int32(), C.c_int32()
        check(lib().mci_last_chain_speculation(self.p, C.byref(g), C.byref(m)))
        return int(g.value), int(m.value)

    def chain_speculation_status(self, solver):
        st = C.c_int32()
        check(lib().mci_chain_speculation_status(self.p, _lib.SOLVERS[solver], C.byref(st)))
        return int(st.value)

    def vegas_check_status(self):
        st, fl = C.c_int32(), C.c_int32()
        check(lib().mci_vegas_check_status(self.p, C.byref(st), C.byref(fl)))
        return int(st.value), int(fl.value)

    def vegas_check_launches(self):
        n = C.c_int64()
        check(lib().mci_debug_vegas_check_launches(self.p, C.byref(n)))
        return int(n.value)

    def vegas_check_reference(self, nevalperblock, block_lo, nblocks, iteration=0, seed=1234, measurefreq=1, x=None, jac=None, w=None):
        packed = np.zeros(self.packed_size)
        bad = (C.c_int64 * 2)()
        ptr = [None, None, None]
        if x is not None:
            keep = [np.ascontiguousarray(v, dtype=np.float64) for v in (x, jac, w)]
            ptr = [v.ctypes.data_as(_lib.c_double_p) for v in keep]
        check(lib().mci_debug_vegas_check(self.p, int(iteration), int(seed), int(nevalperblock), int(block_lo), int(nblocks), int(measurefreq),
                                          ptr[0], ptr[1], ptr[2], packed.ctypes.data_as(_lib.c_double_p), bad))
        return packed, (int(bad[0]), int(bad[1]))

    def vegas_check_layout(self):
        head = (C.c_int32 * 8)()
        check(lib().mci_debug_vegas_check_layout(self.p, head, None, None, None, None))
        nd, ni = int(head[0]), int(head[1])
        draws, scales = (C.c_int32 * (6 * max(nd, 1)))(), (C.c_double * max(nd, 1))()
        own, obs = (C.c_uint64 * max(ni, 1))(), (C.c_int32 * (3 * max(ni, 1)))()
        check(lib().mci_debug_vegas_check_layout(self.p, head, draws, scales, own, obs))
        keys = ("kind", "off", "doff", "nbin", "boff", "hist")
        return dict(ndraw=nd, ni=ni, ncomp=int(head[2]), nobs=int(head[3]), ncols=int(head[4]), nbin=int(head[5]), covered=bool(head[6]),
                    with_obs=bool(head[7]),
                    draws=[dict(zip(keys, [int(draws[6 * k + j]) for j in range(6)]), scale=float(scales[k])) for k in range(nd)],
                    integrands=[dict(own=int(own[i]), obs_off=int(obs[3 * i]), obs_nbin=int(obs[3 * i + 1]), obs_bin_draw=int(obs[3 * i + 2]))
                                for i in range(ni)])

    def compile_chain_speculation(self, solver):
        check(lib().mci_compile_chain_speculation(self.p, _lib.SOLVERS[solver]))

    def set_train_walk(self, mode):
        check(lib().mci_debug_plant_wrong_decision(self.p, 1 if mode in ("serial_wrong_decision", 3) else 0))
        check(lib().mci_set_train_walk(self.p, {"auto": -1, "scan": 0, "serial": 1, "serial_general": 2, "serial_wrong_decision": 1, -1: -1, 0: 0, 1: 1, 2: 2, 3: 1}[mode]))

    def walk_counts(self):
        out = (C.c_int64 * 2)()
        check(lib().mci_debug_walk_counts(self.p, out))
        return int(out[0]), int(out[1])

    def last_launch_cursor(self):
        used, base = C.c_int32(0), C.c_uint64(0)
        check(lib().mci_debug_vegas_cursor(self.p, C.byref(used), C.byref(base)))
        return bool(used.value), int(base.value)

    def split_chunks(self):
        n, b = C.c_int64(), C.c_int64()
        check(lib().mci_debug_split_chunks(self.p, C.byref(n), C.byref(b)))
        return int(n.value), int(b.value)

    def integrate(self, solver, neval, niter=10, block=16, ignore=-1, adapt=True, gamma=1.0, measurefreq=1, seed=1234,
                  nchain=0, first_iteration=0, thermal_ratio=0.1, reweight_goal=None):
        goal = None
        if reweight_goal is not None:
            self._goal = np.ascontiguousarray(reweight_goal, dtype=np.float64)
            goal = _dp(self._goal)
        a = _lib.IntegrateArgs(_lib.SOLVERS[solver], int(neval), int(niter), int(block), int(ignore), 1 if adapt else 0,
                               float(gamma), int(measurefreq), int(seed), int(nchain), int(first_iteration),
                               float(thermal_ratio), goal)
        n = self.nobs
        im, ie = np.zeros((niter, n)), np.zeros((niter, n))
        m, s, c2 = np.zeros(n), np.zeros(n), np.zeros(n)
        vis = np.zeros(self.config.N + 1)
        r = _lib.ResultC(niter, n, _dp(im), _dp(ie), _dp(m), _dp(s), _dp(c2), 0, 0.0, _dp(vis), 0, 0)
        check(lib().mci_integrate(self.p, C.byref(a), C.byref(r)))
        dn, dl = C.c_int64(), C.c_int32()
        check(lib().mci_last_integrate_discarded(self.p, C.byref(dn), C.byref(dl)))
        out = dict(mean=m, stdev=s, chi2=c2, iter_mean=im, iter_std=ie, neval=r.neval, seconds=r.seconds, visited=vis,
                   correlated=bool(r.correlated), block_mean=None, warmup=int(r.warmup), neval_discarded=int(dn.value))
        if _lib.SOLVERS[solver] != _lib.VEGAS and out["correlated"]:
            out["block_mean"] = self.block_means(niter)[0]
        return out

    def _integrate_args(self, solver, neval, niter, block, ignore, adapt, gamma, measurefreq, seed, first_iteration):
        return _lib.IntegrateArgs(_lib.SOLVERS[solver], int(neval), int(niter), int(block), int(ignore), 1 if adapt else 0, float(gamma),
                                  int(measurefreq), int(seed), 0, int(first_iteration), 0.1, None)

    def sweep_supported(self, solver="vegas", neval=10000, niter=10, block=16, measurefreq=1, **kw):
        a = self._integrate_args(solver, neval, niter, block, -1, True, 1.0, measurefreq, 0, 0)
        why = C.create_string_buffer(512)
        if lib().mci_sweep_supported(self.p, C.byref(a), why, len(why)) == _lib.MCI_OK:
            return None
        return why.value.decode() or lib().mci_last_error().decode(errors="replace")

    SWEEP_MAX_POINTS = 65536

    def set_sweep_leaves(self, mode="one"):
        if mode not in ("one", "all"):
            raise ValueError('set_sweep_leaves: "one" or "all", got %r' % (mode,))
        check(lib().mci_set_sweep_leaves(self.p, 1 if mode == "all" else 0))

    def sweep_map_doubles(self):
        n = C.c_int32()
        check(lib().mci_sweep_map_doubles(self.p, C.byref(n)))
        return int(n.value)

    def _split_sweep_map(self, row):
        out, o = [], 0
        for lf in self.config.leaves:
            if hasattr(lf, "ninc"):
                out.append(row[o:o + lf.ninc])
                o += lf.ninc
            else:
                n = lf.upper - lf.lower + 1
                out.append(row[o + n + 1:o + 2 * n + 1])
                o += 2 * n + 1
        return out

    def integrate_sweep(self, solver="vegas", userdata=None, neval=10000, niter=10, block=16, ignore=-1, adapt=True, gamma=1.0, measurefreq=1,
                        seed=1234, seeds=None, maps=None, first_iteration=0):
        nud = len(self.integrand.userdata) if hasattr(self.integrand, "userdata") else 0
        ud = np.ascontiguousarray(userdata if userdata is not None else np.zeros((0, nud)), dtype=np.float64)
        if ud.ndim != 2 or ud.shape[1] != nud:
            raise ValueError("integrate_sweep: userdata must be a 2-D array [points][%d] (one row of the integrand's userdata per point), got shape %s"
                             % (nud, ud.shape))
        P = ud.shape[0]
        if not 1 <= P <= self.SWEEP_MAX_POINTS:
            raise ValueError("integrate_sweep: %d points; a sweep takes 1 to %d" % (P, self.SWEEP_MAX_POINTS))
        sd = None
        if seeds is not None:
            sd = np.ascontiguousarray(seeds, dtype=np.uint64)
            if sd.shape != (P,):
                raise ValueError("integrate_sweep: seeds must hold one seed per point (%d), got shape %s" % (P, sd.shape))
# ... 213 lines not shown
```

Measured before the change: 77020.

## Fuse histogram stage-1 reduction into vegas kernel via last-arriver groups

Each vegas workgroup now bumps a per-group arrival counter after flushing its partial histogram. The last workgroup to arrive in a group sums that group's rows into stage1_out, which removes the separate k_hist_stage1 kernel launch on the default non-atomic path. Launch timing is also reworked to use in-kernel realtime stamps instead of hip events when self-timed, and train tracing stamps are added. This adds an atomic counter, a release/acquire fence and a serial tail reduction in one workgroup per group.

After: 76090. 0.988x the previous value.

```diff
diff --git a/mcintegration.jl_amd/_lib.py b/mcintegration.jl_amd/_lib.py
--- a/mcintegration.jl_amd/_lib.py
+++ b/mcintegration.jl_amd/_lib.py
@@ -160,6 +160,10 @@
     ("mci_debug_compiler_id", C.c_int, [C.c_char_p, C.c_char_p, C.c_int32]),
     ("mci_debug_split_chunks", C.c_int, [_VP, C.POINTER(C.c_int64), C.POINTER(C.c_int64)]),
     ("mci_debug_vegas_cursor", C.c_int, [_VP, C.POINTER(C.c_int32), C.POINTER(C.c_uint64)]),
+    ("mci_debug_stage1_fused", C.c_int, [_VP, C.POINTER(C.c_int32), C.POINTER(C.c_uint64)]),
+    ("mci_debug_stage1", C.c_int, [_VP, C.c_int32, c_double_p, C.c_int64]),
+    ("mci_debug_kernel_timing", C.c_int, [_VP, c_double_p, c_double_p, C.c_int32, c_int32_p]),
+    ("mci_debug_finish_trace", C.c_int, [_VP, C.c_int32, C.POINTER(C.c_uint64)]),
     ("mci_debug_strat_d", C.c_int, [_VP, c_double_p, C.c_int64]),
     ("mci_debug_strat_start_d", C.c_int, [_VP, c_double_p, C.c_int64]),
     ("mci_debug_strat_dump", C.c_int, [_VP, C.c_int64, c_double_p, c_double_p, C.POINTER(C.c_int64), c_double_p, c_double_p]),
diff --git a/mcintegration.jl_amd/csrc/mci_debug.h b/mcintegration.jl_amd/csrc/mci_debug.h
--- a/mcintegration.jl_amd/csrc/mci_debug.h
+++ b/mcintegration.jl_amd/csrc/mci_debug.h
@@ -14,6 +14,10 @@
 int mci_debug_strat_d(mci_problem *prob, double *d, int64_t n);
 int mci_debug_strat_start_d(mci_problem *prob, double *d, int64_t n);
 int mci_debug_vegas_cursor(const mci_problem *prob, int32_t *used, uint64_t *base);
+int mci_debug_stage1_fused(const mci_problem *prob, int32_t *used, uint64_t *base);
+int mci_debug_stage1(mci_problem *prob, int32_t recompute, double *out, int64_t n);
+int mci_debug_kernel_timing(mci_problem *prob, double *ms_stamp, double *ms_event, int32_t n, int32_t *got);
+int mci_debug_finish_trace(mci_problem *prob, int32_t on, unsigned long long *out);
 int mci_debug_compiler_id(const char *set, char *out, int32_t n);
 int mci_debug_mcmc_policy(int64_t pilot_steps, int64_t grow, int64_t carry_holds, int64_t carry_half_floors);
 int mci_debug_vegas_check(mci_problem *prob, int32_t iteration, uint64_t seed, int64_t nevalperblock, int64_t block_lo, int64_t nblocks,
diff --git a/mcintegration.jl_amd/csrc/mci_device.h b/mcintegration.jl_amd/csrc/mci_device.h
--- a/mcintegration.jl_amd/csrc/mci_device.h
+++ b/mcintegration.jl_amd/csrc/mci_device.h
@@ -193,6 +193,10 @@
     int spec_ntree, spec_first;
     float spec_accept[8];
     u64 *clock_out;
+    double *stage1_out;
+    u64 *stage1_arrive;
+    u64 stage1_base;
+    int stage1_groups;
     u64 *cursor;
     u64 cursor_base;
     u32 cursor_log2_big, cursor_ones;
@@ -965,6 +969,18 @@
     u0 = e + z < r.units ? r.units - e - z : 0ull;
 }
 
+__host__ __device__ inline int stage1_per(int nwg, int ngroup) { return (nwg + ngroup - 1) / ngroup; }
+__host__ __device__ inline void stage1_rows(int nwg, int ngroup, int g, int &w0, int &w1) {
+    const int per = stage1_per(nwg, ngroup);
+    w0 = g * per;
+    w1 = w0 + per < nwg ? w0 + per : nwg;
+}
+__host__ __device__ inline int stage1_group(int nwg, int ngroup, int w) { return w / stage1_per(nwg, ngroup); }
+__host__ __device__ inline bool stage1_all_groups(int nwg, int ngroup) { return nwg >= 1 && (ngroup - 1) * stage1_per(nwg, ngroup) < nwg; }
+__host__ __device__ inline bool stage1_completes(unsigned long long ticket, unsigned long long base, int rows) { return ticket - base + 1ull == (unsigned long long)rows; }
+__host__ __device__ inline unsigned long long stage1_deficit(int nwg, int ngroup, int rows) { return (unsigned long long)(stage1_per(nwg, ngroup) - rows); }
+__host__ __device__ inline unsigned long long stage1_advance(int nwg, int ngroup) { return (unsigned long long)stage1_per(nwg, ngroup); }
+
 struct WorkItem {
     i64 rowid, lb;
     int slice, tile;
@@ -983,6 +999,48 @@
     return w;
 }
 
+template <class Cfg> __device__ __forceinline__ void stage1_fused(const BatchArgs &a, double *smem, int row) {
+    const int tid = threadIdx.x, T = blockDim.x;
+    const int nwg = (int)a.nrows, g = stage1_group(nwg, a.stage1_groups, row);
+    int w0, w1;
+    stage1_rows(nwg, a.stage1_groups, g, w0, w1);
+    u64 *const word = a.stage1_arrive + (size_t)g * kCursorStride;
+    u64 *const seen = reinterpret_cast<u64 *>(smem);
+    __builtin_amdgcn_fence(__ATOMIC_RELEASE, "agent");
+    __syncthreads();
+    if (tid == 0) *seen = __hip_atomic_fetch_add(word, 1ull, __ATOMIC_RELAXED, __HIP_MEMORY_SCOPE_AGENT);
+    __syncthreads();
+    if (!stage1_completes(*seen, a.stage1_base, w1 - w0)) return;
+    __builtin_amdgcn_fence(__ATOMIC_ACQUIRE, "agent");
+    auto rd = [&](int w, int bin) { return __hip_atomic_load(&a.part_hist[(size_t)w * Cfg::NBIN + bin], __ATOMIC_RELAXED, __HIP_MEMORY_SCOPE_AGENT); };
+    for (int bin = tid; bin < Cfg::NBIN; bin += T) {
+        double s0 = 0.0, s1 = 0.0, s2 = 0.0, s3 = 0.0;
+        int w = w0;
+        for (; w + 15 < w1; w += 16) {
+            double v[16];
+            static_for<0, 16>([&](auto K) { v[decltype(K)::value] = rd(w + decltype(K)::value, bin); });
+            static_for<0, 4>([&](auto Q) {
+                s0 += v[4 * decltype(Q)::value + 0];
+                s1 += v[4 * decltype(Q)::value + 1];
+                s2 += v[4 * decltype(Q)::value + 2];
+                s3 += v[4 * decltype(Q)::value + 3];
+            });
+        }
+        for (; w + 3 < w1; w += 4) {
+            const double v0 = rd(w + 0, bin), v1 = rd(w + 1, bin), v2 = rd(w + 2, bin), v3 = rd(w + 3, bin);
+            s0 += v0;
+            s1 += v1;
+            s2 += v2;
+            s3 += v3;
+        }
+        for (; w < w1; ++w) s0 += rd(w, bin);
+        a.stage1_out[(size_t)g * Cfg::NBIN + bin] = (s0 + s1) + (s2 + s3);
+    }
+    if (tid == 0 && stage1_deficit(nwg, a.stage1_groups, w1 - w0) != 0ull)
+        __hip_atomic_fetch_add(word, stage1_deficit(nwg, a.stage1_groups, w1 - w0), __ATOMIC_RELAXED, __HIP_MEMORY_SCOPE_AGENT);
+    __syncthreads();
+}
+
 template <class Cfg, bool SPLIT = false> __device__ __forceinline__ void vegas_batch(const BatchArgs &a) {
     extern __shared__ __attribute__((aligned(16))) double smem[];
     const int tid = threadIdx.x, T = blockDim.x;
@@ -991,6 +1049,10 @@
     using L = typename SelectType<NOHIST, LdsEC<Cfg>, Lds<Cfg>>::type;
     double *sE = smem + L::E, *sDA = smem + L::DA, *sDD = smem + L::DD;
     double *sH = smem + L::H, *sO = smem + L::O;
+    if (!SPLIT && Cfg::NTILE == 1 && a.clock_out != nullptr && blockIdx.x == 0 && tid < 64) {
+        const u64 rt = __builtin_amdgcn_s_memrealtime();
+        if (tid == 0) a.clock_out[2] = rt;
+    }
     stage_tables<Cfg>(a.edges, a.dacc, a.ddist, sE, sDA, sDD);
 #ifndef MCI_ZERO_B128
 #define MCI_ZERO_B128 0
@@ -1225,6 +1287,15 @@
     }
     __syncthreads();
     flush_workgroup<Cfg, L, !NOHIST>(a, smem, acc, extra, wi.rowid, tile);
+    if constexpr (!SPLIT && Cfg::NTILE == 1) {
+        if constexpr (Mode<Cfg>::HIST_LDS) {
+            if (a.stage1_out != nullptr) stage1_fused<Cfg>(a, smem, (int)wi.rowid);
+        }
+        if (a.clock_out != nullptr && tid < 64) {
+            const u64 rt = __builtin_amdgcn_s_memrealtime();
+            if (tid == 0) __hip_atomic_fetch_max(&a.clock_out[3], rt, __ATOMIC_RELAXED, __HIP_MEMORY_SCOPE_AGENT);
+        }
+    }
 }
 
 #ifndef MCI_THREADS
diff --git a/mcintegration.jl_amd/csrc/mci_host_access.h b/mcintegration.jl_amd/csrc/mci_host_access.h
--- a/mcintegration.jl_amd/csrc/mci_host_access.h
+++ b/mcintegration.jl_amd/csrc/mci_host_access.h
@@ -323,28 +323,71 @@
 
 int mci_set_kernel_timing(mci_problem *p, int32_t mode) {
     if (!p) return fail(MCI_ERR_INVALID, "NULL argument");
-    p->kernel_timing = mode < 0 ? -1 : mode > 0 ? 1 : 0;
-    return MCI_OK;
-}
-
-int mci_kernel_times_ms(mci_problem *p, float *ms, int32_t n, int32_t *got, int32_t *wg, int32_t *threads) {
-    if (p->ctx->offline) return fail(MCI_ERR_NO_DEVICE, "offline context");
+    p->kernel_timing = mode < 0 ? -1 : mode > 2 ? 1 : mode;
+    return MCI_OK;
+}
+
+static int kernel_times(mci_problem *p, double *ms_stamp, double *ms_event, int32_t n, int32_t *got) {
+    HIPCHK(hipSetDevice(p->ctx->device));
     HIPCHK(hipStreamSynchronize(p->ctx->stream));
     int64_t have = p->launch.launches < mci_problem::kEvRing ? p->launch.launches : mci_problem::kEvRing;
     if (have > n) have = n;
-    int64_t k = 0;
+    std::vector<unsigned long long> h;
+    int khz = 0;
+    if (ms_stamp && p->d_clocks) {
+        HIPCHK(hipDeviceGetAttribute(&khz, hipDeviceAttributeWallClockRate, p->ctx->device));
+        h.resize((size_t)4 * mci_problem::kEvRing);
+        HIPCHK(hipMemcpyAsync(h.data(), p->d_clocks, h.size() * sizeof(unsigned long long), hipMemcpyDeviceToHost, p->ctx->stream));
+        HIPCHK(hipStreamSynchronize(p->ctx->stream));
+    }
+    int32_t k = 0;
     for (int64_t i = 0; i < have; ++i) {
         const int slot = (int)((p->launch.launches - have + i) % mci_problem::kEvRing);
         if (!p->launch.ev_valid[slot]) continue;
-        float t = 0.f;
-        HIPCHK(hipEventElapsedTime(&t, p->evs[2 * slot], p->evs[2 * slot + 1]));
-        ms[k++] = t;
-    }
-    have = k;
+        const double nan = std::nan("");
+        if (ms_stamp) {
+            ms_stamp[k] = nan;
+            if (p->launch.self_timed[slot] && !h.empty() && khz > 0) {
+                const unsigned long long t0 = h[(size_t)4 * slot + 2], t1 = h[(size_t)4 * slot + 3];
+                ms_stamp[k] = t1 >= t0 ? (double)(t1 - t0) / (double)khz : nan;
+            }
+        }
+        if (ms_event) {
+            ms_event[k] = nan;
+            if (p->launch.ev_recorded[slot]) {
+                float t = 0.f;
+                HIPCHK(hipEventElapsedTime(&t, p->evs[2 * slot], p->evs[2 * slot + 1]));
+                ms_event[k] = (double)t;
+            }
+        }
+        ++k;
+    }
+    *got = k;
+    return MCI_OK;
+}
+
+int mci_kernel_times_ms(mci_problem *p, float *ms, int32_t n, int32_t *got, int32_t *wg, int32_t *threads) {
+    if (p->ctx->offline) return fail(MCI_ERR_NO_DEVICE, "offline context");
+    int64_t have = 0;
+    if (n > 0) {
+        std::vector<double> st((size_t)n), ev((size_t)n);
+        int32_t k = 0;
+        int rc = kernel_times(p, st.data(), ev.data(), n, &k);
+        if (rc) return rc;
+        for (int32_t i = 0; i < k; ++i) ms[i] = (float)(std::isnan(st[i]) ? ev[i] : st[i]);
+        have = k;
+    } else HIPCHK(hipStreamSynchronize(p->ctx->stream));
     if (got) *got = (int32_t)have;
     if (wg) *wg = p->launch.last_wg;
     if (threads) *threads = p->launch.last_threads;
     return MCI_OK;
+}
+
+int mci_debug_kernel_timing(mci_problem *p, double *ms_stamp, double *ms_event, int32_t n, int32_t *got) {
+    if (!p || !got || n < 0) return fail(MCI_ERR_INVALID, "NULL argument");
+    if (p->ctx->offline) return fail(MCI_ERR_NO_DEVICE, "offline context");
+    *got = 0;
+    return n > 0 ? kernel_times(p, ms_stamp, ms_event, n, got) : MCI_OK;
 }
 
 int mci_kernel_clocks(mci_problem *p, double *mhz, int32_t n, int32_t *got) {
@@ -355,7 +398,7 @@
     HIPCHK(hipSetDevice(p->ctx->device));
     int khz = 0;
     HIPCHK(hipDeviceGetAttribute(&khz, hipDeviceAttributeWallClockRate, p->ctx->device));
-    std::vector<unsigned long long> h((size_t)2 * mci_problem::kEvRing);
+    std::vector<unsigned long long> h((size_t)4 * mci_problem::kEvRing);
     HIPCHK(hipMemcpyAsync(h.data(), p->d_clocks, h.size() * sizeof(unsigned long long), hipMemcpyDeviceToHost, p->ctx->stream));
     HIPCHK(hipStreamSynchronize(p->ctx->stream));
     int64_t have = p->launch.launches < mci_problem::kEvRing ? p->launch.launches : mci_problem::kEvRing;
@@ -363,8 +406,8 @@
     int32_t k = 0;
     for (int64_t i = 0; i < have; ++i) {
         const int slot = (int)((p->launch.launches - have + i) % mci_problem::kEvRing);
-        if (!p->launch.ev_valid[slot] || !p->launch.clock_valid[slot] || !h[(size_t)2 * slot + 1]) continue;
-        mhz[k++] = (double)h[(size_t)2 * slot] / (double)h[(size_t)2 * slot + 1] * (double)khz * 1.0e-3;
+        if (!p->launch.ev_valid[slot] || !p->launch.clock_valid[slot] || !h[(size_t)4 * slot + 1]) continue;
+        mhz[k++] = (double)h[(size_t)4 * slot] / (double)h[(size_t)4 * slot + 1] * (double)khz * 1.0e-3;
     }
     *got = k;
     return MCI_OK;
diff --git a/mcintegration.jl_amd/csrc/mci_host_iteration.h b/mcintegration.jl_amd/csrc/mci_host_iteration.h
--- a/mcintegration.jl_amd/csrc/mci_host_iteration.h
+++ b/mcintegration.jl_amd/csrc/mci_host_iteration.h
@@ -141,7 +141,8 @@
     const bool split = solver == MCI_VEGAS && s.ntile > 1;
     if (!split && wpb * s.ntile > 4096 / nblocks && s.ntile > 1) wpb = (int)(4096 / nblocks / s.ntile) > 0 ? (int)(4096 / nblocks / s.ntile) : 1;
     const int64_t nrows = nblocks * wpb;
-    const bool atomic_flush = solver == MCI_VEGAS && hist_lds && s.ntile == 1 && atomic_rows_ok(p) && nrows <= kAtomicRows && !s.host_integrand;
+    const bool atomic_flush = solver == MCI_VEGAS && hist_lds && s.ntile == 1 && atomic_rows_ok(p) && nrows <= kAtomicRows && !s.host_integrand &&
+                              !g_over.stage1_fused.on;
     const int64_t nwg = split ? nrows : nrows * s.ntile;
     if ((rc = ensure_capacity(p, nrows, nblocks))) return rc;
     if (solver != MCI_VEGAS && nrows > p->cap_pa) {
@@ -472,6 +473,19 @@
         p->cursor_base += mci::cursor_tickets(r) + r.waves;
     }
     p->launch.last_cursor = cursor;
+    bool stage1_fused = false;
+    if (solver == MCI_VEGAS && G == 1 && hist_lds && s.nbin > 0 && !atomic_flush && !split && s.ntile == 1 && !p->in_self_check && !p->deterministic &&
+        !s.host_integrand && !s.host_measure && nrows < ((int64_t)1 << 30) && mci::stage1_all_groups((int)nrows, (int)mci_problem::kGroups) &&
+        !(g_over.stage1_fused.on && g_over.stage1_fused.v == 0)) {
+        stage1_fused = true;
+        a.stage1_out = p->d_stage1;
+        a.stage1_arrive = p->d_stage1_arrive;
+        a.stage1_base = p->stage1_base;
+        a.stage1_groups = (int)mci_problem::kGroups;
+        p->stage1_base += mci::stage1_advance((int)nrows, (int)mci_problem::kGroups);
+    }
+    p->launch.last_stage1_fused = stage1_fused;
+    p->launch.last_hist_rows = (hist_lds && s.nbin > 0 && !atomic_flush) ? hist_rows : 0;
     void *args[] = {&a};
     hipFunction_t f = p->f_solver[G > 1 ? (solver == MCI_VEGASMC ? kSlotVegasmcSpec : kSlotMcmcSpec) : kern];
     hipStream_t st = p->ctx->stream;
@@ -479,12 +493,14 @@
     p->launch.time_this_launch = p->kernel_timing > 0 || (p->kernel_timing < 0 && nblocks * nevalperblock >= ((int64_t)1 << 20));
     if (p->launch.time_this_launch && solver == MCI_VEGAS) {
         if (!p->d_clocks) {
-            HIPCHK(hipMalloc((void **)&p->d_clocks, (size_t)2 * mci_problem::kEvRing * sizeof(unsigned long long)));
-            HIPCHK(hipMemsetAsync(p->d_clocks, 0, (size_t)2 * mci_problem::kEvRing * sizeof(unsigned long long), st));
-        }
-        a.clock_out = p->d_clocks + 2 * slot;
-    }
-    if (p->launch.time_this_launch) HIPCHK(hipEventRecord(p->evs[2 * slot], st));
+            HIPCHK(hipMalloc((void **)&p->d_clocks, (size_t)4 * mci_problem::kEvRing * sizeof(unsigned long long)));
+            HIPCHK(hipMemsetAsync(p->d_clocks, 0, (size_t)4 * mci_problem::kEvRing * sizeof(unsigned long long), st));
+        }
+        a.clock_out = p->d_clocks + 4 * slot;
+    }
+    const bool self_timed = a.clock_out != nullptr && G == 1 && !split && s.ntile == 1 && !s.host_integrand && !s.host_measure;
+    const bool record_events = p->launch.time_this_launch && (!self_timed || p->kernel_timing == 2);
+    if (record_events) HIPCHK(hipEventRecord(p->evs[2 * slot], st));
     if (solver != MCI_VEGAS && s.host_integrand) {
         const int64_t nc = nblocks * nchain, steps = nevalperblock / nchain;
         const int nw = s.ni * s.ncomp, nd = s.ndraw;
@@ -571,9 +587,11 @@
     if (a.hold_hist && auto_chains && (rc = hold_publish(p, nevalperblock / nchain, solver != MCI_VEGAS && p->launch.last_carried))) return rc;
     if (split)
         HIPCHK(hipModuleLaunchKernel(p->f_tiles[kern == kSlotVegasAny ? 1 : 0], (unsigned)(((hist_rows + 7) / 8) * 8 * (s.ntile - (s.split_all ? 0 : 1))), 1, 1, (unsigned)T, 1, 1, (unsigned)p->lds_bytes, st, args, nullptr));
-    if (p->launch.time_this_launch) HIPCHK(hipEventRecord(p->evs[2 * slot + 1], st));
+    if (record_events) HIPCHK(hipEventRecord(p->evs[2 * slot + 1], st));
     p->launch.ev_valid[slot] = p->launch.time_this_launch;
     p->launch.clock_valid[slot] = a.clock_out != nullptr && !split && s.ntile == 1;
+    p->launch.self_timed[slot] = self_timed;
+    p->launch.ev_recorded[slot] = record_events;
     p->launch.launches += 1;
     if (s.host_measure) {
         const int64_t n = nblocks * hm_n;
@@ -644,7 +662,7 @@
     p->launch.last_nblocks = (int)nblocks;
     if (solver != MCI_VEGAS) p->launch.last_nchain = nchain;
     const int nb256 = (s.nbin + 255) / 256;
-    if (hist_lds && s.nbin > 0 && !atomic_flush)
+    if (hist_lds && s.nbin > 0 && !atomic_flush && !stage1_fused)
         hipLaunchKernelGGL(mci::k_hist_stage1, dim3(nb256, mci_problem::kGroups), dim3(256), 0, st, p->d_part_hist, (int)hist_rows, s.nbin,
                            (int)mci_problem::kGroups, p->d_stage1);
     HIPCHK(hipGetLastError());
@@ -785,6 +803,7 @@
     a.serial_walk = p->train_serial >= 0 ? p->train_serial : (p->launch.last_samples == 0 || p->launch.last_samples >= mci_problem::kSerialWalkSamples) ? 1 : 0;
     if (p->debug_wrong_decision && a.serial_walk == 1) a.serial_walk = 3;
     a.status = p->d_status;
+    a.trace = p->finish_trace ? p->d_finish_trace : nullptr;
     a.maxn = maxn;
     a.spare = (size_t)(mci::train_lds_doubles(maxn) + mci::train_spare_doubles(maxn)) * sizeof(double) <= (size_t)kTrainLdsMax ? 1 : 0;
     const size_t sm = (size_t)(mci::train_lds_doubles(maxn) + (a.spare ? mci::train_spare_doubles(maxn) : maxn)) * sizeof(double);
diff --git a/mcintegration.jl_amd/csrc/mci_host_jit.h b/mcintegration.jl_amd/csrc/mci_host_jit.h
--- a/mcintegration.jl_amd/csrc/mci_host_jit.h
+++ b/mcintegration.jl_amd/csrc/mci_host_jit.h
@@ -552,6 +552,56 @@
     return MCI_OK;
 }
 
+int mci_debug_stage1_fused(const mci_problem *p, int32_t *used, uint64_t *base) {
+    if (!p) return fail(MCI_ERR_INVALID, "NULL argument");
+    if (used) *used = p->launch.last_stage1_fused ? 1 : 0;
+    if (base) *base = p->stage1_base;
+    return MCI_OK;
+}
+
+int mci_debug_stage1(mci_problem *p, int32_t recompute, double *out, int64_t n) {
+    if (!p || !out) return fail(MCI_ERR_INVALID, "NULL argument");
+    if (p->ctx->offline) return fail(MCI_ERR_NO_DEVICE, "offline context");
+    const auto &s = p->shape;
+    const size_t count = (size_t)mci_problem::kGroups * (size_t)s.nbin;
+    if (s.nbin <= 0 || n != (int64_t)count) return fail(MCI_ERR_INVALID, "out must hold %d x %d doubles", (int)mci_problem::kGroups, s.nbin);
+    if (p->launch.last_hist_rows <= 0) return fail(MCI_ERR_INVALID, "the last sample launch left no partial histogram rows");
+    HIPCHK(hipSetDevice(p->ctx->device));
+    hipStream_t st = p->ctx->stream;
+    if (!recompute) {
+        HIPCHK(hipMemcpyAsync(out, p->d_stage1, count * sizeof(double), hipMemcpyDeviceToHost, st));
+        HIPCHK(hipStreamSynchronize(st));
+        return MCI_OK;
+    }
+    double *tmp = nullptr;
+    HIPCHK(hipMalloc((void **)&tmp, count * sizeof(double)));
+    hipLaunchKernelGGL(mci::k_hist_stage1, dim3((s.nbin + 255) / 256, mci_problem::kGroups), dim3(256), 0, st, p->d_part_hist, (int)p->launch.last_hist_rows, s.nbin,
+                       (int)mci_problem::kGroups, tmp);
+    hipError_t e = hipGetLastError();
+    if (e == hipSuccess) e = hipMemcpyAsync(out, tmp, count * sizeof(double), hipMemcpyDeviceToHost, st);
+    if (e == hipSuccess) e = hipStreamSynchronize(st);
+    (void)hipFree(tmp);
+    HIPCHK(e);
+    return MCI_OK;
+}
+
+int mci_debug_finish_trace(mci_problem *p, int32_t on, unsigned long long *out) {
+    if (!p) return fail(MCI_ERR_INVALID, "NULL argument");
+    if (p->ctx->offline) return fail(MCI_ERR_NO_DEVICE, "offline context");
+    HIPCHK(hipSetDevice(p->ctx->device));
+    if (on && !p->d_finish_trace) {
+        HIPCHK(hipMalloc((void **)&p->d_finish_trace, mci::kTrainStamps * sizeof(unsigned long long)));
+        HIPCHK(hipMemsetAsync(p->d_finish_trace, 0, mci::kTrainStamps * sizeof(unsigned long long), p->ctx->stream));
+    }
+    p->finish_trace = on != 0;
+    if (out) {
+        if (!p->d_finish_trace) return fail(MCI_ERR_INVALID, "no stamps: the trace was never switched on");
+        HIPCHK(hipMemcpyAsync(out, p->d_finish_trace, mci::kTrainStamps * sizeof(unsigned long long), hipMemcpyDeviceToHost, p->ctx->stream));
+        HIPCHK(hipStreamSynchronize(p->ctx->stream));
+    }
+    return MCI_OK;
+}
+
 int mci_debug_compiler_id(const char *set, char *out, int32_t n) {
     if (set) mcijit::compiler_id_override() = set;
     if (out && n > 0) snprintf(out, (size_t)n, "%s", mcijit::compiler_id().c_str());
diff --git a/mcintegration.jl_amd/csrc/mci_host_problem.h b/mcintegration.jl_amd/csrc/mci_host_problem.h
--- a/mcintegration.jl_amd/csrc/mci_host_problem.h
+++ b/mcintegration.jl_amd/csrc/mci_host_problem.h
@@ -330,6 +330,8 @@
         HIPCHK(hipMalloc((void **)&p->d_ghist, 3 * (size_t)(s.nbin ? s.nbin : 1) * sizeof(double)));
         HIPCHK(hipMemset(p->d_ghist, 0, 3 * (size_t)(s.nbin ? s.nbin : 1) * sizeof(double)));
         HIPCHK(hipMalloc((void **)&p->d_stage1, (size_t)mci_problem::kGroups * (s.nbin ? s.nbin : 1) * sizeof(double)));
+        HIPCHK(hipMalloc((void **)&p->d_stage1_arrive, (size_t)mci_problem::kGroups * mci::kCursorStride * sizeof(unsigned long long)));
+        HIPCHK(hipMemset(p->d_stage1_arrive, 0, (size_t)mci_problem::kGroups * mci::kCursorStride * sizeof(unsigned long long)));
         HIPCHK(hipMalloc((void **)&p->d_status, 4 * sizeof(int)));
         HIPCHK(hipMemset(p->d_status, 0, 4 * sizeof(int)));
         std::vector<mci::LeafDev> ld;
@@ -380,6 +382,8 @@
         if (p->d_carry_w) (void)hipFree(p->d_carry_w);
         if (p->d_clocks) (void)hipFree(p->d_clocks);
         if (p->d_cursor) (void)hipFree(p->d_cursor);
+        if (p->d_stage1_arrive) (void)hipFree(p->d_stage1_arrive);
+        if (p->d_finish_trace) (void)hipFree(p->d_finish_trace);
         if (p->d_edges_backup) (void)hipFree(p->d_edges_backup);
         if (p->h_hold) (void)hipHostFree(p->h_hold);
         if (p->h_hold_d) (void)hipHostFree(p->h_hold_d);
diff --git a/mcintegration.jl_amd/csrc/mci_host_strat.h b/mcintegration.jl_amd/csrc/mci_host_strat.h
--- a/mcintegration.jl_amd/csrc/mci_host_strat.h
+++ b/mcintegration.jl_amd/csrc/mci_host_strat.h
@@ -488,6 +488,8 @@
     if (p->launch.time_this_launch) HIPCHK(hipEventRecord(p->evs[2 * slot + 1], p->ctx->stream));
     p->launch.ev_valid[slot] = p->launch.time_this_launch;
     p->launch.clock_valid[slot] = false;
+    p->launch.self_timed[slot] = false;
+    p->launch.ev_recorded[slot] = p->launch.time_this_launch;
     p->launch.launches += 1;
     if (dumping) {
         hipStream_t hs = p->ctx->stream;
diff --git a/mcintegration.jl_amd/csrc/mci_host_types.h b/mcintegration.jl_amd/csrc/mci_host_types.h
--- a/mcintegration.jl_amd/csrc/mci_host_types.h
+++ b/mcintegration.jl_amd/csrc/mci_host_types.h
@@ -201,6 +201,10 @@
     unsigned long long *d_cursor = nullptr;
     int64_t cap_cursor = 0, cursor_nblocks = 0;
     unsigned long long cursor_base = 0;
+    unsigned long long *d_stage1_arrive = nullptr;
+    unsigned long long *d_finish_trace = nullptr;
+    bool finish_trace = false;
+    unsigned long long stage1_base = 0;
     hipFunction_t cursor_occ_f = nullptr;
     int cursor_occ_threads = 0, cursor_occ_resident = 0;
     int64_t cursor_occ_lds = 0;
@@ -219,6 +223,10 @@
         bool time_this_launch = true;
         bool ev_valid[kEvRing] = {};
         bool clock_valid[kEvRing] = {};
+        bool self_timed[kEvRing] = {};
+        bool ev_recorded[kEvRing] = {};
+        int64_t last_hist_rows = 0;
+        bool last_stage1_fused = false;
         int chain_cur = 0;
         bool chain_valid = false;
         int chain_solver = -1, chain_iteration = -1;
@@ -306,7 +314,7 @@
 
 namespace {
 struct Override { bool on = false; int64_t v = 0; };
-struct Overrides { Override table_mode, hist_tile_bins, no_split_all, l1_phase, train_walk, hist_copies, fresh_floors, fresh_burnin_pct, spec_self_check, split_chunk, vegas_self_check, vegas_cursor, cursor_log2_big, cursor_ones; } g_over;
+struct Overrides { Override table_mode, hist_tile_bins, no_split_all, l1_phase, train_walk, hist_copies, fresh_floors, fresh_burnin_pct, spec_self_check, split_chunk, vegas_self_check, vegas_cursor, cursor_log2_big, cursor_ones, stage1_fused; } g_over;
 Override *override_slot(const char *key) {
     if (!key) return nullptr;
     if (!strcmp(key, "table_mode")) return &g_over.table_mode;
@@ -323,6 +331,7 @@
     if (!strcmp(key, "vegas_cursor")) return &g_over.vegas_cursor;
     if (!strcmp(key, "cursor_log2_big")) return &g_over.cursor_log2_big;
     if (!strcmp(key, "cursor_ones")) return &g_over.cursor_ones;
+    if (!strcmp(key, "stage1_fused")) return &g_over.stage1_fused;
     return nullptr;
 }
 }
diff --git a/mcintegration.jl_amd/csrc/mci_static_kernels.h b/mcintegration.jl_amd/csrc/mci_static_kernels.h
--- a/mcintegration.jl_amd/csrc/mci_static_kernels.h
+++ b/mcintegration.jl_amd/csrc/mci_static_kernels.h
@@ -10,8 +10,8 @@
     const int bin = blockIdx.x * 256 + threadIdx.x;
     const int g = blockIdx.y;
     if (bin >= nbin) return;
-    const int per = (nwg + ngroup - 1) / ngroup;
-    const int w0 = g * per, w1 = min(nwg, w0 + per);
+    int w0, w1;
+    stage1_rows(nwg, ngroup, g, w0, w1);
     double s0 = 0.0, s1 = 0.0, s2 = 0.0, s3 = 0.0;
     int w = w0;
     for (; w + 3 < w1; w += 4) {
@@ -194,6 +194,8 @@
     double *hl = sm + train_lds_doubles(a.maxn);
     double *hp = a.packed + a.nstat + L.boff;
     const bool train = a.do_train && L.adapt;
+    unsigned long long *tt = (a.trace != nullptr && blockIdx.x == 0) ? reinterpret_cast<unsigned long long *>(ps + 200) : nullptr;
+    if (tt && tid < kTrainStamps) tt[tid] = tid == 12 ? wall_clock64() : 0ull;
     if (train) train_stage_grid(L, sm, a.edges);
     for (int i = tid; i < L.nbin; i += T) {
         const double v = merge_hist_bin(m, L.boff + i);
@@ -201,8 +203,12 @@
         hp[i] = v;
     }
     __syncthreads();
-    if (!train) return;
-    train_leaf(L, hl, hp, sm, ps, bad, ssum, a.edges, a.dacc, a.ddist, a.serial_walk, a.status, true, nullptr, false, a.spare ? hl : nullptr);
+    if (tt && tid == 0) tt[13] = wall_clock64();
+    if (train) train_leaf(L, hl, hp, sm, ps, bad, ssum, a.edges, a.dacc, a.ddist, a.serial_walk, a.status, true, tt, false, a.spare ? hl : nullptr);
+    if (tt) {
+        __syncthreads();
+        if (tid < kTrainStamps) a.trace[tid] = tt[tid];
+    }
 }
 
 struct StratAllocArgs {
diff --git a/mcintegration.jl_amd/csrc/mci_train.h b/mcintegration.jl_amd/csrc/mci_train.h
--- a/mcintegration.jl_amd/csrc/mci_train.h
+++ b/mcintegration.jl_amd/csrc/mci_train.h
@@ -222,7 +222,9 @@
     int *status;
     int maxn;
     int spare;
+    unsigned long long *trace;
 };
+enum { kTrainStamps = 16 };
 
 #ifndef MCI_TRAIN_SCAN_ONLY
 #define MCI_WALK_BIN(K, OFF, DN)                                                                                                       \
@@ -320,12 +322,7 @@
                                   double *__restrict__ edges, double *__restrict__ dacc, double *__restrict__ ddist, int serial_walk,
                                   int *__restrict__ status, bool staged = false, unsigned long long *tt = nullptr, bool checked = false,
                                   double *spare = nullptr) {
-#ifdef MCI_PERSIST_TRACE
 #define MCI_TT(k) if (tt && threadIdx.x == 0) tt[k] = wall_clock64();
-#else
-#define MCI_TT(k)
-    (void)tt;
-#endif
     const int tid = threadIdx.x, T = blockDim.x;
     const int N = L.nbin;
     double *d = sm;
@@ -535,6 +532,7 @@
             for (int k = nslot + tid; k < nslot + kWalkPad; k += T) es[k] = 0.0;
             __syncthreads();
         }
+        MCI_TT(8)
         int cnt;
         for (;;) {
             if (tid == 0) {
@@ -594,6 +592,7 @@
             if (*flag == 0) break;
             given = false;
         }
+        MCI_TT(9)
         if (tid == 0) atomicAdd(status + (given ? 1 : 2), 1);
         {
             int x = cnt;
@@ -661,8 +660,10 @@
     }
 #endif
     __syncthreads();
+    MCI_TT(10)
     if (hclear)
         for (int i = tid; i < N; i += T) hclear[i] = 1.0e-10;
+    MCI_TT(11)
 #undef MCI_TT
 }
 
diff --git a/mcintegration.jl_amd/engine.py b/mcintegration.jl_amd/engine.py
--- a/mcintegration.jl_amd/engine.py
+++ b/mcintegration.jl_amd/engine.py
@@ -581,6 +581,29 @@
         check(lib().mci_debug_walk_counts(self.p, out))
         return int(out[0]), int(out[1])
 
+    def last_launch_stage1_fused(self):
+        used, base = C.c_int32(0), C.c_uint64(0)
+        check(lib().mci_debug_stage1_fused(self.p, C.byref(used), C.byref(base)))
+        return bool(used.value), int(base.value)
+
+    def stage1(self, recompute=False):
+        nd = self.config.N + 1
+        nbin = self.packed_size - (2 * self.nobs + 2 + nd) - 2 * 3 * nd * max(nd, len(self.config.var))
+        out = np.empty((32, nbin))
+        check(lib().mci_debug_stage1(self.p, 1 if recompute else 0, _dp(out), out.size))
+        return out
+
+    def kernel_timing_both(self, n=512):
+        st, ev = np.empty(n), np.empty(n)
+        got = C.c_int32()
+        check(lib().mci_debug_kernel_timing(self.p, _dp(st), _dp(ev), n, C.byref(got)))
+        return st[:got.value].copy(), ev[:got.value].copy()
+
+    def finish_trace(self, on=True, read=False):
+        out = (C.c_uint64 * 16)()
+        check(lib().mci_debug_finish_trace(self.p, 1 if on else 0, out if read else None))
+        return np.array(out[:], dtype=np.uint64) if read else None
+
     def last_launch_cursor(self):
         used, base = C.c_int32(0), C.c_uint64(0)
         check(lib().mci_debug_vegas_cursor(self.p, C.byref(used), C.byref(base)))
```
